# iPERDance/iPERCore

Hardware: AMD Instinct MI355X
Metric: synthesized frames/sec at 512x512 (run_imitator) (higher is better)
Workload: dtype f32; 1 GPU; run_imitator 512x512 single src/ref pair, 300-frame reference clip frame-sharded over 1 GPU(s), AttLWB-SPADE generator fp32 (BASELINE configs[1] at N = 1, configs[2] at N = 8); poses=imitate, image_size=512, frame_batch=300, frame_batch_requested=384, world_size=1, parallelism=frame-shard x1, batches_in_flight=1, weights=random-init (seeded) of the real architecture, 36,276,992 params

## Files before the change

include/lwg_hip.h:

```cpp
#ifndef LWG_HIP_H
#define LWG_HIP_H

#include <stddef.h>
#include <stdint.h>

#ifdef __cplusplus
extern "C" {
#endif

typedef void* lwg_stream_t;

#define LWG_ABI_VERSION 10
int lwg_abi_version(void);

#define LWG_MAX_TAPS 52
enum { LWG_EPI_NONE = 0, LWG_EPI_RESIDUAL = 1, LWG_EPI_SPADE = 2 };
enum { LWG_ACTIVATION_NONE = 0, LWG_ACTIVATION_RELU = 1, LWG_ACTIVATION_TANH = 2, LWG_ACTIVATION_SIGMOID = 3 };
#define LWG_ACTIVATION_RELU_MASK 5
enum { LWG_DT_F32 = 0, LWG_DT_BF16 = 1,
       LWG_DT_F32_Q4 = 2 };

typedef struct LwgConvArgs {
    const float* x0;
    const float* x1;
    int C0, C1;
    int B, H, W;
    int OH, OW;
    int M;
    int stride;
    int ntaps;
    int cshift;
    const float* w;
    int N;
    const float* bias;
    float* y;
    int YH, YW, YC, ycoff;
    int omul, ooy, oox;
    int epi;
    int act;
    const float* res;
    const float* xn;
    const float* mean;
    const float* rstd;
    int xdt;
    int ydt;
    signed char dy[LWG_MAX_TAPS];
    signed char dx[LWG_MAX_TAPS];
} LwgConvArgs;

int lwg_conv2d_nhwc_f32(const LwgConvArgs* args, lwg_stream_t stream);
size_t lwg_conv2d_ws_floats(const LwgConvArgs* args);
int lwg_conv2d_nhwc_f32_ws(const LwgConvArgs* args, float* ws, lwg_stream_t stream);
int lwg_conv_slice_count(const LwgConvArgs* args);

int lwg_conv2d_nhwc_bf16(const LwgConvArgs* args, lwg_stream_t stream);
int lwg_conv2d_winograd_f32(const LwgConvArgs* args, lwg_stream_t stream);
size_t lwg_conv2d_winograd_ws_floats(const LwgConvArgs* args);
int lwg_conv2d_winograd_f32_ws(const LwgConvArgs* args, float* ws, lwg_stream_t stream);
int lwg_conv2d_winograd_plan(const LwgConvArgs* args, int with_ws, long long* blocks, int* slices, int* nbv, int* workgroups);
int lwg_winograd_panel_f32(const float* wpanel, float* upk, int Cin, int N, const int* tap9, lwg_stream_t stream);
typedef struct LwgWinoDesc {
    const float* wpanel;
    float* upk;
    int Cin, N, first_block;
    int tap9[9];
} LwgWinoDesc;
int lwg_winograd_panels_f32(const LwgWinoDesc* descs_dev, int ndesc, int total_blocks, lwg_stream_t stream);
int lwg_conv2d_winograd4_f32(const LwgConvArgs* args, lwg_stream_t stream);
int lwg_winograd4_panel_f32(const float* wpanel, float* upk, int Cin, int N, const int* tap9, lwg_stream_t stream);
int lwg_conv2d_nhwc_bf16_hr(const LwgConvArgs* args, lwg_stream_t stream);
int lwg_conv2d_winograd_bf16(const LwgConvArgs* args, lwg_stream_t stream);
int lwg_conv2d_nhwc_c8_bf16(const LwgConvArgs* args, lwg_stream_t stream);
int lwg_conv_transpose4_nhwc_bf16(const LwgConvArgs* args, lwg_stream_t stream);
int lwg_conv_transpose4_nhwc_f32(const LwgConvArgs* args, lwg_stream_t stream);
int lwg_conv_transpose4_is_one_grid(const LwgConvArgs* args);
int lwg_conv_transpose4_winograd_f32(const LwgConvArgs* args, lwg_stream_t stream);

int lwg_conv_transpose4_winograd24_f32(const LwgConvArgs* args, lwg_stream_t stream);

int lwg_conv2d_nhwc_f32_split(const LwgConvArgs* args, lwg_stream_t stream);

size_t lwg_conv2d_wgrad_ws_floats(int Ktot, int N, int M);
int lwg_conv2d_wgrad_nhwc_f32(const LwgConvArgs* args, const float* dy, float* dw, float* ws, lwg_stream_t stream);
int lwg_conv2d_wgrad_unpacked_f32(const LwgConvArgs* args, const float* dy, float* ws, float* dw, int D0, int D1, int KH, int KW,
                                  int transposed, const int* kidx, int cin, int nout, float* db, lwg_stream_t stream);
int lwg_colsum_nhwc_f32(const float* x, size_t rows, int C, float* out, float* ws, lwg_stream_t stream);
size_t lwg_conv2d_wgrad_winograd_ws_floats(const LwgConvArgs* args);
int lwg_conv2d_wgrad_winograd_f32(const LwgConvArgs* args, const float* dy, float* ws, float* dw, int cin, int nout, lwg_stream_t stream);

int lwg_act_bwd_f32(const float* dy, const float* y, size_t n, int act, float* out, lwg_stream_t stream);
int lwg_norm_fwd_nhwc_f32(const float* x, const float* mean, const float* rstd, const float* gamma, const float* beta, int gstride,
                          int B, int HW, int C, int act, float* y, lwg_stream_t stream);
int lwg_norm_bwd_nhwc_f32(const float* dy, const float* y, const float* x, const float* mean, const float* rstd,
                          const float* gamma, int gstride, int B, int HW, int C, int act, int nsplit, float* dx, float* dgamma,
                          float* dbeta, float* ws, lwg_stream_t stream);
int lwg_adam_step_f32(float* p, const float* g, float* m, float* v, size_t n, float lr, float beta1, float beta2, float eps, int t,
                      lwg_stream_t stream);
int lwg_adam_step_dev_f32(float* p, const float* g, float* m, float* v, size_t n, float lr, float beta1, float beta2, float eps,
                          int* t_dev, lwg_stream_t stream);
int lwg_pack_panel_f32(const float* w, int D0, int D1, int KH, int KW, int transposed, const int* kidx, int ntaps, int cin,
                       int cin_pad, int nout, int n_pad, float* out, lwg_stream_t stream);
int lwg_unpack_wgrad_f32(const float* dwk, int D0, int D1, int KH, int KW, int transposed, const int* kidx, int ntaps, int cin,
                         int cin_pad, int nout, int n_pad, float* dw, lwg_stream_t stream);
typedef struct LwgPackDesc {
    const float* w;
    float* out;
    int D1, KHW, transposed, ntaps, cin, cin_pad, nout, n_pad, Kp, first_block;
    int kidx[LWG_MAX_TAPS];
} LwgPackDesc;
int lwg_pack_panels_f32(const LwgPackDesc* descs_dev, int ndesc, int total_blocks, lwg_stream_t stream);
int lwg_maxpool2_fwd_nhwc_f32(const float* x, float* y, int B, int H, int W, int C, lwg_stream_t stream);
int lwg_maxpool2_bwd_nhwc_f32(const float* x, const float* dy, float* dx, int B, int H, int W, int C, lwg_stream_t stream);
int lwg_crop_resize_bilinear_f32(const float* x, const long long* box, float* y, float* valid, int N, int C, int H, int W, int OH, int OW,
                                 lwg_stream_t stream);
int lwg_crop_resize_bilinear_bwd_f32(const float* dy, const long long* box, float* dx, int N, int C, int H, int W, int OH, int OW, lwg_stream_t stream);
int lwg_prelu_f32(const float* x, const float* slope, const float* res, size_t rows, int C, float* y, lwg_stream_t stream);
int lwg_prelu_bwd_f32(const float* x, const float* slope, const float* dy, size_t rows, int C, float* dx, lwg_stream_t stream);

int lwg_instnorm_stats_nhwc_f32(const float* x, int B, int HW, int C, float eps, float* mean, float* rstd,
                                float* ws, int nsplit, lwg_stream_t stream);
int lwg_instnorm_stats_nhwc_bf16(const void* x, int B, int HW, int C, float eps, float* mean, float* rstd, float* ws, int nsplit,
                                 lwg_stream_t stream);
int lwg_instnorm_apply_nhwc_f32(const float* x, const float* mean, const float* rstd, const float* res,
                                float* y, int B, int HW, int C, int act, lwg_stream_t stream);

int lwg_flow_resize_f32(const float* T, int n, int S, int h, int w, float* out, lwg_stream_t stream);
int lwg_lwb_attention_f32(const float* q, const float* Ks, const float* Vs, const float* bk, const float* bv,
                          const float* T, float* out, int B, int ns, int h, int w, int C, int S,
                          int src_batched, lwg_stream_t stream);
int lwg_lwb_attention_bf16(const void* q, const void* Ks, const void* Vs, const float* bk, const float* bv, const float* T, void* out,
                           int B, int ns, int h, int w, int C, int S, int src_batched, lwg_stream_t stream);
int lwg_lwb_attention_x_records(int h, int w, int C, int element_size);
int lwg_lwb_attention_x_f32(const float* x, const float* Kq, const float* kappa, const float* Vs, const float* bv, const float* T,
                            float* out, float* stats, int B, int ns, int h, int w, int C, int src_batched, lwg_stream_t stream);
int lwg_lwb_attention_x_bf16(const void* x, const void* Kq, const float* kappa, const void* Vs, const float* bv, const float* T,
                             void* out, float* stats, int B, int ns, int h, int w, int C, int src_batched, lwg_stream_t stream);
size_t lwg_instnorm_finalize_ws_floats(int B, int C, int nrec);
int lwg_instnorm_finalize_f32(float* ws, int B, int C, int nrec, float eps, float* mean, float* rstd, lwg_stream_t stream);
int lwg_lwb_attention_bwd_f32(const float* q, const float* Ks, const float* Vs, const float* bk, const float* bv,
                              const float* T, const float* dout, float* dq, float* dKs, float* dVs, int B, int ns,
                              int h, int w, int C, int S, int src_batched, lwg_stream_t stream);
int lwg_lwb_attention_kv_f32(const float* q, const float* kv, const float* bk, const float* bv, const float* T, float* out,
                             int B, int ns, int h, int w, int C, int S, int src_batched, lwg_stream_t stream);
int lwg_lwb_attention_kv_bwd_f32(const float* q, const float* kv, const float* bk, const float* bv, const float* T,
                                 const float* dout, float* dq, float* dkv, int B, int ns, int h, int w, int C, int S,
                                 int src_batched, lwg_stream_t stream);
int lwg_lwb_fuse_f32(const float* tsf_x, const float* src_x, const float* gate, const float* T, float* out, int B, int ns,
                     int h, int w, int C, int S, int src_batched, float scale_w, float scale_o, lwg_stream_t stream);

size_t lwg_rasterize_ws_bytes(int B, int nf, int S);
int lwg_project_faces_f32(const float* verts, const float* cam, const int32_t* faces, int B, int nv, int nf,
                          float eye_dist, float* faces_v, float* f2pts, lwg_stream_t stream);
int lwg_rasterize_fim_wim_f32(const float* faces_v, int B, int nf, int S, float near, float far, int32_t* fim,
                              float* wim, void* ws, lwg_stream_t stream);
int lwg_texture_sample_f32(const int32_t* fim, const float* wim, const float* faces_v, const float* textures, int B, int nf,
                           int S, int T, int tex_batched, float eps, const float* bg_color3_host, float* rgb, lwg_stream_t stream);

int lwg_flow_compose_f32(const int32_t* fim, const float* wim, int B, int S, const float* map_fn, int nf,
                         const float* f_uvs2img, const float* uv_img4, int Hu, int Wu, const float* src_f2pts,
                         int ns, float* tsf_inputs, float* Tst, float* cond_nchw, float* Tuv, lwg_stream_t stream);
int lwg_bc_transform_f32(const float* f2pts, const int32_t* fim, const float* wim, int B, int S, int nf, float* T,
                         lwg_stream_t stream);
int lwg_encode_fim_f32(const int32_t* fim, const float* map_fn, int B, int S, int nf, int D, float* out,
                       lwg_stream_t stream);

size_t lwg_smpl_lbs_ws_floats(int B, int nv, int nj);
int lwg_smpl_lbs_f32(const float* pose, int pose_stride, const float* beta, int beta_stride, int nbeta,
                     const float* cam, int cam_stride, const float* v_template, const float* offsets, int off_batched,
                     const float* shapedirs, const float* posedirs, const float* J_regressor, const int32_t* parents,
                     const float* lbs_weights, const int32_t* links, int nlinks, int B, int nv, int nj, float* verts,
                     float* j3d, float* j2d, float* ws, lwg_stream_t stream);

int lwg_head_compose_f32(const float* x, const float* wpk, const float* bg, size_t bg_bstride, int B, int S, int C,
                         float* pred, float* mask, float* img, lwg_stream_t stream);
int lwg_head_compose_q4_f32(const float* x, const float* wpk, const float* bg, size_t bg_bstride, int B, int S, int C,
                            float* pred, float* mask, float* img, lwg_stream_t stream);
int lwg_thin_conv_f32(const float* x, const float* wpk, int B, int S, int C, int ks, float* y, lwg_stream_t stream);
int lwg_head_compose_bf16(const void* x, const void* wb, const float* bg, size_t bg_bstride, int B, int S, int C, float* pred,
                          float* mask, float* img, lwg_stream_t stream);
int lwg_up4_head_compose_bf16(const LwgConvArgs* args, const void* whead, const float* bg, size_t bg_bstride, float* pred, float* mask, float* img,
                              lwg_stream_t stream);
int lwg_frames_to_u8(const float* pred, int B, int S, int bgr, uint8_t* out, lwg_stream_t stream);
int lwg_nchw_to_nhwc_f32(const float* src, float* dst, int B, int C, int Cp, int P, lwg_stream_t stream);
int lwg_nhwc_to_nchw_f32(const float* src, float* dst, int B, int C, int Cs, int P, lwg_stream_t stream);

int lwg_morph_f32(const float* in, float* out, int n, int H, int W, int ks, int mode, float* ws, lwg_stream_t stream);
int lwg_canny_f32(const float* sil, int n, int H, int W, const float* gauss9, const float* sobelx9, float low, float high,
                  float* edges, float* ws, lwg_stream_t stream);
int lwg_boundary_fill_f32(const float* src, const float* confidant, const float* outpad, const float* edges, int n, int H,
                          int W, float* out, int32_t* top3, int32_t* ws, lwg_stream_t stream);
int lwg_grid_sample_nchw_f32(const float* img, size_t img_bstride, const float* grid, int n, int C, int H, int W, int Ho,
                             int Wo, float* out, lwg_stream_t stream);
int lwg_uv_merge_f32(const float* src_warp, const float* vis, int ns, int H, int W, float* out, lwg_stream_t stream);
int lwg_uv_merge_parts_f32(const float* uv_imgs, const float* vis, int n, int H, int W, float* out, lwg_stream_t stream);
int lwg_pack_inputs_f32(const float* a, int Ca, const float* b, int Cb, const float* mask, int n, int H, int W, int Cp,
                        float* out, lwg_stream_t stream);

int lwg_device_cu_count(void);

#ifdef __cplusplus
}
#endif
#endif
```

ipercore_amd/_lib.py:

```python
import ctypes
import os
import re

_HERE = os.path.dirname(os.path.abspath(__file__))
LIB_PATH = os.path.join(_HERE, "liblwg_hip.so")
HEADER_PATH = os.path.join(os.path.dirname(_HERE), "include", "lwg_hip.h")

LWG_MAX_TAPS = 52
EPI_NONE, EPI_RESIDUAL, EPI_SPADE = 0, 1, 2
ACT_NONE, ACT_RELU, ACT_TANH, ACT_SIGMOID, ACT_LRELU = 0, 1, 2, 3, 4
ACT_RELU_MASK = 5
DT_F32, DT_BF16, DT_F32_Q4 = 0, 1, 2

c_f = ctypes.c_void_p
c_i = ctypes.c_int


class LwgConvArgs(ctypes.Structure):
    _fields_ = [
        ("x0", c_f), ("x1", c_f),
        ("C0", c_i), ("C1", c_i),
        ("B", c_i), ("H", c_i), ("W", c_i),
        ("OH", c_i), ("OW", c_i),
        ("M", c_i), ("stride", c_i), ("ntaps", c_i), ("cshift", c_i),
        ("w", c_f), ("N", c_i), ("bias", c_f),
        ("y", c_f), ("YH", c_i), ("YW", c_i), ("YC", c_i), ("ycoff", c_i),
        ("omul", c_i), ("ooy", c_i), ("oox", c_i),
        ("epi", c_i), ("act", c_i),
        ("res", c_f), ("xn", c_f), ("mean", c_f), ("rstd", c_f),
        ("xdt", c_i), ("ydt", c_i),
        ("dy", ctypes.c_byte * LWG_MAX_TAPS), ("dx", ctypes.c_byte * LWG_MAX_TAPS),
    ]


class LwgWinoDesc(ctypes.Structure):
    _fields_ = [("wpanel", ctypes.c_void_p), ("upk", ctypes.c_void_p), ("Cin", c_i), ("N", c_i), ("first_block", c_i), ("tap9", c_i * 9)]


class LwgPackDesc(ctypes.Structure):
    _fields_ = [("w", c_f), ("out", c_f)] + [(n, c_i) for n in ("D1", "KHW", "transposed", "ntaps", "cin", "cin_pad", "nout", "n_pad", "Kp",
                                                               "first_block")] + [("kidx", c_i * LWG_MAX_TAPS)]


_SIGS = {
    "lwg_abi_version": (c_i, []),
    "lwg_device_cu_count": (c_i, []),
    "lwg_conv2d_nhwc_f32": (c_i, [ctypes.POINTER(LwgConvArgs), c_f]),
    "lwg_conv2d_ws_floats": (ctypes.c_size_t, [ctypes.POINTER(LwgConvArgs)]),
    "lwg_conv2d_nhwc_f32_ws": (c_i, [ctypes.POINTER(LwgConvArgs), c_f, c_f]),
    "lwg_conv2d_nhwc_bf16": (c_i, [ctypes.POINTER(LwgConvArgs), c_f]),
    "lwg_conv2d_winograd_f32": (c_i, [ctypes.POINTER(LwgConvArgs), c_f]),
    "lwg_conv2d_winograd_ws_floats": (ctypes.c_size_t, [ctypes.POINTER(LwgConvArgs)]),
    "lwg_conv2d_winograd_f32_ws": (c_i, [ctypes.POINTER(LwgConvArgs), c_f, c_f]),
    "lwg_conv2d_winograd_plan": (c_i, [ctypes.POINTER(LwgConvArgs), c_i, ctypes.POINTER(ctypes.c_longlong), ctypes.POINTER(c_i), ctypes.POINTER(c_i),
                                       ctypes.POINTER(c_i)]),
    "lwg_winograd_panel_f32": (c_i, [c_f, c_f, c_i, c_i, ctypes.POINTER(c_i), c_f]),
    "lwg_winograd_panels_f32": (c_i, [c_f, c_i, c_i, c_f]),
    "lwg_conv2d_winograd4_f32": (c_i, [ctypes.POINTER(LwgConvArgs), c_f]),
    "lwg_winograd4_panel_f32": (c_i, [c_f, c_f, c_i, c_i, ctypes.POINTER(c_i), c_f]),
    "lwg_conv2d_nhwc_bf16_hr": (c_i, [ctypes.POINTER(LwgConvArgs), c_f]),
    "lwg_conv2d_winograd_bf16": (c_i, [ctypes.POINTER(LwgConvArgs), c_f]),
    "lwg_conv2d_nhwc_c8_bf16": (c_i, [ctypes.POINTER(LwgConvArgs), c_f]),
    "lwg_conv_transpose4_nhwc_bf16": (c_i, [ctypes.POINTER(LwgConvArgs), c_f]),
    "lwg_conv_transpose4_nhwc_f32": (c_i, [ctypes.POINTER(LwgConvArgs), c_f]),
    "lwg_conv_transpose4_winograd_f32": (c_i, [ctypes.POINTER(LwgConvArgs), c_f]),
    "lwg_conv_transpose4_winograd24_f32": (c_i, [ctypes.POINTER(LwgConvArgs), c_f]),
    "lwg_conv_transpose4_is_one_grid": (c_i, [ctypes.POINTER(LwgConvArgs)]),
    "lwg_conv_slice_count": (c_i, [ctypes.POINTER(LwgConvArgs)]),
    "lwg_conv2d_nhwc_f32_split": (c_i, [ctypes.POINTER(LwgConvArgs), c_f]),
    "lwg_conv2d_wgrad_ws_floats": (ctypes.c_size_t, [c_i, c_i, c_i]),
    "lwg_conv2d_wgrad_nhwc_f32": (c_i, [ctypes.POINTER(LwgConvArgs), c_f, c_f, c_f, c_f]),
    "lwg_conv2d_wgrad_unpacked_f32": (c_i, [ctypes.POINTER(LwgConvArgs), c_f, c_f, c_f] + [c_i] * 5 + [ctypes.POINTER(ctypes.c_int), c_i, c_i, c_f, c_f]),
    "lwg_colsum_nhwc_f32": (c_i, [c_f, ctypes.c_size_t, c_i, c_f, c_f, c_f]),
    "lwg_conv2d_wgrad_winograd_ws_floats": (ctypes.c_size_t, [ctypes.POINTER(LwgConvArgs)]),
    "lwg_conv2d_wgrad_winograd_f32": (c_i, [ctypes.POINTER(LwgConvArgs), c_f, c_f, c_f, c_i, c_i, c_f]),
    "lwg_act_bwd_f32": (c_i, [c_f, c_f, ctypes.c_size_t, c_i, c_f, c_f]),
    "lwg_norm_fwd_nhwc_f32": (c_i, [c_f, c_f, c_f, c_f, c_f, c_i, c_i, c_i, c_i, c_i, c_f, c_f]),
    "lwg_norm_bwd_nhwc_f32": (c_i, [c_f, c_f, c_f, c_f, c_f, c_f, c_i, c_i, c_i, c_i, c_i, c_i, c_f, c_f, c_f, c_f, c_f]),
    "lwg_adam_step_f32": (c_i, [c_f, c_f, c_f, c_f, ctypes.c_size_t, ctypes.c_float, ctypes.c_float, ctypes.c_float, ctypes.c_float, c_i, c_f]),
    "lwg_adam_step_dev_f32": (c_i, [c_f, c_f, c_f, c_f, ctypes.c_size_t, ctypes.c_float, ctypes.c_float, ctypes.c_float, ctypes.c_float, c_f, c_f]),
    "lwg_pack_panel_f32": (c_i, [c_f] + [c_i] * 5 + [ctypes.POINTER(ctypes.c_int)] + [c_i] * 5 + [c_f, c_f]),
    "lwg_pack_panels_f32": (c_i, [c_f, c_i, c_i, c_f]),
    "lwg_unpack_wgrad_f32": (c_i, [c_f] + [c_i] * 5 + [ctypes.POINTER(ctypes.c_int)] + [c_i] * 5 + [c_f, c_f]),
    "lwg_maxpool2_fwd_nhwc_f32": (c_i, [c_f, c_f, c_i, c_i, c_i, c_i, c_f]),
    "lwg_maxpool2_bwd_nhwc_f32": (c_i, [c_f, c_f, c_f, c_i, c_i, c_i, c_i, c_f]),
    "lwg_crop_resize_bilinear_f32": (c_i, [c_f, c_f, c_f, c_f, c_i, c_i, c_i, c_i, c_i, c_i, c_f]),
    "lwg_crop_resize_bilinear_bwd_f32": (c_i, [c_f, c_f, c_f, c_i, c_i, c_i, c_i, c_i, c_i, c_f]),
    "lwg_prelu_f32": (c_i, [c_f, c_f, c_f, ctypes.c_size_t, c_i, c_f, c_f]),
    "lwg_prelu_bwd_f32": (c_i, [c_f, c_f, c_f, ctypes.c_size_t, c_i, c_f, c_f]),
    "lwg_instnorm_stats_nhwc_f32": (c_i, [c_f, c_i, c_i, c_i, ctypes.c_float, c_f, c_f, c_f, c_i, c_f]),
    "lwg_instnorm_apply_nhwc_f32": (c_i, [c_f, c_f, c_f, c_f, c_f, c_i, c_i, c_i, c_i, c_f]),
    "lwg_lwb_attention_f32": (c_i, [c_f, c_f, c_f, c_f, c_f, c_f, c_f, c_i, c_i, c_i, c_i, c_i, c_i, c_i, c_f]),
    "lwg_lwb_attention_bf16": (c_i, [c_f, c_f, c_f, c_f, c_f, c_f, c_f, c_i, c_i, c_i, c_i, c_i, c_i, c_i, c_f]),
    "lwg_instnorm_stats_nhwc_bf16": (c_i, [c_f, c_i, c_i, c_i, ctypes.c_float, c_f, c_f, c_f, c_i, c_f]),
    "lwg_head_compose_bf16": (c_i, [c_f, c_f, c_f, ctypes.c_size_t, c_i, c_i, c_i, c_f, c_f, c_f, c_f]),
    "lwg_up4_head_compose_bf16": (c_i, [ctypes.POINTER(LwgConvArgs), c_f, c_f, ctypes.c_size_t, c_f, c_f, c_f, c_f]),
    "lwg_flow_resize_f32": (c_i, [c_f, c_i, c_i, c_i, c_i, c_f, c_f]),
    "lwg_lwb_fuse_f32": (c_i, [c_f] * 5 + [c_i] * 7 + [ctypes.c_float, ctypes.c_float, c_f]),
    "lwg_lwb_attention_x_f32": (c_i, [c_f] * 8 + [c_i] * 6 + [c_f]),
    "lwg_lwb_attention_x_bf16": (c_i, [c_f] * 8 + [c_i] * 6 + [c_f]),
    "lwg_lwb_attention_x_records": (c_i, [c_i, c_i, c_i, c_i]),
    "lwg_instnorm_finalize_ws_floats": (ctypes.c_size_t, [c_i, c_i, c_i]),
    "lwg_instnorm_finalize_f32": (c_i, [c_f, c_i, c_i, c_i, ctypes.c_float, c_f, c_f, c_f]),
    "lwg_lwb_attention_bwd_f32": (c_i, [c_f] * 10 + [c_i] * 7 + [c_f]),
    "lwg_lwb_attention_kv_f32": (c_i, [c_f] * 6 + [c_i] * 7 + [c_f]),
    "lwg_lwb_attention_kv_bwd_f32": (c_i, [c_f] * 8 + [c_i] * 7 + [c_f]),
    "lwg_rasterize_ws_bytes": (ctypes.c_size_t, [c_i, c_i, c_i]),
    "lwg_project_faces_f32": (c_i, [c_f, c_f, c_f, c_i, c_i, c_i, ctypes.c_float, c_f, c_f, c_f]),
    "lwg_rasterize_fim_wim_f32": (c_i, [c_f, c_i, c_i, c_i, ctypes.c_float, ctypes.c_float, c_f, c_f, c_f, c_f]),
    "lwg_texture_sample_f32": (c_i, [c_f, c_f, c_f, c_f, c_i, c_i, c_i, c_i, c_i, ctypes.c_float, ctypes.POINTER(ctypes.c_float), c_f, c_f]),
    "lwg_flow_compose_f32": (c_i, [c_f, c_f, c_i, c_i, c_f, c_i, c_f, c_f, c_i, c_i, c_f, c_i, c_f, c_f, c_f, c_f, c_f]),
    "lwg_bc_transform_f32": (c_i, [c_f, c_f, c_f, c_i, c_i, c_i, c_f, c_f]),
    "lwg_encode_fim_f32": (c_i, [c_f, c_f, c_i, c_i, c_i, c_i, c_f, c_f]),
    "lwg_smpl_lbs_ws_floats": (ctypes.c_size_t, [c_i, c_i, c_i]),
    "lwg_smpl_lbs_f32": (c_i, [c_f, c_i, c_f, c_i, c_i, c_f, c_i, c_f, c_f, c_i, c_f, c_f, c_f, c_f, c_f, c_f, c_i, c_i, c_i,
                               c_i, c_f, c_f, c_f, c_f, c_f]),
    "lwg_head_compose_f32": (c_i, [c_f, c_f, c_f, ctypes.c_size_t, c_i, c_i, c_i, c_f, c_f, c_f, c_f]),
    "lwg_head_compose_q4_f32": (c_i, [c_f, c_f, c_f, ctypes.c_size_t, c_i, c_i, c_i, c_f, c_f, c_f, c_f]),
    "lwg_thin_conv_f32": (c_i, [c_f, c_f, c_i, c_i, c_i, c_i, c_f, c_f]),
    "lwg_nchw_to_nhwc_f32": (c_i, [c_f, c_f, c_i, c_i, c_i, c_i, c_f]),
    "lwg_nhwc_to_nchw_f32": (c_i, [c_f, c_f, c_i, c_i, c_i, c_i, c_f]),
    "lwg_frames_to_u8": (c_i, [c_f, c_i, c_i, c_i, c_f, c_f]),
    "lwg_morph_f32": (c_i, [c_f, c_f, c_i, c_i, c_i, c_i, c_i, c_f, c_f]),
    "lwg_canny_f32": (c_i, [c_f, c_i, c_i, c_i, ctypes.POINTER(ctypes.c_float), ctypes.POINTER(ctypes.c_float),
                            ctypes.c_float, ctypes.c_float, c_f, c_f, c_f]),
    "lwg_boundary_fill_f32": (c_i, [c_f, c_f, c_f, c_f, c_i, c_i, c_i, c_f, c_f, c_f, c_f]),
    "lwg_grid_sample_nchw_f32": (c_i, [c_f, ctypes.c_size_t, c_f, c_i, c_i, c_i, c_i, c_i, c_i, c_f, c_f]),
    "lwg_uv_merge_f32": (c_i, [c_f, c_f, c_i, c_i, c_i, c_f, c_f]),
    "lwg_uv_merge_parts_f32": (c_i, [c_f, c_f, c_i, c_i, c_i, c_f, c_f]),
    "lwg_pack_inputs_f32": (c_i, [c_f, c_i, c_f, c_i, c_f, c_i, c_i, c_i, c_i, c_f, c_f]),
}

_lib = None


def header_symbols():
    with open(HEADER_PATH) as fp:
        src = re.sub(r"/\*.*?\*/", "", fp.read(), flags=re.S)
    return sorted(set(re.findall(r"\b(lwg_[a-z0-9_]+)\s*\(", src)))


def lib():
    global _lib
    if _lib is None:
        if not os.path.exists(LIB_PATH):
            raise RuntimeError(
                f"{LIB_PATH} not found: the HIP kernels are not built (run `python -c 'import __graft_entry__ as g; "
                "g.build()'` or `make -C ipercore_amd/csrc`).  There is no CPU fallback.")
        import torch
        handle = ctypes.CDLL(LIB_PATH)
        for name, (res, args) in _SIGS.items():
            fn = getattr(handle, name)
            fn.restype = res
            fn.argtypes = args
        if handle.lwg_abi_version() != 10:
            raise RuntimeError("liblwg_hip.so ABI version mismatch")
        _lib = handle
    return _lib


def check(err, what):
    if err != 0:
        raise RuntimeError(f"{what} failed with hipError_t {err}")
```

ipercore_amd/csrc/conv_winograd4.hip:

```cpp
#include <hip/hip_runtime.h>
#include "lwg_common.h"
#include "lwg_conv_wino.h"

#define W4_THREADS 512
#define W4_PBX 8
#define W4_PBY 4
#define W4_NB 64
#define W4_KS 8
#define W4_HW 34
#define W4_HH 18
#ifndef W4_RS
#define W4_RS 40
#endif
#define W4_PLANE (18 * W4_RS + 4)
#define W4_RAW (W4_KS * W4_PLANE)
#define W4_VS (36 * W4_KS * 32)
#define W4_NEL (W4_HW * W4_HH * 2)
#define W4_NQ 3
#define W4_DUMP_OFF (2 * W4_RAW + 2 * W4_VS)
#define W4_DUMP (W4_THREADS + 3 * W4_PLANE)
#define W4_LOOP (W4_DUMP_OFF + W4_DUMP)
#define W4_MSR 68
#define W4_NPL 28
#define W4_MS (W4_NPL * 16 * W4_MSR)
#define W4_BIAS_OFF (W4_LOOP > W4_MS ? W4_LOOP : W4_MS)
#ifndef LWG_W4_XCD
#define LWG_W4_XCD 1
#endif
#ifndef LWG_W4_CHUNK
#define LWG_W4_CHUNK 1
#endif
#ifndef LWG_W4_RDMAP
#define LWG_W4_RDMAP 1
#endif
#ifndef LWG_W4_SMALL
#define LWG_W4_SMALL 1
#endif
#define W4SB() __builtin_amdgcn_sched_barrier(0)

#ifdef LWG_W4_TS
#define W4TS(i) do { if (tid == 0 && lab_bi == 1) reinterpret_cast<unsigned long long*>(const_cast<float*>(a.res))[(size_t)blockIdx.x * 16 + (i)] = __builtin_readcyclecounter(); } while (0)
#define W4TSA(i) do { if (tid == 0) reinterpret_cast<unsigned long long*>(const_cast<float*>(a.res))[(size_t)blockIdx.x * 16 + (i)] = __builtin_readcyclecounter(); } while (0)
#else
#define W4TS(i) do { } while (0)
#define W4TSA(i) do { } while (0)
#endif

#ifndef W4_NT
#define W4_NT 0
#endif
#ifndef W4_NT_LD
#define W4_NT_LD W4_NT
#endif
#ifndef W4_NT_RES
#define W4_NT_RES 0
#endif
#ifndef W4_NT_ST
#define W4_NT_ST 2
#endif

__device__ __forceinline__ void w4_bt6(const float (&r)[6], float (&v)[6]) {
    const float a = __builtin_fmaf(-4.f, r[2], r[4]), b = __builtin_fmaf(-4.f, r[1], r[3]);
    const float c = r[4] - r[2], e = r[3] - r[1];
    v[0] = __builtin_fmaf(-5.f, r[2], __builtin_fmaf(4.f, r[0], r[4]));
    v[1] = a + b;
    v[2] = a - b;
    v[3] = __builtin_fmaf(2.f, e, c);
    v[4] = __builtin_fmaf(-2.f, e, c);
    v[5] = __builtin_fmaf(-5.f, r[3], __builtin_fmaf(4.f, r[1], r[5]));
}

template <int EPI, bool TWO, bool SM = false>
__global__ __launch_bounds__(SM ? 256 : W4_THREADS, 1) void lwg_conv_winograd4_kernel(const LwgConvArgs a) {
    constexpr bool SMS = SM && EPI == LWG_EPI_SPADE;
    constexpr int NVP = SM && !SMS ? 2 : 1;
    constexpr int NTH = SM ? 256 : W4_THREADS;
    constexpr int NQ = SM ? 5 : W4_NQ;
    constexpr int NBV = SM ? 32 : W4_NB;
    constexpr int MSR = SM ? 36 : W4_MSR;
    constexpr int NHF = SM ? 2 : 1;
    extern __shared__ __attribute__((aligned(16))) float smem[];
    const int wid = __builtin_amdgcn_readfirstlane(threadIdx.x >> 6);
    const float* __restrict__ bias = a.bias;
    const int H = a.H, W = a.W, Cin = a.C0 + a.C1, N = a.N;
    float* __restrict__ y = a.y;
    float* const raw0 = smem;
    float* const Ms = smem;
    const int tid = threadIdx.x, lane = tid & 63;
    const CwGrid g = cw_grid(a.B, H, W, N, 4 * W4_PBX, 4 * W4_PBY, NBV);
    const CwOrder o = cw_order(cw4_order_kind(LWG_W4_XCD, LWG_W4_CHUNK, SM, gridDim.x, N / NBV, Cin, N, g.tiles, g.total), gridDim.x, blockIdx.x, N / NBV, g);
    int blk = blockIdx.x;
    const int nst = Cin / W4_KS;
    const __amdgpu_buffer_rsrc_t ru = __builtin_amdgcn_make_buffer_rsrc(const_cast<float*>(a.w), 0, (int)(144u * (unsigned)Cin * (unsigned)N), 0x00020000);
    const int q = wid & 3, ct = SM ? 0 : wid >> 2;
    const int half = SM ? 0 : wid >> 2;
    floatx16 acc[9];
    CwBlock<NQ, TWO> bk;
    unsigned uvoff, uvoffc;
    auto setup = [&](int id) {
        int cb, t;
        cw_block(o, id, cb, t);
        bk.locate(a, g, t, 4 * W4_PBX, 4 * W4_PBY, SMS ? cw4_n0_spade_small(cb) : cw_n0(cb, NBV));
        int tids = tid;
        asm volatile("" : "+v"(tids));
        bk.halo(a, tids, NTH, W4_HW, W4_NEL);
        const int col = SMS ? bk.n0 + (((lane & 31) >> 4) << 5) + (lane & 15) : bk.n0 + ct * 32 + (lane & 31);
        uvoff = (unsigned)(((lane >> 5) * 9 * N + 4 * col) * 4);
        uvoffc = (unsigned)(((lane >> 5) * 9 * N + 8 * N + col) * 4);
    };
    setup(blk);
    int wst[NQ];
#pragma unroll
    for (int k = 0; k < NQ; ++k) {
        const int i = tid + NTH * k;
        const int pix = i >> 1, hq = i & 1, hy = pix / W4_HW, hx = pix - hy * W4_HW;
        wst[k] = i < W4_NEL ? 4 * hq * W4_PLANE + hy * W4_RS + hx : W4_DUMP_OFF + tid;
    }
    floatx4 rreg[NQ];
    auto rld1 = [&](int st, int k) -> floatx4 {
#ifdef W4_LAB_HFIX
        const int c = 0 * st;
#else
        const int c = st * W4_KS;
#endif
        return bk.template rld1<W4_NT_LD>(a, c, k);
    };
    auto rst1 = [&](int buf, int k, floatx4 v) { cw_rst1(raw0 + buf * W4_RAW + wst[k], W4_PLANE, v); };
    floatx4 ufa[4], ufb[4];
    float ufc[4];
    const unsigned ukk = (unsigned)N * 72u;
    const unsigned uq = (unsigned)q * (unsigned)nst * 4u * ukk;
    const unsigned ubo = (unsigned)N * 16u;
    auto uldpart = [&](int set, int st, int kk, int part) {
#ifdef W4_LAB_UFIX
        const unsigned so = uq + 0u * (unsigned)(st + kk);
#else
        const unsigned so = uq + (unsigned)(st * 4 + kk) * ukk;
#endif
        if (part == 0) ufa[set] = cw_buf_load(ru, uvoff, so);
        else if (part == 1) ufb[set] = cw_buf_load(ru, uvoff, so + ubo);
        else ufc[set] = __builtin_bit_cast(float, __builtin_amdgcn_raw_buffer_load_b32(ru, (int)uvoffc, (int)so, 0));
    };
    auto uldset = [&](int set, int st, int kk) {
#ifdef W4_LAB_UFIX
        const unsigned so = uq + 0u * (unsigned)(st + kk);
#else
        const unsigned so = uq + (unsigned)(st * 4 + kk) * ukk;
#endif
        ufa[set] = cw_buf_load(ru, uvoff, so);
        ufb[set] = cw_buf_load(ru, uvoff, so + ubo);
        ufc[set] = __builtin_bit_cast(float, __builtin_amdgcn_raw_buffer_load_b32(ru, (int)uvoffc, (int)so, 0));
    };
    const int patch = tid & 31, tc = (tid >> 5) & 7;
    const int pty = patch >> 3, ptx = patch & 7;
    unsigned dbs = (unsigned)(tc * W4_PLANE + (4 * pty) * W4_RS + 4 * ptx) >> 2;
    asm volatile("" : "+v"(dbs));
    dbs <<= 2;
    unsigned dbx[NHF], vbx[NHF], vbt[NHF];
    float alpha[NHF], beta[NHF], nbeta[NHF];
#pragma unroll
    for (int hi = 0; hi < NHF; ++hi) {
        const int hf = SM ? hi : half;
        dbx[hi] = (unsigned)(tc * W4_PLANE + (4 * pty + hf) * W4_RS + 4 * ptx) >> 2;
        asm volatile("" : "+v"(dbx[hi]));
        dbx[hi] <<= 2;
        vbx[hi] = (unsigned)(2 * W4_RAW + (hf ? 30 : 0) * W4_KS * 32 + tc * 32 + patch);
        vbt[hi] = (unsigned)(2 * W4_RAW + (hf ? 18 : 6) * W4_KS * 32 + tc * 32 + patch);
        asm volatile("" : "+v"(vbx[hi]));
        asm volatile("" : "+v"(vbt[hi]));
        alpha[hi] = hf ? -1.f : -4.f;
        beta[hi] = hf ? 2.f : 1.f;
        nbeta[hi] = -beta[hi];
    }
    unsigned fbs[2];
    fbs[0] = (unsigned)(2 * W4_RAW + (6 * q) * W4_KS * 32 + lane);
    fbs[1] = (unsigned)(2 * W4_RAW + (6 * (4 + (q >> 1)) + 3 * (q & 1)) * W4_KS * 32 + lane);
    asm volatile("" : "+v"(fbs[0]));
    asm volatile("" : "+v"(fbs[1]));
    float fb[9];
    auto frag1 = [&](int buf, int kk, int j) -> float {
        return smem[fbs[j < 6 ? 0 : 1] + buf * W4_VS + ((j < 6 ? j : j - 6) * W4_KS + 2 * kk) * 32];
    };
    auto rd6 = [&](unsigned base, int buf, int r, float (&d)[6]) {
        const floatx4 v4 = *reinterpret_cast<const floatx4*>(smem + base + buf * W4_RAW + r * W4_RS);
        const float2 v2 = *reinterpret_cast<const float2*>(smem + base + buf * W4_RAW + r * W4_RS + 4);
        d[0] = v4[0]; d[1] = v4[1]; d[2] = v4[2]; d[3] = v4[3]; d[4] = v2.x; d[5] = v2.y;
    };
    auto vst6 = [&](unsigned base, int buf, int i, const float (&v)[6]) {
        float* dst = smem + base + buf * W4_VS + (6 * i) * W4_KS * 32;
#pragma unroll
        for (int nu = 0; nu < 6; ++nu) dst[nu * W4_KS * 32] = v[nu];
    };
    auto transform_full = [&](int buf) {
#pragma unroll
        for (int hi = 0; hi < NHF; ++hi) {
            float X[6], P[6], Q[6], v[6];
            {
                float dR[3][6];
                rd6(dbx[hi], buf, 0, dR[0]); rd6(dbx[hi], buf, 2, dR[1]); rd6(dbx[hi], buf, 4, dR[2]);
#pragma unroll
                for (int j = 0; j < 6; ++j) X[j] = __builtin_fmaf(-5.f, dR[1][j], __builtin_fmaf(4.f, dR[0][j], dR[2][j]));
            }
            {
                float dR[2][6];
                rd6(dbs, buf, 2, dR[0]); rd6(dbs, buf, 4, dR[1]);
#pragma unroll
                for (int j = 0; j < 6; ++j) P[j] = __builtin_fmaf(alpha[hi], dR[0][j], dR[1][j]);
                rd6(dbs, buf, 1, dR[0]); rd6(dbs, buf, 3, dR[1]);
#pragma unroll
                for (int j = 0; j < 6; ++j) Q[j] = __builtin_fmaf(alpha[hi], dR[0][j], dR[1][j]);
            }
            w4_bt6(X, v); vst6(vbx[hi], buf, 0, v);
            float T[6];
#pragma unroll
            for (int j = 0; j < 6; ++j) T[j] = __builtin_fmaf(beta[hi], Q[j], P[j]);
            w4_bt6(T, v); vst6(vbt[hi], buf, 0, v);
#pragma unroll
            for (int j = 0; j < 6; ++j) T[j] = __builtin_fmaf(nbeta[hi], Q[j], P[j]);
            w4_bt6(T, v); vst6(vbt[hi], buf, 1, v);
        }
    };
    auto iteration = [&](int s, auto SET, auto NXT) {
        constexpr int set = decltype(SET)::value;
        constexpr bool nxt = decltype(NXT)::value != 0;
        const int s3 = s + 3 < nst ? s + 3 : nst - 1;
        float X[6], P[6], Q[6], dR[3][6];
        auto mf = [&](int kk, int j, bool refill) {
            acc[j] = __builtin_amdgcn_mfma_f32_32x32x2f32(j < 4 ? ufa[kk][j & 3] : j < 8 ? ufb[kk][j & 3] : ufc[kk], fb[j], acc[j], 0, 0, 0);
#ifndef W4_KO_FRAG
            if (refill && (j & 1)) {
                fb[j - 1] = kk < 3 ? frag1(set, kk + 1, j - 1) : frag1(set ^ 1, 0, j - 1);
                fb[j] = kk < 3 ? frag1(set, kk + 1, j) : frag1(set ^ 1, 0, j);
            } else if (refill && j == 8) {
                fb[8] = kk < 3 ? frag1(set, kk + 1, 8) : frag1(set ^ 1, 0, 8);
            }
#endif
            W4SB();
        };
        auto ul = [&](int kk, int part) {
#ifndef W4_KO_ULD
            if (kk < 2) uldpart(kk + 2, s, kk + 2, part);
            else if (nxt) uldpart(kk - 2, s + 1, kk - 2, part);
#endif
            W4SB();
        };
        auto halo = [&](int k) {
#ifdef W4_KO_HALO
            return;
#endif
            if (nxt) { rst1(set, k, rreg[k]); rreg[k] = rld1(s3, k); }
            W4SB();
        };
#ifdef W4_KO_TR
        constexpr bool trn = false;
// ... 126 lines not shown
    for (int j = 0; j < 9; ++j) fb[j] = frag1(0, 0, j);
#pragma unroll
    for (int j = 0; j < 9; ++j)
#pragma unroll
        for (int r = 0; r < 16; ++r) acc[j][r] = 0.f;
    if (q == 1) {
#pragma unroll
        for (int g = 0; g < 4; ++g) {
            const floatx4 b4 = *reinterpret_cast<const floatx4*>(smem + W4_BIAS_OFF + ct * 32 + 8 * g + 4 * (lane >> 5));
#pragma unroll
            for (int k = 0; k < 4; ++k) acc[1][4 * g + k] = b4[k];
        }
    }
    W4TS(1);
    {
        int s = 0;
        for (; s + 2 < nst; s += 2) {
            iteration(s, IntC<0>(), IntC<1>());
            iteration(s + 1, IntC<1>(), IntC<1>());
        }
        iteration(s, IntC<0>(), IntC<1>());
        iteration(s + 1, IntC<1>(), IntC<0>());
    }
    W4TS(2);
    const int eb = bk.b, ex0 = bk.x0, ey0 = bk.y0, en0 = bk.n0;
#pragma unroll
    for (int r = 0; r < 16; ++r) {
        const float m0 = acc[0][r], m1 = acc[1][r], m2 = acc[2][r], m3 = acc[3][r], m4 = acc[4][r], m5 = acc[5][r];
        const float s12 = m1 + m2, d12 = m1 - m2, s34 = m3 + m4, d34 = m3 - m4;
        acc[0][r] = (m0 + s12) + s34;
        acc[1][r] = __builtin_fmaf(2.f, d34, d12);
        acc[2][r] = __builtin_fmaf(4.f, s34, s12);
        acc[3][r] = __builtin_fmaf(8.f, d34, d12) + m5;
    }
    if (q & 1) {
#pragma unroll
        for (int r = 0; r < 16; ++r) {
            const float h0 = acc[6][r], h1 = acc[7][r];
            acc[6][r] = h0 + h1;
            acc[7][r] = h0 - h1;
        }
    } else {
#pragma unroll
        for (int r = 0; r < 16; ++r) {
            const float h0 = acc[6][r], h1 = acc[7][r], h2 = acc[8][r];
            acc[6][r] = (h0 + h1) + h2;
            acc[7][r] = h1 - h2;
            acc[8][r] = h1 + h2;
        }
    }
    W4TS(4);
    int tide = tid;
    asm volatile("" : "+v"(tide));
    const int lanee = tide & 63;
    const int rb = wid & 3;
    const unsigned l5 = (unsigned)lanee & 31u, gsel = (0x0FF0F00Fu >> l5) & 1u;
    const int gidx = __builtin_popcount((gsel ? 0x0FF0F00Fu : 0xF00F0FF0u) & ((1u << l5) - 1u));
    const int p16 = LWG_W4_RDMAP && !SM ? (wid >> 2) * 4 + 2 * (lanee >> 5) + (gsel ? 0 : 1) + 8 * (gidx >> 3) : (wid >> 2) * 8 + (lanee >> 3);
    const int n4 = SMS ? (lanee & 3) * 4 : LWG_W4_RDMAP && !SM ? (gidx & 7) * 4 : (lanee & 7) * 4;
    const int cbase = SMS ? (en0 >> 6) * 32 + ((en0 >> 4) & 1) * 16 : en0 >> 1;
    floatx4 mu, rs;
    if (EPI == LWG_EPI_SPADE) {
        mu = *reinterpret_cast<const floatx4*>(a.mean + (size_t)eb * a.YC + cbase + n4);
        rs = *reinterpret_cast<const floatx4*>(a.rstd + (size_t)eb * a.YC + cbase + n4);
    }
    typedef unsigned int w4_u4 __attribute__((ext_vector_type(4)));
    const unsigned img_bytes = (unsigned)(H * W) * (unsigned)a.YC * 4u;
    const __amdgpu_buffer_rsrc_t ry = __builtin_amdgcn_make_buffer_rsrc(y + (size_t)eb * H * W * a.YC, 0, (int)img_bytes, 0x00020000);
    const float* const esrc = EPI == LWG_EPI_SPADE ? a.xn : EPI == LWG_EPI_RESIDUAL ? a.res : a.y;
    const __amdgpu_buffer_rsrc_t re = __builtin_amdgcn_make_buffer_rsrc(const_cast<float*>(esrc) + (size_t)eb * H * W * a.YC, 0, (int)img_bytes, 0x00020000);
    const int chan = EPI == LWG_EPI_SPADE ? cbase + n4 : a.ycoff + en0 + n4;
    bool more = false;
    int nblk = blk;
#pragma unroll
    for (int ph = 0; ph < 2; ++ph) {
        if (ph == 1) __syncthreads();
        if (((lanee >> 4) & 1) == ph) {
            float* dst = Ms + (lanee & 15) * MSR + ct * 32 + 4 * (lanee >> 5);
#pragma unroll
            for (int g = 0; g < 4; ++g) {
#pragma unroll
                for (int bb = 0; bb < 4; ++bb)
                    *reinterpret_cast<floatx4*>(dst + (4 * q + bb) * 16 * MSR + 8 * g) = floatx4{acc[bb][4 * g], acc[bb][4 * g + 1], acc[bb][4 * g + 2], acc[bb][4 * g + 3]};
#pragma unroll
                for (int i = 0; i < 3; ++i)
                    *reinterpret_cast<floatx4*>(dst + (16 + 3 * q + i) * 16 * MSR + 8 * g) = floatx4{acc[6 + i][4 * g], acc[6 + i][4 * g + 1], acc[6 + i][4 * g + 2], acc[6 + i][4 * g + 3]};
            }
        }
        unsigned vo[NVP][4];
#pragma unroll
        for (int hp = 0; hp < NVP; ++hp) {
            const int p = ph * 16 + (SMS ? lanee >> 2 : SM ? 8 * hp + (lanee >> 3) : p16);
            const int ox = ex0 + 4 * (p & 7) + rb, oyb = ey0 + 4 * (p >> 3);
#pragma unroll
            for (int i = 0; i < 4; ++i)
                vo[hp][i] = cw4_out_voff(ox, oyb + i, H, W, a.YC, chan);
        }
        floatx4 ext[2][4];
        if (EPI != LWG_EPI_NONE) {
#pragma unroll
            for (int h = 0; h < (EPI == LWG_EPI_SPADE ? 1 : 2); ++h)
#pragma unroll
                for (int i = 0; i < 4; ++i) ext[h][i] = __builtin_bit_cast(floatx4, __builtin_amdgcn_raw_buffer_load_b128(re, (int)cw4_out_group(vo[NVP == 2 ? h : 0][i], h, !SM), 0, W4_NT_RES));
        }
        if (ph == 1) {
            W4TS(8);
            nblk = blk + (int)gridDim.x;
            more = cw_has_block(o, nblk);
            setup(more ? nblk : blk);
            W4TS(9);
            issue_loads();
            W4TS(10);
        }
        __syncthreads();
        if (ph == 0) W4TS(5); else W4TS(7);
        floatx4 gam[4];
#pragma unroll
        for (int h = 0; h < 2; ++h) {
            const float* base = Ms + (SMS ? lanee >> 2 : SM ? 8 * h + (lanee >> 3) : p16) * MSR + (SMS ? h * 16 : SM ? 0 : h * 32) + n4;
            floatx4 F[6];
#pragma unroll
            for (int xi = 0; xi < 4; ++xi) F[xi] = *reinterpret_cast<const floatx4*>(base + (4 * xi + rb) * 16 * MSR);
            const int ia = rb == 0 ? 0 : rb == 2 ? 2 : 1, ib = (rb & 1) ? 4 : 3;
            const float cb = (float)(1 << rb);
#pragma unroll
            for (int r = 0; r < 2; ++r) {
                const float* hb = base + (16 + 6 * r) * 16 * MSR;
                const floatx4 pa = *reinterpret_cast<const floatx4*>(hb + ia * 16 * MSR);
                const floatx4 pb = *reinterpret_cast<const floatx4*>(hb + ib * 16 * MSR);
                floatx4 f;
#pragma unroll
                for (int c = 0; c < 4; ++c) f[c] = __builtin_fmaf(cb, pb[c], pa[c]);
                if (rb == 3) f += *reinterpret_cast<const floatx4*>(hb + 5 * 16 * MSR);
                F[4 + r] = f;
            }
            floatx4 o[4];
#pragma unroll
            for (int c = 0; c < 4; ++c) {
                const float s12 = F[1][c] + F[2][c], d12 = F[1][c] - F[2][c], s34 = F[3][c] + F[4][c], d34 = F[3][c] - F[4][c];
                o[0][c] = (F[0][c] + s12) + s34;
                o[1][c] = __builtin_fmaf(2.f, d34, d12);
                o[2][c] = __builtin_fmaf(4.f, s34, s12);
                o[3][c] = __builtin_fmaf(8.f, d34, d12) + F[5][c];
            }
            if (EPI == LWG_EPI_SPADE) {
                if (h == 0) {
#pragma unroll
                    for (int i = 0; i < 4; ++i) gam[i] = o[i];
                    continue;
                }
#pragma unroll
                for (int i = 0; i < 4; ++i)
#pragma unroll
                    for (int c = 0; c < 4; ++c) o[i][c] = (ext[0][i][c] - mu[c]) * rs[c] * (1.f + gam[i][c]) + o[i][c];
            } else if (EPI == LWG_EPI_RESIDUAL) {
                if (a.act == LWG_ACT_RELU_MASK) {
#pragma unroll
                    for (int i = 0; i < 4; ++i)
#pragma unroll
                        for (int c = 0; c < 4; ++c) o[i][c] = ext[h][i][c] > 0.f ? o[i][c] : 0.f;
                } else {
#pragma unroll
                    for (int i = 0; i < 4; ++i) o[i] += ext[h][i];
                }
            }
            lwg_act_dispatch(a.act, [&](auto ACTC) {
                constexpr int EA = decltype(ACTC)::value;
#pragma unroll
                for (int i = 0; i < 4; ++i)
#pragma unroll
                    for (int c = 0; c < 4; ++c) o[i][c] = lwg_act_c<EA>(o[i][c], a.act);
            });
#pragma unroll
            for (int i = 0; i < 4; ++i)
                __builtin_amdgcn_raw_buffer_store_b128(__builtin_bit_cast(w4_u4, o[i]), ry, (int)cw4_out_group(vo[NVP == 2 ? h : 0][i], h, EPI != LWG_EPI_SPADE && !SM), 0, W4_NT_ST);
        }
        if (ph == 0) W4TS(6);
    }
    W4TS(3);
#ifdef LWG_W4_TS
    ++lab_bi;
#endif
    if (!more) break;
    blk = nblk;
    __syncthreads();
    }
    W4TSA(12);
#ifdef LWG_W4_TS
    if (tid == 0) reinterpret_cast<unsigned long long*>(const_cast<float*>(a.res))[(size_t)blockIdx.x * 16 + 13] = (unsigned long long)lab_bi;
#endif
}


__global__ __launch_bounds__(256) void lwg_winograd4_panel_kernel(const float* __restrict__ wp, float* __restrict__ U, int Cin, int N, LwgWinoTaps taps) {
    const int n = blockIdx.x * 64 + (threadIdx.x & 63), c = blockIdx.y * 4 + (threadIdx.x >> 6);
    if (n >= N || c >= Cin) return;
    double g[3][3];
#pragma unroll
    for (int r = 0; r < 3; ++r)
#pragma unroll
        for (int s = 0; s < 3; ++s) {
            const int k = ((c >> 5) * 9 + taps.t[3 * r + s]) * 32 + (c & 31);
            g[r][s] = (double)wp[((size_t)(k >> 2) * N + n) * 4 + (k & 3)];
        }
    const double G[6][3] = {{1.0 / 4, 0, 0}, {-1.0 / 6, -1.0 / 6, -1.0 / 6}, {-1.0 / 6, 1.0 / 6, -1.0 / 6}, {1.0 / 24, 1.0 / 12, 1.0 / 6}, {1.0 / 24, -1.0 / 12, 1.0 / 6}, {0, 0, 1}};
    double t[6][3];
#pragma unroll
    for (int i = 0; i < 6; ++i)
#pragma unroll
        for (int s = 0; s < 3; ++s) t[i][s] = G[i][0] * g[0][s] + G[i][1] * g[1][s] + G[i][2] * g[2][s];
    const int s8 = c >> 3, kk = (c & 7) >> 1, kh = c & 1;
#pragma unroll
    for (int qq = 0; qq < 4; ++qq) {
        float* dst = U + ((((size_t)qq * (Cin >> 3) + s8) * 4 + kk) * 2 + kh) * 9 * (size_t)N;
        float o[9];
#pragma unroll
        for (int j = 0; j < 9; ++j) {
            const int xi = j < 6 ? qq : 4 + (qq >> 1), nu = j < 6 ? j : 3 * (qq & 1) + (j - 6);
            o[j] = (float)(t[xi][0] * G[nu][0] + t[xi][1] * G[nu][1] + t[xi][2] * G[nu][2]);
        }
        *reinterpret_cast<floatx4*>(dst + 4 * n) = floatx4{o[0], o[1], o[2], o[3]};
        *reinterpret_cast<floatx4*>(dst + 4 * (size_t)N + 4 * n) = floatx4{o[4], o[5], o[6], o[7]};
        dst[8 * (size_t)N + n] = o[8];
    }
}

extern "C" int lwg_winograd4_panel_f32(const float* wpanel, float* upk, int Cin, int N, const int* tap9, lwg_stream_t stream_) {
    LwgWinoTaps taps;
    if (!cw_panel_args_ok(wpanel, upk, Cin, N, tap9, taps)) return (int)hipErrorInvalidValue;
    hipLaunchKernelGGL(lwg_winograd4_panel_kernel, dim3((unsigned)((N + 63) / 64), (unsigned)((Cin + 3) / 4)), dim3(256), 0,
                       reinterpret_cast<hipStream_t>(stream_), wpanel, upk, Cin, N, taps);
    return (int)hipGetLastError();
}

template <int EPI, bool SM>
static int lwg_wino4_go(const LwgConvArgs& a, dim3 grid, size_t lds, hipStream_t stream) {
    return a.C1 > 0 ? cw_launch<lwg_conv_winograd4_kernel<EPI, true, SM>>(grid, SM ? 256 : W4_THREADS, lds, stream, a)
                    : cw_launch<lwg_conv_winograd4_kernel<EPI, false, SM>>(grid, SM ? 256 : W4_THREADS, lds, stream, a);
}

extern "C" int lwg_conv2d_winograd4_f32(const LwgConvArgs* pa, lwg_stream_t stream_) {
    hipStream_t stream = reinterpret_cast<hipStream_t>(stream_);
    if (!pa || !cw_contract_ok(*pa, 144ull, 256ll)) return (int)hipErrorInvalidValue;
    const LwgConvArgs& a = *pa;
    const size_t lds = (size_t)(W4_BIAS_OFF + 64) * 4;
    const int cus = lwg_device_cus();
    long long total = cw_total_blocks(a.B, a.H, a.W, a.N, 4 * W4_PBX, 4 * W4_PBY, W4_NB);
    const bool sm = LWG_W4_SMALL && 2 * total <= cus;
    if (sm) total *= 2;
    const dim3 grid = cw_persistent_grid(total, cus);
    if (a.epi == LWG_EPI_SPADE) return sm ? lwg_wino4_go<LWG_EPI_SPADE, true>(a, grid, lds, stream) : lwg_wino4_go<LWG_EPI_SPADE, false>(a, grid, lds, stream);
    if (a.epi == LWG_EPI_RESIDUAL) return sm ? lwg_wino4_go<LWG_EPI_RESIDUAL, true>(a, grid, lds, stream) : lwg_wino4_go<LWG_EPI_RESIDUAL, false>(a, grid, lds, stream);
    return sm ? lwg_wino4_go<LWG_EPI_NONE, true>(a, grid, lds, stream) : lwg_wino4_go<LWG_EPI_NONE, false>(a, grid, lds, stream);
}
```

ipercore_amd/csrc/lwb_attn_x.hip:

```cpp
#include "lwg_common.h"
#include "lwg_conv_args.h"

typedef unsigned int uintx4 __attribute__((ext_vector_type(4)));

template <typename ST> struct AttnXTraits;
template <> struct AttnXTraits<float> {
    static constexpr int CPL = 4;
    __device__ static __forceinline__ void unpack(const uintx4 v, float (&f)[4]) {
#pragma unroll
        for (int k = 0; k < 4; ++k) {
            const unsigned u = v[k];
            f[k] = __builtin_bit_cast(float, u);
        }
    }
    __device__ static __forceinline__ uintx4 pack(const float (&f)[4]) {
        uintx4 v;
#pragma unroll
        for (int k = 0; k < 4; ++k) v[k] = __builtin_bit_cast(unsigned, f[k]);
        return v;
    }
};
template <> struct AttnXTraits<__bf16> {
    static constexpr int CPL = 8;
    __device__ static __forceinline__ void unpack(const uintx4 v, float (&f)[8]) {
#pragma unroll
        for (int k = 0; k < 4; ++k) {
            f[2 * k] = __builtin_bit_cast(float, v[k] << 16);
            f[2 * k + 1] = __builtin_bit_cast(float, v[k] & 0xffff0000u);
        }
    }
    __device__ static __forceinline__ uintx4 pack(const float (&f)[8]) {
        typedef __bf16 bf16x2 __attribute__((ext_vector_type(2)));
        uintx4 v;
#pragma unroll
        for (int k = 0; k < 4; ++k) {
            bf16x2 p;
            p[0] = (__bf16)f[2 * k];
            p[1] = (__bf16)f[2 * k + 1];
            v[k] = __builtin_bit_cast(unsigned, p);
        }
        return v;
    }
};

template <typename ST, int LPP, bool STATS, int NSU, int PW, int OCC, bool PIPE = false>
__global__ __launch_bounds__(256 * PW, PW == 1 ? OCC : 1) void lwg_lwb_attnx_kernel(const ST* __restrict__ x, const ST* __restrict__ Kq,
                                                                 const float* __restrict__ kappa, const ST* __restrict__ Vs,
                                                                 const float* __restrict__ bv, const float* __restrict__ T,
                                                                 ST* __restrict__ out, float* __restrict__ stats, int B, int ns, int h, int w,
                                                                 int src_batched) {
    using TR = AttnXTraits<ST>;
    constexpr int CPL = TR::CPL;
    constexpr int C = CPL * LPP;
    constexpr int PPW = 64 / LPP;
    constexpr int PPP = 4 * PPW;
    constexpr int NPASS = 64 / PPP;
    constexpr int NIT = NPASS / PW;
    static_assert(NPASS % PW == 0, "PW must divide the tile's pass count");
    constexpr int NT = NSU > 0 ? NSU : 1;
    constexpr unsigned ROWB = (unsigned)C * sizeof(ST);
    const int lane = threadIdx.x & 63, wid = threadIdx.x >> 6;
    const int wq = wid & 3, pl = wid >> 2;
    const int cl = lane % LPP, pg = lane / LPP;
    const int tiles_x = (w + 7) >> 3;
    int tile, b;
    if (LWG_ATTNX_INTERLEAVE) {
        const int xcd = blockIdx.x & 7;
        const long idx = blockIdx.x >> 3;
        const long grp = idx / B;
        tile = (int)(grp * 8 + xcd);
        b = (int)(idx - grp * B);
        if (tile >= tiles_x * ((h + 7) >> 3)) return;
    } else {
        const long L = lwg_xcd_remap(blockIdx.x, gridDim.x);
        tile = (int)(L / B);
        b = (int)(L - (long)tile * B);
    }
    const int ty = tile / tiles_x, tx = tile - ty * tiles_x;
    const int hw = h * w;
    const unsigned nsrc = (unsigned)(src_batched ? B * ns : ns);
    __amdgpu_buffer_rsrc_t rK = __builtin_amdgcn_make_buffer_rsrc(const_cast<ST*>(Kq), 0, (int)(nsrc * (unsigned)hw * ROWB), 0x00020000);
    __amdgpu_buffer_rsrc_t rV = __builtin_amdgcn_make_buffer_rsrc(const_cast<ST*>(Vs), 0, (int)(nsrc * (unsigned)hw * ROWB), 0x00020000);
    __amdgpu_buffer_rsrc_t rA = __builtin_amdgcn_make_buffer_rsrc(const_cast<float*>(kappa), 0, (int)(nsrc * (unsigned)hw * 4u), 0x00020000);
    const float inv_sqrt_c = 1.0f / sqrtf((float)C);
    constexpr bool BV_REG = CPL == 4 || LWG_ATTNX_BVREG16;
    float bvr[CPL];
    if (BV_REG) {
#pragma unroll
        for (int k = 0; k < CPL; ++k) bvr[k] = bv[CPL * cl + k];
    }
    const float2* Tb = reinterpret_cast<const float2*>(T) + (size_t)b * ns * hw;

    auto pixel_of = [&](int pass, int& yc, int& xc) -> bool {
        const int p = pass * PPP + wq * PPW + pg;
        const int y = ty * 8 + (p >> 3), xx = tx * 8 + (p & 7);
        const bool live = y < h && xx < w;
        yc = live ? y : ty * 8;
        xc = live ? xx : tx * 8;
        return live;
    };
    extern __shared__ __attribute__((aligned(16))) char smem_ax[];
    char* xs = smem_ax;
    float2* Tl = reinterpret_cast<float2*>(smem_ax + NPASS * 4096);
    {
        __amdgpu_buffer_rsrc_t rX = __builtin_amdgcn_make_buffer_rsrc(const_cast<ST*>(x) + (size_t)b * hw * C, 0, (int)((unsigned)hw * ROWB), 0x00020000);
#pragma unroll
        for (int it = 0; it < NIT; ++it) {
            const int pass = it * PW + pl;
            int yc, xc;
            pixel_of(pass, yc, xc);
            const unsigned voff = (unsigned)(yc * w + xc) * ROWB + (unsigned)(CPL * cl) * (unsigned)sizeof(ST);
            __builtin_amdgcn_raw_ptr_buffer_load_lds(rX, (__attribute__((address_space(3))) void*)(xs + (pass * 4 + wq) * 1024), 16, (int)voff, 0, 0, 0);
        }
        for (int i = threadIdx.x; i < ns * 64; i += 256 * PW) {
            const int s = i >> 6, p = i & 63;
            const int y = ty * 8 + (p >> 3), xx = tx * 8 + (p & 7);
            const bool in = y < h && xx < w;
            Tl[i] = Tb[(size_t)s * hw + (size_t)(in ? y : ty * 8) * w + (in ? xx : tx * 8)];
        }
        asm volatile("s_waitcnt vmcnt(0)" ::: "memory");
        __syncthreads();
    }
    auto x_row = [&](int pass) -> uintx4 { return *reinterpret_cast<const uintx4*>(xs + ((pass * 4 + wq) * 64 + lane) * 16); };

    float shift[CPL], s1[CPL], s2[CPL];
    if (STATS) {
        TR::unpack(*reinterpret_cast<const uintx4*>(xs + cl * 16), shift);
#pragma unroll
        for (int k = 0; k < CPL; ++k) s1[k] = s2[k] = 0.f;
    }
    int nlive = 0;
    auto stats_add = [&](const float (&xv)[CPL]) {
        ++nlive;
        if (PW == 1) {
#pragma unroll
            for (int k = 0; k < CPL; ++k) {
                const float d = xv[k] - shift[k];
                s1[k] += d;
                s2[k] = __builtin_fmaf(d, d, s2[k]);
            }
        }
    };
    auto taps_of = [&](const float2 t, float (&wt)[4], int& tx0, int& ty0) {
        const float ix = ((t.x + 1.f) * (float)w - 1.f) * 0.5f, iy = ((t.y + 1.f) * (float)h - 1.f) * 0.5f;
        const float fx0 = floorf(ix), fy0 = floorf(iy);
        const float wx1 = ix - fx0, wy1 = iy - fy0, wx0 = (fx0 + 1.f) - ix, wy0 = (fy0 + 1.f) - iy;
        tx0 = (int)fminf(fmaxf(fx0, -2.f), (float)w + 1.f);
        ty0 = (int)fminf(fmaxf(fy0, -2.f), (float)h + 1.f);
        wt[0] = wy0 * wx0; wt[1] = wy0 * wx1; wt[2] = wy1 * wx0; wt[3] = wy1 * wx1;
    };
    auto fold = [&](const float (&ka)[CPL], const float (&va)[CPL], float kap, const float (&xv)[CPL], float& mrun, float& lrun, float (&o)[CPL]) {
        float dot = 0.f;
#pragma unroll
        for (int k = 0; k < CPL; ++k) dot = __builtin_fmaf(ka[k], xv[k], dot);
#pragma unroll
        for (int off = LPP >> 1; off > 0; off >>= 1) dot += __shfl_xor(dot, off, 64);
        const float logit = (dot + kap) * inv_sqrt_c;
        const float mnew = fmaxf(mrun, logit);
        const float corr = expf(mrun - mnew);
        const float pr = expf(logit - mnew);
        lrun = __builtin_fmaf(lrun, corr, pr);
#pragma unroll
        for (int k = 0; k < CPL; ++k) o[k] = __builtin_fmaf(o[k], corr, pr * va[k]);
        mrun = mnew;
    };
    auto finish = [&](long gp, float lrun, const float (&o)[CPL]) {
        const float invl = 1.f / lrun;
        float r[CPL];
        if (!BV_REG) {
#pragma unroll
            for (int k = 0; k < CPL; k += 4) {
                const floatx4 b4 = *reinterpret_cast<const floatx4*>(bv + CPL * cl + k);
#pragma unroll
                for (int j = 0; j < 4; ++j) bvr[k + j] = b4[j];
            }
        }
#pragma unroll
        for (int k = 0; k < CPL; ++k) r[k] = __builtin_fmaf(o[k], invl, bvr[k]);
        *reinterpret_cast<uintx4*>(out + gp * C + CPL * cl) = TR::pack(r);
    };

    if constexpr (PIPE) {
        static_assert(NSU == 2 && PW == 1 && (NIT % 2) == 0, "the pipelined form is the ns = 2 frame-batch form");
        bool mine = false;
#pragma unroll 1
        for (int it = 0; it < NIT; ++it) {
            int yc, xc;
            const bool live = pixel_of(it, yc, xc);
            const int ptile = it * PPP + wq * PPW + pg;
#pragma unroll
            for (int s = 0; s < 2; ++s) {
                const float2 t = Tl[s * 64 + ptile];
                float wt[4];
                int tx0, ty0;
                taps_of(t, wt, tx0, ty0);
                mine |= live && tx0 >= -1 && tx0 < w && ty0 >= -1 && ty0 < h;
            }
        }
        if (__syncthreads_or(mine ? 1 : 0) == 0) {
#pragma unroll 1
            for (int it = 0; it < NIT; ++it) {
                int yc, xc;
                const bool live = pixel_of(it, yc, xc);
                float xv[CPL];
                TR::unpack(x_row(it), xv);
                if (live) {
                    if (STATS) stats_add(xv);
                    float o[CPL];
#pragma unroll
                    for (int k = 0; k < CPL; ++k) o[k] = 0.f;
                    finish(((long)b * h + yc) * w + xc, 2.f, o);
                }
            }
        } else {
            struct Taps { uintx4 kr[2][4], vr[2][4]; float ar[2][4], wt[2][4]; };
            auto issue = [&](int pass, Taps& g) {
                int yc, xc;
                const bool live = pixel_of(pass, yc, xc);
                const int ptile = pass * PPP + wq * PPW + pg;
#pragma unroll
                for (int s = 0; s < 2; ++s) {
                    int tx0, ty0;
                    taps_of(Tl[s * 64 + ptile], g.wt[s], tx0, ty0);
                    const unsigned pbase = (unsigned)(src_batched ? b * ns + s : s) * (unsigned)hw;
#pragma unroll
                    for (int tp = 0; tp < 4; ++tp) {
                        const int tyy = ty0 + (tp >> 1), txx = tx0 + (tp & 1);
                        const bool ok = live && tyy >= 0 && tyy < h && txx >= 0 && txx < w;
                        const unsigned pix = pbase + (unsigned)(tyy * w + txx);
                        const unsigned voff = ok ? pix * ROWB + (unsigned)(CPL * cl) * (unsigned)sizeof(ST) : 0xC0000000u;
                        g.kr[s][tp] = __builtin_bit_cast(uintx4, __builtin_amdgcn_raw_buffer_load_b128(rK, (int)voff, 0, 0));
                        g.vr[s][tp] = __builtin_bit_cast(uintx4, __builtin_amdgcn_raw_buffer_load_b128(rV, (int)voff, 0, 0));
                        g.ar[s][tp] = __builtin_bit_cast(float, __builtin_amdgcn_raw_buffer_load_b32(rA, ok ? (int)(pix * 4u) : (int)0xC0000000u, 0, 0));
                    }
                }
            };
            auto consume = [&](int pass, const Taps& g) {
                int yc, xc;
                const bool live = pixel_of(pass, yc, xc);
                float xv[CPL];
                TR::unpack(x_row(pass), xv);
                if (STATS && live) stats_add(xv);
                float mrun = -INFINITY, lrun = 0.f;
                float o[CPL];
#pragma unroll
                for (int k = 0; k < CPL; ++k) o[k] = 0.f;
#pragma unroll
                for (int s = 0; s < 2; ++s) {
                    float ka[CPL], va[CPL], kap = 0.f;
#pragma unroll
                    for (int k = 0; k < CPL; ++k) ka[k] = va[k] = 0.f;
#pragma unroll
                    for (int tp = 0; tp < 4; ++tp) {
                        float k8[CPL], v8[CPL];
                        TR::unpack(g.kr[s][tp], k8);
                        TR::unpack(g.vr[s][tp], v8);
#pragma unroll
                        for (int k = 0; k < CPL; ++k) {
                            ka[k] = __builtin_fmaf(k8[k], g.wt[s][tp], ka[k]);
                            va[k] = __builtin_fmaf(v8[k], g.wt[s][tp], va[k]);
                        }
                        kap = __builtin_fmaf(g.ar[s][tp], g.wt[s][tp], kap);
                    }
                    fold(ka, va, kap, xv, mrun, lrun, o);
                }
                if (live) finish(((long)b * h + yc) * w + xc, lrun, o);
            };
            Taps g0, g1;
            issue(0, g0);
#pragma unroll 1
            for (int it = 0; it < NIT; it += 2) {
                issue(it + 1, g1);
                consume(it, g0);
                issue(it + 2 < NIT ? it + 2 : it + 1, g0);
                consume(it + 1, g1);
            }
        }
    } else {
#pragma unroll 1
    for (int it = 0; it < NIT; ++it) {
        const int pass = it * PW + pl;
        int yc, xc;
        const bool live = pixel_of(pass, yc, xc);
        const long gp = ((long)b * h + yc) * w + xc;
        const int ptile = pass * PPP + wq * PPW + pg;
        float xv[CPL];
        TR::unpack(x_row(pass), xv);
        if (STATS && live) stats_add(xv);
        float mrun = -INFINITY, lrun = 0.f;
        float o[CPL];
#pragma unroll
        for (int k = 0; k < CPL; ++k) o[k] = 0.f;

        auto source = [&](int s, const float2 t) {
            float wt[4];
            int tx0, ty0;
            taps_of(t, wt, tx0, ty0);
            const bool any_tap = live && tx0 >= -1 && tx0 < w && ty0 >= -1 && ty0 < h;
            float ka[CPL], va[CPL], kap = 0.f;
#pragma unroll
            for (int k = 0; k < CPL; ++k) ka[k] = va[k] = 0.f;
            if (__builtin_amdgcn_ballot_w64(any_tap) != 0ull) {
                const unsigned sidx = (unsigned)(src_batched ? b * ns + s : s);
                const unsigned pbase = sidx * (unsigned)hw;
                uintx4 kr[4], vr[4];
                float ar[4];
#pragma unroll
                for (int tp = 0; tp < 4; ++tp) {
                    const int tyy = ty0 + (tp >> 1), txx = tx0 + (tp & 1);
                    const bool ok = live && tyy >= 0 && tyy < h && txx >= 0 && txx < w;
                    const unsigned pix = pbase + (unsigned)(tyy * w + txx);
                    const unsigned voff = ok ? pix * ROWB + (unsigned)(CPL * cl) * (unsigned)sizeof(ST) : 0xC0000000u;
                    kr[tp] = __builtin_bit_cast(uintx4, __builtin_amdgcn_raw_buffer_load_b128(rK, (int)voff, 0, 0));
                    vr[tp] = __builtin_bit_cast(uintx4, __builtin_amdgcn_raw_buffer_load_b128(rV, (int)voff, 0, 0));
                    ar[tp] = __builtin_bit_cast(float, __builtin_amdgcn_raw_buffer_load_b32(rA, ok ? (int)(pix * 4u) : (int)0xC0000000u, 0, 0));
                }
#pragma unroll
                for (int tp = 0; tp < 4; ++tp) {
                    float k8[CPL], v8[CPL];
                    TR::unpack(kr[tp], k8);
                    TR::unpack(vr[tp], v8);
#pragma unroll
                    for (int k = 0; k < CPL; ++k) {
                        ka[k] = __builtin_fmaf(k8[k], wt[tp], ka[k]);
                        va[k] = __builtin_fmaf(v8[k], wt[tp], va[k]);
                    }
                    kap = __builtin_fmaf(ar[tp], wt[tp], kap);
                }
            }
            fold(ka, va, kap, xv, mrun, lrun, o);
        };
        if (NSU > 0) {
#pragma unroll
            for (int s = 0; s < NT; ++s) source(s, Tl[s * 64 + ptile]);
        } else {
#pragma unroll 1
            for (int s = 0; s < ns; ++s) source(s, Tl[s * 64 + ptile]);
        }
        if (live) finish(gp, lrun, o);
    }
    }

    if (STATS) {
        if (PW > 1) {
            __shared__ float acc[4][64][2 * CPL];
            if (pl == 0) {
#pragma unroll
                for (int k = 0; k < 2 * CPL; ++k) acc[wq][lane][k] = 0.f;
            }
            __syncthreads();
#pragma unroll 1
            for (int p = 0; p < NPASS; ++p) {
                if (pl == p % PW) {
                    int yc, xc;
                    if (pixel_of(p, yc, xc)) {
                        float xv[CPL];
                        TR::unpack(x_row(p), xv);
#pragma unroll
                        for (int k = 0; k < CPL; ++k) {
                            const float d = xv[k] - shift[k];
                            acc[wq][lane][k] += d;
                            acc[wq][lane][CPL + k] = __builtin_fmaf(d, d, acc[wq][lane][CPL + k]);
                        }
                    }
                }
                __syncthreads();
            }
            if (pl == 0) {
#pragma unroll
                for (int k = 0; k < CPL; ++k) {
                    s1[k] = acc[wq][lane][k];
                    s2[k] = acc[wq][lane][CPL + k];
                }
            }
        }
        __syncthreads();
        float (*sh)[2][C] = reinterpret_cast<float (*)[2][C]>(smem_ax);
        float* shn = reinterpret_cast<float*>(smem_ax + 4 * 2 * C * sizeof(float));
        float fn = (float)nlive;
#pragma unroll
        for (int off = LPP; off < 64; off <<= 1) {
#pragma unroll
            for (int k = 0; k < CPL; ++k) {
                s1[k] += __shfl_xor(s1[k], off, 64);
                s2[k] += __shfl_xor(s2[k], off, 64);
            }
            fn += __shfl_xor(fn, off, 64);
        }
        if (pg == 0) {
            if (pl == 0) {
#pragma unroll
                for (int k = 0; k < CPL; ++k) {
                    sh[wq][0][CPL * cl + k] = s1[k];
                    sh[wq][1][CPL * cl + k] = s2[k];
                }
            }
            if (cl == 0) shn[wid] = fn;
        }
        __syncthreads();
        if (wid == 0 && pg == 0) {
            float tn = 0.f;
#pragma unroll
            for (int k = 0; k < 4 * PW; ++k) tn += shn[k];
            const int nrec = tiles_x * ((h + 7) >> 3);
#pragma unroll
            for (int k = 0; k < CPL; ++k) {
                const int c = CPL * cl + k;
                const float t1 = ((sh[0][0][c] + sh[1][0][c]) + sh[2][0][c]) + sh[3][0][c];
                const float t2 = ((sh[0][1][c] + sh[1][1][c]) + sh[2][1][c]) + sh[3][1][c];
                const float mean = shift[k] + t1 / tn;
                const float m2 = t2 - t1 * t1 / tn;
                float* rec = stats + (((size_t)b * nrec + tile) * C + c) * 3;
                rec[0] = tn;
                rec[1] = mean;
                rec[2] = m2 > 0.f ? m2 : 0.f;
            }
        }
    }
}

extern "C" int lwg_lwb_attention_x_records(int h, int w, int C, int esz) {
    if (h <= 0 || w <= 0 || C <= 0 || (esz != 2 && esz != 4)) return 0;
    const int lpp = C / (16 / esz);
    if (lpp < 8 || lpp > 64 || (lpp & (lpp - 1)) != 0) return 0;
    return ((w + 7) >> 3) * ((h + 7) >> 3);
}

template <typename ST>
static int lwg_attnx_launch(const ST* x, const ST* Kq, const float* kappa, const ST* Vs, const float* bv, const float* T, ST* out, float* stats,
                            int B, int ns, int h, int w, int C, int src_batched, hipStream_t stream) {
    if (!x || !Kq || !kappa || !Vs || !bv || !T || !out || B <= 0 || ns <= 0 || ns > 64 || h <= 0 || w <= 0) return (int)hipErrorInvalidValue;
    const unsigned long long nsrc = (unsigned long long)(src_batched ? B * ns : ns);
    if (nsrc * (unsigned long long)h * w * (unsigned long long)C * sizeof(ST) >= 0xC0000000ull) return (int)hipErrorInvalidValue;
    const long tiles = (long)((w + 7) >> 3) * ((h + 7) >> 3);
    constexpr int CPL = AttnXTraits<ST>::CPL;
    const int npass = (C / CPL) / 4;
    const dim3 grid((unsigned)((LWG_ATTNX_INTERLEAVE ? (tiles + 7) / 8 * 8 : tiles) * B));
    const bool wide = LWG_ATTNX_WIDE && tiles * B < 512 && npass >= 4;
#define LWG_ATTNX_GO(LPP, ST_, NSU, PW)                                                                                              \
    {                                                                                                                                \
             \
        constexpr bool pipe = LWG_ATTNX_PIPE && CPL == 4 && (LPP) == 64 && (NSU) == 2 && (PW) == 1;                                  \
        auto kern = lwg_lwb_attnx_kernel<ST, LPP, ST_, NSU, PW, (pipe ? 2 : CPL == 4 ? LWG_ATTNX_OCC : LWG_ATTNX_OCC16), pipe>;        \
        const size_t lds = (size_t)((LPP) / 4) * 4096 + (size_t)ns * 512;                         \
        static unsigned long long lds_ok = 0;                                                                                        \
        if (lds > 65536) {                                                                                                           \
            const hipError_t e = lwg_allow_dynamic_lds(reinterpret_cast<const void*>(kern), lds, lds_ok);                            \
            if (e != hipSuccess) return (int)e;                                                                                      \
        }                                                                                                                            \
        hipLaunchKernelGGL(kern, grid, dim3(256 * PW), lds, stream, x, Kq, kappa, Vs, bv, T, out, stats, B, ns, h, w, src_batched);   \
    }
#define LWG_ATTNX_PW(LPP, ST_, NSU)                                                                                                  \
    {                                                                                                                                \
        if constexpr ((LPP) / 4 >= 4) {                                                                                              \
            if (wide) LWG_ATTNX_GO(LPP, ST_, NSU, 4) else LWG_ATTNX_GO(LPP, ST_, NSU, 1)                                             \
        } else {                                                                                                                     \
            LWG_ATTNX_GO(LPP, ST_, NSU, 1)                                                                                           \
        }                                                                                                                            \
    }
#define LWG_ATTNX_LAUNCH(LPP)                                                                                                        \
    if (stats) { if (LWG_ATTNX_NSU2 && ns == 2) LWG_ATTNX_PW(LPP, true, 2) else LWG_ATTNX_PW(LPP, true, 0) }                         \
    else { if (LWG_ATTNX_NSU2 && ns == 2) LWG_ATTNX_PW(LPP, false, 2) else LWG_ATTNX_PW(LPP, false, 0) }
    switch (C / CPL) {
        case 8: LWG_ATTNX_LAUNCH(8) break;
        case 16: LWG_ATTNX_LAUNCH(16) break;
        case 32: LWG_ATTNX_LAUNCH(32) break;
        case 64: if constexpr (CPL == 4) { LWG_ATTNX_LAUNCH(64) break; }
                 return (int)hipErrorInvalidValue;
        default: return (int)hipErrorInvalidValue;
    }
#undef LWG_ATTNX_LAUNCH
#undef LWG_ATTNX_PW
#undef LWG_ATTNX_GO
    return (int)hipGetLastError();
}

extern "C" int lwg_lwb_attention_x_f32(const float* x, const float* Kq, const float* kappa, const float* Vs, const float* bv, const float* T,
                                       float* out, float* stats, int B, int ns, int h, int w, int C, int src_batched, lwg_stream_t stream_) {
    if (C != 32 && C != 64 && C != 128 && C != 256) return (int)hipErrorInvalidValue;
    return lwg_attnx_launch<float>(x, Kq, kappa, Vs, bv, T, out, stats, B, ns, h, w, C, src_batched, reinterpret_cast<hipStream_t>(stream_));
}

extern "C" int lwg_lwb_attention_x_bf16(const void* x, const void* Kq, const float* kappa, const void* Vs, const float* bv, const float* T,
                                        void* out, float* stats, int B, int ns, int h, int w, int C, int src_batched, lwg_stream_t stream_) {
    if (C != 64 && C != 128 && C != 256) return (int)hipErrorInvalidValue;
    return lwg_attnx_launch<__bf16>(static_cast<const __bf16*>(x), static_cast<const __bf16*>(Kq), kappa, static_cast<const __bf16*>(Vs), bv, T,
                                    static_cast<__bf16*>(out), stats, B, ns, h, w, C, src_batched, reinterpret_cast<hipStream_t>(stream_));
}

__global__ __launch_bounds__(1024) void lwg_in_stats_merge_seg(const float* __restrict__ ws, int C, int nrec, int nseg, float eps,
                                                              float* __restrict__ part, float* __restrict__ mean, float* __restrict__ rstd) {
    const int lane = threadIdx.x & 63, wid = threadIdx.x >> 6;
    const int c = blockIdx.x * 64 + lane, b = blockIdx.y, seg = blockIdx.z;
    const bool cok = c < C;
    const float* base = ws + ((size_t)b * nrec * C + (cok ? c : 0)) * 3;
    const float r = base[1];
    const int per = (nrec + nseg - 1) / nseg;
    const int r0 = seg * per, r1 = min(nrec, r0 + per);
    float sa = 0.f, ss = 0.f, sq = 0.f;
    if (cok) {
        for (int i = r0 + wid; i < r1; i += 16) {
            const float* o = base + (size_t)i * C * 3;
            const float n = o[0], d = o[1] - r;
            sa += n;
            ss = __builtin_fmaf(n, d, ss);
            sq += __builtin_fmaf(n * d, d, o[2]);
        }
    }
    __shared__ float sh[16][3][64];
    sh[wid][0][lane] = sa;
    sh[wid][1][lane] = ss;
    sh[wid][2][lane] = sq;
    __syncthreads();
    if (wid == 0 && cok) {
        float ta = 0.f, ts = 0.f, tq = 0.f;
#pragma unroll
        for (int k = 0; k < 16; ++k) { ta += sh[k][0][lane]; ts += sh[k][1][lane]; tq += sh[k][2][lane]; }
        if (nseg == 1) {
            const float m2 = tq - ts * ts / ta;
            mean[(size_t)b * C + c] = r + ts / ta;
            rstd[(size_t)b * C + c] = 1.0f / sqrtf((m2 > 0.f ? m2 : 0.f) / ta + eps);
        } else {
            float* o = part + (((size_t)b * nseg + seg) * C + c) * 3;
            o[0] = ta; o[1] = ts; o[2] = tq;
        }
    }
}

__global__ __launch_bounds__(256) void lwg_in_stats_merge_fin(const float* __restrict__ ws, const float* __restrict__ part, int BC, int C, int nrec,
                                                             int nseg, float eps, float* __restrict__ mean, float* __restrict__ rstd) {
    const int i = blockIdx.x * 256 + threadIdx.x;
    if (i >= BC) return;
    const int b = i / C, c = i - b * C;
    const float r = ws[((size_t)b * nrec * C + c) * 3 + 1];
    float ta = 0.f, ts = 0.f, tq = 0.f;
    for (int s = 0; s < nseg; ++s) {
        const float* o = part + (((size_t)b * nseg + s) * C + c) * 3;
        ta += o[0]; ts += o[1]; tq += o[2];
    }
    const float m2 = tq - ts * ts / ta;
    mean[i] = r + ts / ta;
    rstd[i] = 1.0f / sqrtf((m2 > 0.f ? m2 : 0.f) / ta + eps);
}

extern "C" size_t lwg_instnorm_finalize_ws_floats(int B, int C, int nrec) {
    if (B <= 0 || C <= 0 || nrec <= 0) return 0;
    const size_t nseg = nrec > 512 ? (size_t)(nrec + 255) / 256 : 0;
    return (size_t)B * nrec * C * 3 + (size_t)B * nseg * C * 3;
}
extern "C" int lwg_instnorm_finalize_f32(float* ws, int B, int C, int nrec, float eps, float* mean, float* rstd, lwg_stream_t stream_) {
    if (!ws || !mean || !rstd || B <= 0 || C <= 0 || nrec <= 0 || B > 65535) return (int)hipErrorInvalidValue;
    hipStream_t stream = reinterpret_cast<hipStream_t>(stream_);
    const int nseg = nrec > 512 ? (nrec + 255) / 256 : 1;
    if (nseg > 65535) return (int)hipErrorInvalidValue;
    float* part = ws + (size_t)B * nrec * C * 3;
    hipLaunchKernelGGL(lwg_in_stats_merge_seg, dim3((C + 63) / 64, B, nseg), dim3(1024), 0, stream, ws, C, nrec, nseg, eps, part, mean, rstd);
    if (nseg > 1)
        hipLaunchKernelGGL(lwg_in_stats_merge_fin, dim3((B * C + 255) / 256), dim3(256), 0, stream, ws, part, B * C, C, nrec, nseg, eps, mean, rstd);
    return (int)hipGetLastError();
}
```

ipercore_amd/csrc/lwg_conv_epilogue.h:

```cpp
#pragma once
#include "lwg_common.h"
#include "lwg_conv_args.h"

template <int TM, int TN, int EPI, int EA>
__device__ __forceinline__ void lwg_conv_epilogue_a(const LwgConvArgs& a, floatx16 (&acc)[TM][TN], int m_base, int n_base,
                                                    int wm, int wn, int lane, int ooy_add, int oox_add) {
    const int khalf = lane >> 5;
    const int HW = a.OH * a.OW;
    const bool direct = (a.omul == 1) && (a.YH == a.OH) && (a.YW == a.OW);
    const int ncol0 = n_base + wn * TN * 32 + 4 * khalf;
    floatx4 bias4[TN][4];
#pragma unroll
    for (int j = 0; j < TN; ++j)
#pragma unroll
        for (int g = 0; g < 4; ++g) {
            bias4[j][g] = floatx4{0.f, 0.f, 0.f, 0.f};
            if (a.bias) bias4[j][g] = *reinterpret_cast<const floatx4*>(a.bias + ncol0 + 32 * j + 8 * g);
        }
#pragma unroll
    for (int i = 0; i < TM; ++i) {
        const int m = m_base + wm * TM * 32 + i * 32 + (lane & 31);
        if (m >= a.M) continue;
        size_t opix = (size_t)m;
        int bimg = 0;
        if (!direct || EPI == LWG_EPI_SPADE) {
            const int b = m / HW;
            bimg = b;
            if (!direct) {
                const int rem = m - b * HW;
                const int oy = rem / a.OW, ox = rem - oy * a.OW;
                opix = ((size_t)b * a.YH + (oy * a.omul + a.ooy + ooy_add)) * a.YW + (ox * a.omul + a.oox + oox_add);
            }
        }
        if (EPI == LWG_EPI_SPADE) {
            static_assert(EPI != LWG_EPI_SPADE || TN == 2, "SPADE epilogue needs gamma|beta in one wave");
            const int ch0 = ((n_base + wn * TN * 32) >> 1) + 4 * khalf;
            const float* xr = a.xn + opix * a.YC + ch0;
            const float* mr = a.mean + (size_t)bimg * a.YC + ch0;
            const float* rr = a.rstd + (size_t)bimg * a.YC + ch0;
            float* yr = a.y + opix * a.YC + ch0;
#pragma unroll
            for (int g = 0; g < 4; ++g) {
                const floatx4 xv = *reinterpret_cast<const floatx4*>(xr + 8 * g);
                const floatx4 mu = *reinterpret_cast<const floatx4*>(mr + 8 * g);
                const floatx4 rs = *reinterpret_cast<const floatx4*>(rr + 8 * g);
                floatx4 o;
#pragma unroll
                for (int c = 0; c < 4; ++c) {
                    const float gm = acc[i][0][4 * g + c] + bias4[0][g][c];
                    const float bt = acc[i][TN - 1][4 * g + c] + bias4[TN - 1][g][c];
                    o[c] = lwg_act_c<EA>((xv[c] - mu[c]) * rs[c] * (1.f + gm) + bt, a.act);
                }
                *reinterpret_cast<floatx4*>(yr + 8 * g) = o;
            }
        } else if (EPI == LWG_EPI_NONE && a.ydt == LWG_DT_F32_Q4) {
            const int b = m / HW;
            const int rem = m - b * HW;
            const int oy = rem / a.OW, ox = rem - oy * a.OW;
            const size_t plane = (size_t)a.YH * a.YW;
            const size_t pix = (size_t)(oy * a.omul + a.ooy + ooy_add) * a.YW + (ox * a.omul + a.oox + oox_add);
            float* yq = a.y + (((size_t)b * (a.YC >> 2) + ((a.ycoff + ncol0) >> 2)) * plane + pix) * 4;
#pragma unroll
            for (int j = 0; j < TN; ++j)
#pragma unroll
                for (int g = 0; g < 4; ++g) {
                    floatx4 o;
#pragma unroll
                    for (int c = 0; c < 4; ++c) o[c] = lwg_act_c<EA>(acc[i][j][4 * g + c] + bias4[j][g][c], a.act);
                    *reinterpret_cast<floatx4*>(yq + (size_t)(8 * j + 2 * g) * plane * 4) = o;
                }
        } else {
            float* yr = a.y + opix * a.YC + a.ycoff + ncol0;
            const float* rr = EPI == LWG_EPI_RESIDUAL ? a.res + opix * a.YC + a.ycoff + ncol0 : nullptr;
#pragma unroll
            for (int j = 0; j < TN; ++j)
#pragma unroll
                for (int g = 0; g < 4; ++g) {
                    floatx4 o;
                    floatx4 rv = floatx4{0.f, 0.f, 0.f, 0.f};
                    if (EPI == LWG_EPI_RESIDUAL) rv = *reinterpret_cast<const floatx4*>(rr + 32 * j + 8 * g);
#pragma unroll
                    for (int c = 0; c < 4; ++c) {
                        const float v = acc[i][j][4 * g + c] + bias4[j][g][c];
                        o[c] = (EPI == LWG_EPI_RESIDUAL && lwg_act_is_mask<EA>(a.act)) ? (rv[c] > 0.f ? v : 0.f) : lwg_act_c<EA>(v + rv[c], a.act);
                    }
                    if (EPI == LWG_EPI_NONE && a.ydt == LWG_DT_BF16) {
                        typedef __bf16 lwg_bf16x4 __attribute__((ext_vector_type(4)));
                        lwg_bf16x4 ob;
#pragma unroll
                        for (int c = 0; c < 4; ++c) ob[c] = (__bf16)o[c];
                        *reinterpret_cast<lwg_bf16x4*>(reinterpret_cast<__bf16*>(a.y) + opix * a.YC + a.ycoff + ncol0 + 32 * j + 8 * g) = ob;
                    } else {
                        *reinterpret_cast<floatx4*>(yr + 32 * j + 8 * g) = o;
                    }
                }
        }
    }
}

template <int TM, int TN, int EPI>
__device__ __forceinline__ void lwg_conv_epilogue(const LwgConvArgs& a, floatx16 (&acc)[TM][TN], int m_base, int n_base,
                                                  int wm, int wn, int lane, int ooy_add = 0, int oox_add = 0) {
    if (a.act == LWG_ACT_RELU) lwg_conv_epilogue_a<TM, TN, EPI, LWG_ACT_RELU>(a, acc, m_base, n_base, wm, wn, lane, ooy_add, oox_add);
    else if (a.act == LWG_ACT_NONE) lwg_conv_epilogue_a<TM, TN, EPI, LWG_ACT_NONE>(a, acc, m_base, n_base, wm, wn, lane, ooy_add, oox_add);
    else if (EPI == LWG_EPI_RESIDUAL && a.act == LWG_ACT_RELU_MASK)
        lwg_conv_epilogue_a<TM, TN, EPI, LWG_ACT_RELU_MASK>(a, acc, m_base, n_base, wm, wn, lane, ooy_add, oox_add);
    else lwg_conv_epilogue_a<TM, TN, EPI, -1>(a, acc, m_base, n_base, wm, wn, lane, ooy_add, oox_add);
}

template <int TM, int TN>
__device__ __forceinline__ void lwg_conv_epilogue_slab(float* __restrict__ slab, int M, int N, floatx16 (&acc)[TM][TN], int m_base,
                                                       int n_base, int wm, int wn, int lane) {
    const int ncol0 = n_base + wn * TN * 32 + 4 * (lane >> 5);
#pragma unroll
    for (int i = 0; i < TM; ++i) {
        const int m = m_base + wm * TM * 32 + i * 32 + (lane & 31);
        if (m >= M) continue;
        float* yr = slab + (size_t)m * N + ncol0;
#pragma unroll
        for (int j = 0; j < TN; ++j)
#pragma unroll
            for (int g = 0; g < 4; ++g) {
                floatx4 o;
#pragma unroll
                for (int c = 0; c < 4; ++c) o[c] = acc[i][j][4 * g + c];
                *reinterpret_cast<floatx4*>(yr + 32 * j + 8 * g) = o;
            }
    }
}
```

ipercore_amd/csrc/lwg_conv_wino.h:

```cpp
#pragma once
#include <stddef.h>
#include "lwg_conv_args.h"

#ifdef __HIPCC__
#define CW_FN __host__ __device__ __forceinline__
#else
#define CW_FN static inline
#endif
#ifdef __HIP_DEVICE_COMPILE__
#define CW_UNIFORM(v) __builtin_amdgcn_readfirstlane(v)
#else
#define CW_UNIFORM(v) (v)
#endif
#define CW_OOB 0xC0000000u
#define CW_KS 8
#define CW_NB 64
struct CwGrid { int bx, by, tiles, total; };
CW_FN CwGrid cw_grid(int B, int H, int W, int N, int ex, int ey, int nbv) {
    const int bx = (W + ex - 1) / ex, by = (H + ey - 1) / ey, tiles = bx * by * B;
    return CwGrid{bx, by, tiles, tiles * (N / nbv)};
}
CW_FN long long cw_total_blocks(int B, int H, int W, int N, int ex, int ey, int nbv) {
    return (long long)((W + ex - 1) / ex) * ((H + ey - 1) / ey) * B * (N / nbv);
}
// ... 1 lines not shown
enum { CW_COLMAJOR = 0, CW_CHUNK = 1, CW_XCD = 2 };
struct CwOrder { int kind, nwg, wg, ncb, tiles, total, xg, xr; };

CW_FN int cw4_order_kind(int xcd_sw, int chunk_sw, bool sm, unsigned nwg, int ncb, int Cin, int N, int tiles, int total) {
    const bool xcd = xcd_sw && !sm && (nwg & 7u) == 0 && (ncb == 4 || ncb == 8 || (ncb == 2 && (Cin >= 192 || xcd_sw == 2))) && (int)nwg < total && tiles >= (int)nwg / ncb;
    return xcd ? CW_XCD : chunk_sw == 2 || (chunk_sw == 1 && 144u * (unsigned)Cin * (unsigned)N <= (5u << 20)) ? CW_CHUNK : CW_COLMAJOR;
}
CW_FN CwOrder cw_order(int kind, unsigned nwg, unsigned wg, int ncb, const CwGrid& g) {
    return CwOrder{kind, (int)nwg, (int)wg, ncb, g.tiles, g.total, (int)nwg / ncb, (int)(((wg & 7u) / (unsigned)ncb) * (nwg >> 3) + (wg >> 3))};
}
CW_FN bool cw_has_block(const CwOrder& o, int id) {
    return o.kind == CW_XCD ? (id / o.nwg) * o.xg + o.xr < o.tiles : id < o.total;
}
CW_FN void cw_block(const CwOrder& o, int id, int& cb, int& t) {
    if (o.kind == CW_XCD) {
        cb = (int)((unsigned)o.wg & 7u) & (o.ncb - 1);
        t = CW_UNIFORM((id / o.nwg) * o.xg + o.xr);
    } else if (o.kind == CW_CHUNK) {
        const int G = o.nwg, per = G * o.ncb;
        const int ch = CW_UNIFORM(id / per);
        const int r = id - ch * per, base = ch * G;
        const int nt = o.tiles - base < G ? o.tiles - base : G;
        cb = CW_UNIFORM(r / nt);
        t = CW_UNIFORM(base + r - cb * nt);
    } else {
        cb = CW_UNIFORM(id / o.tiles);
        t = CW_UNIFORM(id - cb * o.tiles);
    }
}
CW_FN int cw_image(const CwGrid& g, int t) { return t / (g.bx * g.by); }
CW_FN void cw_corner(const CwGrid& g, int t_in_image, int ex, int ey, int& x0, int& y0) { x0 = (t_in_image % g.bx) * ex, y0 = (t_in_image / g.bx) * ey; }
CW_FN int cw_n0(int cb, int nbv) { return cb * nbv; }
CW_FN int cw4_n0_spade_small(int cb) { return (cb >> 1) * 64 + (cb & 1) * 16; }
CW_FN int cw_halo_pixel(int i, int hw, int nel, int lgp, int x0, int y0, int H, int W) {
    const int pix = i >> lgp, hy = pix / hw, hx = pix - hy * hw;
    const int gy = y0 - 1 + hy, gx = x0 - 1 + hx;
    return i < nel && gy >= 0 && gy < H && gx >= 0 && gx < W ? gy * W + gx : -1;
}
CW_FN unsigned cw_halo_pixel_voff(int lin, int i, int lgp, int C, int ebytes) {
    return lin >= 0 ? (unsigned)(lin * C + (16 / ebytes) * (i & ((1 << lgp) - 1))) * (unsigned)ebytes : CW_OOB;
}
CW_FN unsigned cw_halo_voff(int i, int hw, int nel, int lgp, int x0, int y0, int H, int W, int C, int ebytes) {
    return cw_halo_pixel_voff(cw_halo_pixel(i, hw, nel, lgp, x0, y0, H, W), i, lgp, C, ebytes);
}
CW_FN bool cw_stage_second(int c, int C0, bool two) { return two && c >= C0; }
CW_FN unsigned cw_stage_soff(int c, int C0, bool two, int ebytes) { return (unsigned)(cw_stage_second(c, C0, two) ? c - C0 : c) * (unsigned)ebytes; }
CW_FN unsigned cw4_out_voff(int ox, int oy, int H, int W, int YC, int chan) {
    return ox < W && oy < H ? (unsigned)((oy * W + ox) * YC + chan) * 4u : CW_OOB;
}
CW_FN unsigned cw4_out_group(unsigned vo, int h, bool grouped) { return vo + (grouped ? 128u * (unsigned)h : 0u); }

#define CW_NO_OUT_BUFFER (-1ll)
CW_FN bool cw_contract_ok(const LwgConvArgs& a, unsigned long long pair_bytes, long long out_slack) {
    if (!a.x0 || !a.w || !a.y || a.M <= 0 || a.ntaps != 9 || a.stride != 1 || a.omul != 1 || a.C0 <= 0 || (a.C0 % CW_KS) != 0 || a.C1 < 0 ||
        (a.C1 % CW_KS) != 0 || ((a.C0 + a.C1) % (2 * CW_KS)) != 0 || (a.C1 > 0 && !a.x1) || a.N <= 0 || (a.N % CW_NB) != 0 || a.OH != a.H ||
        a.OW != a.W || a.YH != a.H || a.YW != a.W || a.xdt != LWG_DT_F32 || a.ydt != LWG_DT_F32 || (long long)a.M != (long long)a.B * a.H * a.W ||
        a.ycoff < 0 || (a.ycoff % 4) != 0 || (a.YC % 4) != 0 || (a.act == LWG_ACTIVATION_RELU_MASK && a.epi != LWG_EPI_RESIDUAL))
        return false;
    if (a.epi == LWG_EPI_SPADE) {
        if (!a.xn || !a.mean || !a.rstd || !a.bias || a.YC * 2 != a.N || a.ycoff != 0) return false;
    } else {
        if (a.ycoff + a.N > a.YC) return false;
        if (a.epi != LWG_EPI_NONE && (a.epi != LWG_EPI_RESIDUAL || !a.res)) return false;
    }
    const unsigned long long cmax = (unsigned long long)(a.C0 > a.C1 ? a.C0 : a.C1);
    if ((unsigned long long)a.H * a.W * cmax * 4ull >= (unsigned long long)CW_OOB || pair_bytes * (a.C0 + a.C1) * a.N >= 0xffffffffull) return false;
    if (out_slack >= 0 && (unsigned long long)a.H * a.W * a.YC * 4ull + (unsigned long long)out_slack >= (unsigned long long)CW_OOB) return false;
    return true;
}
CW_FN bool cwb_contract_ok(const LwgConvArgs& a) {
    if (!a.x0 || !a.w || !a.y || a.B <= 0 || a.H <= 0 || a.W <= 0 || a.C0 <= 0 || a.C1 < 0 || a.N <= 0 || a.xdt != LWG_DT_BF16 || a.ydt != LWG_DT_BF16 ||
        a.ntaps != 9 || a.stride != 1 || a.omul != 1 || a.ooy != 0 || a.oox != 0 || a.OH != a.H || a.OW != a.W || a.YH != a.H || a.YW != a.W ||
        (long long)a.M != (long long)a.B * a.H * a.W)
        return false;
    for (int t = 0; t < 9; ++t)
        if (a.dy[t] != t / 3 - 1 || a.dx[t] != t % 3 - 1) return false;
    const int Cin = a.C0 + a.C1;
    if (a.N % 64 != 0 || Cin % 64 != 0 || (a.YC & 7) != 0 || (a.ycoff & 7) != 0 || a.ycoff < 0 || (a.C1 != 0 && (a.C0 % 64 != 0 || !a.x1))) return false;
    if (a.act != LWG_ACTIVATION_NONE && a.act != LWG_ACTIVATION_RELU && a.act != LWG_ACTIVATION_TANH && a.act != LWG_ACTIVATION_SIGMOID) return false;
    if ((unsigned long long)a.H * a.W * (unsigned long long)(a.C0 > a.C1 ? a.C0 : a.C1) * 2ull >= (unsigned long long)CW_OOB ||
        32ull * (unsigned long long)Cin * (unsigned long long)a.N >= (unsigned long long)CW_OOB || cw_total_blocks(a.B, a.H, a.W, a.N, 16, 16, 64) >= 0x7fffffffll)
        return false;
    if (a.epi == LWG_EPI_SPADE) return a.xn && a.mean && a.rstd && a.bias && a.YC * 2 == a.N && a.ycoff == 0;
    return a.ycoff + a.N <= a.YC && (a.epi == LWG_EPI_NONE || (a.epi == LWG_EPI_RESIDUAL && a.res));
}

struct LwgWinoTaps { int t[9]; };
CW_FN bool cw_panel_args_ok(const float* wpanel, const float* upk, int Cin, int N, const int* tap9, LwgWinoTaps& taps) {
    if (!wpanel || !upk || !tap9 || Cin <= 0 || (Cin % 32) != 0 || N <= 0) return false;
    for (int i = 0; i < 9; ++i) {
        if (tap9[i] < 0 || tap9[i] > 8) return false;
        taps.t[i] = tap9[i];
    }
    return true;
}

#ifdef __HIPCC__
#include "lwg_common.h"

template <int V> struct IntC { static constexpr int value = V; };
template <int POLICY = 0>
__device__ __forceinline__ floatx4 cw_buf_load(__amdgpu_buffer_rsrc_t r, unsigned voff, unsigned soff) {
    return __builtin_bit_cast(floatx4, __builtin_amdgcn_raw_buffer_load_b128(r, (int)voff, (int)soff, POLICY));
}
__device__ __forceinline__ __amdgpu_buffer_rsrc_t cw_image_rsrc(const void* x, int b, int H, int W, int C, unsigned ebytes) {
    const unsigned img = (unsigned)(H * W);
    return __builtin_amdgcn_make_buffer_rsrc(const_cast<char*>(static_cast<const char*>(x)) + (size_t)b * img * C * ebytes, 0, (int)(img * (unsigned)C * ebytes), 0x00020000);
}

template <int NQ, bool TWO>
struct CwBlock {
    int b, x0, y0, n0;
    __amdgpu_buffer_rsrc_t rx0, rx1;
    unsigned voff0[NQ], voff1[NQ];

    __device__ __forceinline__ void locate(const LwgConvArgs& a, const CwGrid& g, int t, int ex, int ey, int n) {
        b = __builtin_amdgcn_readfirstlane(cw_image(g, t));
        cw_corner(g, t - b * g.bx * g.by, ex, ey, x0, y0);
        n0 = n;
        rx0 = cw_image_rsrc(a.x0, b, a.H, a.W, a.C0, 4u);
        if constexpr (TWO) rx1 = cw_image_rsrc(a.x1, b, a.H, a.W, a.C1, 4u);
    }
    __device__ __forceinline__ void halo(const LwgConvArgs& a, int tid, int nth, int hw, int nel) {
#pragma unroll
        for (int k = 0; k < NQ; ++k) {
            voff0[k] = cw_halo_voff(tid + nth * k, hw, nel, 1, x0, y0, a.H, a.W, a.C0, 4);
            if constexpr (TWO) voff1[k] = cw_halo_voff(tid + nth * k, hw, nel, 1, x0, y0, a.H, a.W, a.C1, 4);
        }
    }
    template <int POLICY = 0>
    __device__ __forceinline__ floatx4 rld1(const LwgConvArgs& a, int c, int k) const {
        if constexpr (!TWO) {
            return cw_buf_load<POLICY>(rx0, voff0[k], cw_stage_soff(c, a.C0, false, 4));
        } else {
            const bool second = cw_stage_second(c, a.C0, true);
            const __amdgpu_buffer_rsrc_t r = second ? rx1 : rx0;
            const unsigned v = second ? voff1[k] : voff0[k];
            return cw_buf_load<POLICY>(r, v, cw_stage_soff(c, a.C0, true, 4));
        }
    }
};
__device__ __forceinline__ void cw_rst1(float* dst, int plane, floatx4 v) {
#pragma unroll
    for (int k = 0; k < 4; ++k) dst[k * plane] = v[k];
}

template <void (*KERNEL)(const LwgConvArgs)>
static inline int cw_launch(dim3 grid, unsigned threads, size_t lds, hipStream_t stream, const LwgConvArgs& a) {
    static unsigned long long done = 0ull;
    if (hipError_t e = lwg_allow_dynamic_lds(reinterpret_cast<const void*>(KERNEL), lds, done); e != hipSuccess) return (int)e;
    hipLaunchKernelGGL(KERNEL, grid, dim3(threads), lds, stream, a);
    return (int)hipGetLastError();
}
static inline dim3 cw_persistent_grid(long long total, int cus) { return dim3((unsigned)(LWG_WINO_PERSIST && total > cus ? cus : total)); }
#endif
```

ipercore_amd/networks/generator.py:

```python
import math

import torch
import torch.nn as nn

from .. import ops
from . import packing
from .params import generator_param_shapes


class _Node(nn.Module):

    def __init__(self):
        super().__init__()


class ParamTree(nn.Module):
    def __init__(self, shapes):
        super().__init__()
        self._shapes = dict(shapes)
        for name, shape in shapes.items():
            parts = name.split(".")
            node = self
            for p in parts[:-1]:
                if not hasattr(node, p):
# ... 83 lines not shown
    i += 3
    for d in range(1, len(bgf)):
        layers.append(("conv", conv(f"bg_net.main.{i}", stride=2)))
        i += 3
    for _ in range(n_res):
        layers.append(("res", (conv(f"bg_net.main.{i}.main.0"), conv(f"bg_net.main.{i}.main.3"))))
        i += 1
    for d in range(len(bgf) - 1, 0, -1):
        layers.append(("convT", convT(f"bg_net.main.{i}")))
        i += 3
    layers.append(("out", conv(f"bg_net.main.{i}", stride=1, pad=3, n_pad=64)))
    return layers


def run_bg_layers(layers, bg4):
    scratch = _Scratch()
    x = bg4

    def norm(t, act, res=None):
        B, h, w, C = t.shape
        mean, rstd = t.new_empty(B, C), t.new_empty(B, C)
        nsplit = max(1, min(64, (h * w) // 64))
        ops.instnorm_stats(t, mean, rstd, scratch.get(B * C * nsplit * 3, t.device), eps=1e-5, nsplit=nsplit)
        return ops.instnorm_apply(t, mean, rstd, torch.empty_like(t), act=act, res=res)

    for kind, spec in layers:
        B, H, W, _ = x.shape
        if kind == "conv":
            y = ops.conv2d(x, spec, x.new_empty(B, H // spec.stride, W // spec.stride, spec.N))
            x = norm(y, ops.ACT_RELU)
        elif kind == "res":
            h = norm(ops.conv2d(x, spec[0], torch.empty_like(x)), ops.ACT_RELU)
            x = norm(ops.conv2d(h, spec[1], torch.empty_like(x)), ops.ACT_NONE, res=x)
        elif kind == "convT":
            y = x.new_empty(B, 2 * H, 2 * W, spec[0].N)
            x = norm(ops.conv_transpose2d(x, spec, y, act=ops.ACT_NONE), ops.ACT_RELU)
        else:
            y = ops.conv2d(x, spec, x.new_empty(B, H, W, spec.N), act=ops.ACT_TANH)
            return ops.nhwc_to_nchw(y, channels=3)


def _param_version(gen):
    return tuple((p.data_ptr(), p._version) for p in gen.parameters())


class SourceFeatures:

    def __init__(self, enc, res, kv, ns, batched=False):
        self.enc, self.res, self.kv, self.ns, self.batched = enc, res, kv, ns, batched


class AttentionLWBGenerator(nn.Module):
    has_bg = True
    lwb_kind = "att"

    def __init__(self, cfg, temporal=False):
        super().__init__()
        self._name = _get(cfg, "name", "AttLWB-SPADE")
        tsf = _get(cfg, "TSFNet")
        sid = _get(cfg, "SIDNet")
        self.num_filters = [int(c) for c in _get(tsf, "num_filters")]
        self.n_res_block = int(_get(tsf, "n_res_block"))
        if [int(c) for c in _get(sid, "num_filters")] != self.num_filters or int(_get(sid, "n_res_block")) != self.n_res_block:
            raise ValueError("SIDNet and TSFNet must share num_filters / n_res_block (the LWB sites pair them up)")
        for c in self.num_filters:
            if c not in (64, 128, 256):
                raise ValueError(f"num_filters entries must be in {{64,128,256}} for the HIP kernels, got {c}")
        self.cond_nc = int(_get(tsf, "cond_nc"))
        self.temporal = temporal
        self.bg_filters, bg_cond = None, 4
        if self.has_bg:
            bgc = _get(cfg, "BGNet")
            self.bg_filters = [int(c) for c in _get(bgc, "num_filters")]
            bg_cond = int(_get(bgc, "cond_nc"))
        shapes = generator_param_shapes(self.num_filters, self.n_res_block, self.bg_filters or (), cond_nc=self.cond_nc,
                                        bg_cond_nc=bg_cond, with_bg=self.has_bg,
                                        lwb={"att": "att", "add": "plain", "avg": "plain"}.get(self.lwb_kind, "softgate"))
        tree = ParamTree(shapes)
        for name, child in tree.named_children():
            self.add_module(name, child)
        self._packed = None
        self.conv_precision = "winograd"

    def packed(self):
        if self._packed is None or self._packed.version != _param_version(self):
            self._packed = _Packed(self)
        return self._packed

    def _check(self, *tensors):
        if torch.is_grad_enabled() and any(p.requires_grad for p in self.parameters()) and self.training:
            raise NotImplementedError("these methods are the no_grad inference engine: call under torch.no_grad() / .eval(), or train "
                                      "through ipercore_amd.networks.training.TrainableGenerator (trainers.LWGTrainer)")
        for t in tensors:
            if t is not None and not t.is_cuda:
                raise RuntimeError("ipercore_amd generator runs on the MI355X only: got a CPU tensor (no fallback)")

    @staticmethod
    def _check_square(t):
        if t.shape[-1] != t.shape[-2]:
            raise ValueError(f"square images only (got {t.shape[-2]} x {t.shape[-1]}): the reference's image_size is one number and the "
                             "attention blocks' flow fields are resized to square feature maps")

    @torch.no_grad()
    def _encode_sources_impl(self, src8, batched=False, ns=None):
        pk = self.packed()
        x = src8
        adt = self._act_dtype()
        enc, res = [], []
        for i, spec in enumerate(pk.src_enc):
            n, H, W, _ = x.shape
            y = x.new_empty(n, H // 2, W // 2, spec.N, dtype=adt)
            x = ops.conv2d(x, spec, y, act=ops.ACT_RELU)
            enc.append(x)
        for c0, c1 in pk.src_res:
            h = ops.conv2d(x, c0, torch.empty_like(x), act=ops.ACT_RELU)
            x = ops.conv2d(h, c1, torch.empty_like(x), epi=ops.EPI_RESIDUAL, res=x)
            res.append(x)
        return SourceFeatures(enc, res, self._project_sources(pk, enc, res), ns if ns is not None else src8.shape[0], batched)

    def _project_sources(self, pk, enc, res):
        kv = []
        for feats, sites in ((enc, pk.enc_sites), (res, pk.res_sites)):
            for f, st in zip(feats, sites):
                if self.lwb_kind == "att":
                    n, h, w, _ = f.shape
                    with ops.conv_precision("fp32" if self.conv_precision in ("bf16", "bf16_winograd") else self.conv_precision):
                        kap = ops.conv2d(f.float(), st["fkap"], f.new_empty(n, h, w, 64, dtype=torch.float32))[..., 0].contiguous()
                    kv.append((ops.conv2d(f, st["fkq"], torch.empty_like(f)), ops.conv2d(f, st["fv"], torch.empty_like(f)), kap))
                else:
                    kv.append((f, None, None))
        return kv

    def _attlwb(self, st, tsf_x, kv, Tst, batched, scratch):
        B, h, w, C = tsf_x.shape
        if self.lwb_kind != "att":
            ns = Tst.shape[1]
            Tst = scratch.flow(Tst, h, w)
            if self.lwb_kind == "add":
                return ops.lwb_fuse(tsf_x, kv[0], Tst, torch.empty_like(tsf_x), src_batched=batched)
            if self.lwb_kind == "avg":
                return ops.lwb_fuse(tsf_x, kv[0], Tst, torch.empty_like(tsf_x), scale_o=1.0 / (ns + 1), src_batched=batched)
            g = ops.conv2d(tsf_x, st["g0"], torch.empty_like(tsf_x), act=ops.ACT_RELU)
            g = ops.conv2d(g, st["g2"], torch.empty_like(tsf_x), act=ops.ACT_SIGMOID)
            return ops.lwb_fuse(tsf_x, kv[0], Tst, torch.empty_like(tsf_x), gate=g,
                                scale_w=1.0 if self.lwb_kind == "sg_add" else 1.0 / ns, src_batched=batched)
        mean = tsf_x.new_empty(B, C, dtype=torch.float32)
        rstd = tsf_x.new_empty(B, C, dtype=torch.float32)
        nrec = ops.attn_records(h, w, C, tsf_x.dtype)
        ws = scratch.get(ops.instnorm_finalize_ws(B, C, nrec), tsf_x.device)
        flow = scratch.flow(Tst, h, w)
        if tuple(flow.shape[2:4]) != (h, w):
            raise NotImplementedError("the attention block takes flows resized to its feature size: non-square feature maps are not built "
                                      "(image_size is one number throughout the reference)")
        att = ops.lwb_attention_x(tsf_x, kv[0], kv[2], kv[1], st["bv"], flow, torch.empty_like(tsf_x), stats=ws,
                                  src_batched=batched)
        ops.instnorm_finalize(ws, B, C, nrec, mean, rstd, eps=1e-5)
        actv = ops.conv2d(att, st["shared"], tsf_x.new_empty(B, h, w, st["shared"].N), act=ops.ACT_RELU)
        return ops.conv2d(actv, st["gb"], torch.empty_like(tsf_x), epi=ops.EPI_SPADE, xn=tsf_x, mean=mean, rstd=rstd)

    @staticmethod
    def _upconv(x, specs, act, q4=False):
        B, H, W, _ = x.shape
        if q4:
            return ops.conv_transpose2d(x, specs, x.new_empty(B, specs[0].N // 4, 2 * H, 2 * W, 4), act=act, q4=True)
        y = x.new_empty(B, 2 * H, 2 * W, specs[0].N)
        return ops.conv_transpose2d(x, specs, y, act=act)

    @torch.no_grad()
    def _run_tsf_impl(self, tsf8, feats, Tst, bg=None, want_pred=True, want_mask=True, want_img=False):
        pk = self.packed()
        scratch = _Scratch()
        n_down = len(pk.tsf_enc)
        x = tsf8
        adt = self._act_dtype()
        if adt != torch.float32 and self.lwb_kind != "att":
            raise NotImplementedError("bf16 activation storage is built for the attention LWB (AttLWB-SPADE) generators")
        if feats.kv[0][0].dtype != adt:
            raise RuntimeError(f"source features are {feats.kv[0][0].dtype} but the generator runs in {self.conv_precision} mode: "
                               "rebuild them (Imitator.set_source / forward_src) after changing conv_precision")
        enc = []
        site = 0
        for i, spec in enumerate(pk.tsf_enc):
            B, H, W, _ = x.shape
            x = ops.conv2d(x, spec, x.new_empty(B, H // 2, W // 2, spec.N, dtype=adt), act=ops.ACT_RELU)
            x = self._attlwb(pk.enc_sites[i], x, feats.kv[site], Tst, feats.batched, scratch)
            site += 1
            enc.append(x)
        for i, (c0, c1) in enumerate(pk.res):
            h = ops.conv2d(x, c0, torch.empty_like(x), act=ops.ACT_RELU)
            x = ops.conv2d(h, c1, torch.empty_like(x), epi=ops.EPI_RESIDUAL, res=x)
            x = self._attlwb(pk.res_sites[i], x, feats.kv[site], Tst, feats.batched, scratch)
            site += 1
        q4 = adt == torch.float32 and self.conv_precision in ("fp32", "winograd", "winograd2x2")
        for i in range(n_down):
            if i == n_down - 1 and pk.head16 is not None and ops.up4_head_eligible(x, pk.upconvs[i], ops.ACT_RELU):
                return ops.up4_head_compose_bf16(x, pk.upconvs[i], pk.head16, bg, want_pred=want_pred and bg is not None, want_mask=want_mask,
                                                 want_img=want_img)
            x = self._upconv(x, pk.upconvs[i], ops.ACT_RELU, q4=q4 and i == n_down - 1)
            if i != n_down - 1:
                skip = enc[n_down - 2 - i]
                sp = pk.skippers[i]
                x = ops.conv2d(skip, sp, x.new_empty(x.shape[0], x.shape[1], x.shape[2], sp.N), x1=x, act=ops.ACT_RELU)
        head = pk.head
        if x.dtype == torch.bfloat16:
            if pk.head16 is not None:
                head = pk.head16
            else:
                x = x.float()
        return ops.head_compose(x, head, bg, want_pred=want_pred and bg is not None, want_mask=want_mask, want_img=want_img, q4=q4)

    def _act_dtype(self):
        return torch.bfloat16 if self.conv_precision in ("bf16", "bf16_winograd") else torch.float32

    @torch.no_grad()
    def _run_bg_impl(self, bg4):
        return run_bg_layers(self.packed().bg, bg4)

    @torch.no_grad()
    def _run_src_decode_impl(self, x):
        pk = self.packed()
        for specs in pk.src_dec:
            x = self._upconv(x, specs, ops.ACT_RELU)
        _, mask, img = ops.head_compose(x.float(), pk.src_head, None, want_pred=False, want_mask=True, want_img=True)
        return img, mask

    def encode_sources(self, *a, **k):
        with ops.conv_precision(self.conv_precision):
            return self._encode_sources_impl(*a, **k)

    def run_tsf(self, *a, **k):
        with ops.conv_precision(self.conv_precision):
            return self._run_tsf_impl(*a, **k)

    def run_bg(self, *a, **k):
        with ops.conv_precision("fp32" if self.conv_precision in ("bf16", "bf16_winograd") else self.conv_precision):
            return self._run_bg_impl(*a, **k)

    def run_src_decode(self, *a, **k):
        with ops.conv_precision(self.conv_precision):
            return self._run_src_decode_impl(*a, **k)

    @torch.no_grad()
    def forward_bg(self, bg_inputs):
        if not self.has_bg:
            raise AttributeError("this generator has no background network")
        self._check(bg_inputs)
        bs, ns, c, h, w = bg_inputs.shape
        x = ops.nchw_to_nhwc(bg_inputs.reshape(bs * ns, c, h, w).contiguous().float(), c_pad=4)
        return self.run_bg(x).view(bs, ns, 3, h, w)

    @torch.no_grad()
    def forward_src(self, src_inputs, only_enc=True):
        self._check(src_inputs)
        self._check_square(src_inputs)
        bs, ns, c, h, w = src_inputs.shape
        src8 = ops.nchw_to_nhwc(src_inputs.reshape(bs * ns, c, h, w).contiguous().float(), c_pad=8)
        feats = self.encode_sources(src8, batched=bs > 1, ns=ns)
        enc = _FeatList(ops.nhwc_to_nchw(t.float()) for t in feats.enc)
        res = _FeatList(ops.nhwc_to_nchw(t.float()) for t in feats.res)
        enc.lwg_cache = res.lwg_cache = feats
        if only_enc:
            return enc, res
        img, mask = self.run_src_decode(feats.res[-1])
        return enc, res, img.view(bs, ns, 3, h, w), mask.view(bs, ns, 1, h, w)

    def _features_from_api(self, src_enc_outs, src_res_outs, bs):
        cache = getattr(src_enc_outs, "lwg_cache", None)
        if cache is not None and getattr(src_res_outs, "lwg_cache", None) is cache:
            return cache
        pk = self.packed()
        adt = self._act_dtype()
        enc = [ops.nchw_to_nhwc(t.contiguous().float()).to(adt) for t in src_enc_outs]
        res = [ops.nchw_to_nhwc(t.contiguous().float()).to(adt) for t in src_res_outs]
        n = enc[0].shape[0]
        return SourceFeatures(enc, res, self._project_sources(pk, enc, res), n // bs, batched=bs > 1)

    @torch.no_grad()
    def forward_tsf(self, tsf_inputs, src_enc_outs, src_res_outs, Tst, temp_enc_outs=None, temp_res_outs=None, Ttt=None):
        self._check(tsf_inputs, Tst)
        self._check_square(tsf_inputs)
        bs = tsf_inputs.shape[0]
        feats = self._features_from_api(src_enc_outs, src_res_outs, bs)
        T = Tst.contiguous().float()
        if temp_enc_outs is not None and Ttt is not None and self.lwb_kind == "att":
            if bs != 1:
                raise NotImplementedError("temporal attention runs one clip per process (bs = 1), as Imitator.inference does")
            tfe = self._features_from_api(temp_enc_outs, temp_res_outs, bs)
            feats = SourceFeatures(feats.enc, feats.res, [tuple(torch.cat([a, ta], dim=0) for a, ta in zip(site, tsite))
                                                          for site, tsite in zip(feats.kv, tfe.kv)],
                                   feats.ns + Ttt.shape[1], batched=False)
            T = torch.cat([T, Ttt.contiguous().float()], dim=1).contiguous()
        tsf8 = ops.nchw_to_nhwc(tsf_inputs.contiguous().float(), c_pad=8)
        _, mask, img = self.run_tsf(tsf8, feats, T, bg=None, want_pred=False, want_mask=True, want_img=True)
        return img, mask

    @torch.no_grad()
    def _forward_streams(self, src_inputs, tsf_inputs, Tst, only_tsf):
        bs, nt = Tst.shape[0], Tst.shape[1]
        if only_tsf:
            enc, res = self.forward_src(src_inputs, only_enc=True)
            src_imgs = src_masks = None
        else:
            enc, res, src_imgs, src_masks = self.forward_src(src_inputs, only_enc=False)
        imgs, masks = [], []
        for t in range(nt):
            if t != 0 and self.temporal:
                raise NotImplementedError("multi-step temporal training forward (Ttt inside forward()) is not built; "
                                          "temporal INFERENCE goes through Imitator(temporal=True) / forward_tsf(temp_*)")
            img, mask = self.forward_tsf(tsf_inputs[:, t], enc, res, Tst[:, t].contiguous())
# ... 204 lines not shown
```

ipercore_amd/ops.py:

```python
import ctypes

import torch

from . import _lib
from ._lib import ACT_LRELU, ACT_NONE, ACT_RELU, ACT_RELU_MASK, ACT_SIGMOID, ACT_TANH, EPI_NONE, EPI_RESIDUAL, EPI_SPADE

EYE_DIST = 2.7320508075688776


def _ptr(t, dtype=torch.float32):
    if t is None:
        return None
    if not t.is_cuda:
        raise RuntimeError("ipercore_amd ops need CUDA (HIP) tensors: the MI355X path has no CPU fallback")
    if t.dtype != dtype:
        raise TypeError(f"expected {dtype}, got {t.dtype}")
    if not t.is_contiguous():
        raise ValueError("tensor must be contiguous")
    return t.data_ptr()


CONV_PRECISION = "fp32"


# ... 223 lines not shown
    units32 = blocks.value * (nbv.value // 32)
    return slices.value * a.M * spec.N if units32 >= WINO_MIN_GRID else None


def _wwino(spec):
    if spec._wwino is None or spec._wwino.device != spec.w.device:
        K4, N, _ = spec.w.shape
        cin, nt = spec.Cin, spec.ntaps
        assert nt == 9 and cin % 32 == 0 and K4 * 4 == nt * cin, (cin, nt, K4)
        if not spec.w.is_cuda:
            raise RuntimeError("ipercore_amd ops need CUDA (HIP) tensors: the MI355X path has no CPU fallback")
        tap9 = (ctypes.c_int * 9)()
        for t in range(nt):
            tap9[3 * (spec.dy[t] + 1) + spec.dx[t] + 1] = t
        if PANEL_CACHE is not None:
            U = PANEL_CACHE.winograd(spec, list(tap9))
            if U is not None:
                spec._wwino = U
                return U
        U = torch.empty(16, cin // 8, 2, N, 4, device=spec.w.device, dtype=torch.float32)
        _lib.check(_lib.lib().lwg_winograd_panel_f32(_ptr(spec.w), _ptr(U), cin, N, tap9, _stream()), "lwg_winograd_panel_f32")
        spec._wwino = U
    return spec._wwino


WINO4 = True
WINO4_MIN_CIN = 64


def _wino4_use(spec, splitk):
    return WINO4 and not splitk and spec.Cin >= WINO4_MIN_CIN


def _wwino4(spec):
    if spec._wwino4 is None or spec._wwino4.device != spec.w.device:
        K4, N, _ = spec.w.shape
        cin, nt = spec.Cin, spec.ntaps
        assert nt == 9 and cin % 32 == 0 and K4 * 4 == nt * cin, (cin, nt, K4)
        if not spec.w.is_cuda:
            raise RuntimeError("ipercore_amd ops need CUDA (HIP) tensors: the MI355X path has no CPU fallback")
        tap9 = (ctypes.c_int * 9)()
        for t in range(nt):
            tap9[3 * (spec.dy[t] + 1) + spec.dx[t] + 1] = t
        U = torch.empty(4, cin // 8, 4, 2, 9 * N, device=spec.w.device, dtype=torch.float32)
        _lib.check(_lib.lib().lwg_winograd4_panel_f32(_ptr(spec.w), _ptr(U), cin, N, tap9, _stream()), "lwg_winograd4_panel_f32")
        spec._wwino4 = U
    return spec._wwino4


def conv_args(x0, spec, y, x1=None, epi=EPI_NONE, act=ACT_NONE, res=None, xn=None, mean=None, rstd=None,
              out_hw=None, ycoff=0, q4=False):
    B, H, W, C0 = x0.shape
    C1 = 0 if x1 is None else x1.shape[3]
    assert C0 + C1 == spec.Cin, (C0, C1, spec.Cin)
    if q4:
        YB, YCq, YH, YW, four = y.shape
        assert four == 4 and y.dtype == torch.float32 and x0.dtype == torch.float32 and epi == EPI_NONE and y.is_contiguous()
        YC = 4 * YCq
    else:
        YB, YH, YW, YC = y.shape
    if out_hw is None:
        OH, OW = (YH, YW) if spec.omul == 1 else (YH // spec.omul, YW // spec.omul)
    else:
        OH, OW = out_hw
    a = _lib.LwgConvArgs()
    xdt, ydt = x0.dtype, y.dtype
    a.xdt = _lib.DT_BF16 if xdt == torch.bfloat16 else _lib.DT_F32
    a.ydt = _lib.DT_F32_Q4 if q4 else (_lib.DT_BF16 if ydt == torch.bfloat16 else _lib.DT_F32)
    a.x0, a.x1 = _ptr(x0, xdt), _ptr(x1, xdt)
    a.C0, a.C1 = C0, C1
    a.B, a.H, a.W = B, H, W
    a.OH, a.OW, a.M = OH, OW, B * OH * OW
    a.stride, a.ntaps, a.cshift = spec.stride, spec.ntaps, spec.cshift
    a.w, a.N, a.bias = _ptr(spec.w), spec.N, _ptr(spec.bias)
    a.y, a.YH, a.YW, a.YC, a.ycoff = _ptr(y, ydt), YH, YW, YC, ycoff
    a.omul, a.ooy, a.oox = spec.omul, spec.ooy, spec.oox
    a.epi, a.act = epi, act
    a.res, a.xn, a.mean, a.rstd = _ptr(res, ydt), _ptr(xn, ydt), _ptr(mean), _ptr(rstd)
    for i in range(spec.ntaps):
        a.dy[i] = spec.dy[i]
        a.dx[i] = spec.dx[i]
    return a


def _hook_end(a, spec, epi, kind, slices=True, extra=0):
    n = (max(1, int(_lib.lib().lwg_conv_slice_count(a))) if slices else 1) + extra
    CONV_HOOK(False, a.M, spec, epi, {"kernels": n, "kind": kind})


def conv2d(x0, spec, y, x1=None, epi=EPI_NONE, act=ACT_NONE, res=None, xn=None, mean=None, rstd=None,
           out_hw=None, ycoff=0, splitk=False, q4=False):
    a = conv_args(x0, spec, y, x1, epi, act, res, xn, mean, rstd, out_hw, ycoff, q4)
    if q4 and (splitk or CONV_PRECISION not in ("fp32", "winograd") or x0.dtype != torch.float32):
        raise ValueError("channel-quad-plane outputs: fp32 activations on the fp32 MFMA path, no split-K")
    if CONV_HOOK is not None:
        CONV_HOOK(True, a.M, spec, epi, None)
    kind, sliced, extra = "direct", True, 0
    if x0.dtype == torch.bfloat16:
        kind = "bf16"
        if y.dtype != torch.bfloat16 or spec.Cin % 64 != 0:
            raise ValueError("bf16 convolutions need bf16 outputs and Cin % 64 == 0")
        if CONV_PRECISION == "bf16_winograd" and _bf16_wino_eligible(spec, x0, y, x1, epi, act, out_hw, ycoff):
            kind, sliced = "bf16_winograd", False
            panel, bias = _wwino16(spec, epi == EPI_SPADE)
            a.w, a.bias = _ptr(panel, torch.bfloat16), _ptr(bias)
            for i, (dy, dx) in enumerate(_WINO_TAPS):
                a.dy[i], a.dx[i] = dy, dx
            _lib.check(_lib.lib().lwg_conv2d_winograd_bf16(a, _stream()), "lwg_conv2d_winograd_bf16")
        elif _hr_eligible(spec, x0, y, out_hw) or _pw_eligible(spec, x0, y, x1, epi, out_hw):
            panel, bias = _w16hr(spec, epi == EPI_SPADE)
            a.w, a.bias = _ptr(panel, torch.bfloat16), _ptr(bias)
            for i, t in enumerate(_hr_tap_order(spec)):
                a.dy[i], a.dx[i] = spec.dy[t], spec.dx[t]
            _lib.check(_lib.lib().lwg_conv2d_nhwc_bf16_hr(a, _stream()), "lwg_conv2d_nhwc_bf16_hr")
        else:
            a.w = _ptr(_w16v2(spec), torch.bfloat16)
            _lib.check(_lib.lib().lwg_conv2d_nhwc_bf16(a, _stream()), "lwg_conv2d_nhwc_bf16")
    elif y.dtype == torch.bfloat16:
        if BF16_C8 and spec.Cin == 8 and spec.N == 64 and spec.ntaps <= 10 and x1 is None and epi == EPI_NONE and spec.omul == 1:
            a.w = _ptr(_w16c8(spec), torch.bfloat16)
            _lib.check(_lib.lib().lwg_conv2d_nhwc_c8_bf16(a, _stream()), "lwg_conv2d_nhwc_c8_bf16")
        else:
            _lib.check(_lib.lib().lwg_conv2d_nhwc_f32(a, _stream()), "lwg_conv2d_nhwc_f32")
    elif CONV_PRECISION == "winograd" and _wino_eligible(spec, x0, y, x1, epi, act, out_hw, q4, ycoff) and \
            (nws := _wino_plan(a, spec, y, splitk)) is not None:
        kind, sliced = "winograd", False
        if _wino4_use(spec, splitk):
            a.w = _ptr(_wwino4(spec))
            kind = "winograd4"
            _lib.check(_lib.lib().lwg_conv2d_winograd4_f32(a, _stream()), "lwg_conv2d_winograd4_f32")
        elif nws:
            a.w = _ptr(_wwino(spec))
            ws, extra = torch.empty(nws, device=x0.device, dtype=torch.float32), 1
            _lib.check(_lib.lib().lwg_conv2d_winograd_f32_ws(a, _ptr(ws), _stream()), "lwg_conv2d_winograd_f32_ws")
        else:
            a.w = _ptr(_wwino(spec))
            _lib.check(_lib.lib().lwg_conv2d_winograd_f32(a, _stream()), "lwg_conv2d_winograd_f32")
    elif CONV_PRECISION == "split" and spec.Cin % 32 == 0:
        a.w = _ptr(_w16x3(spec), torch.bfloat16)
        kind = "split"
        _lib.check(_lib.lib().lwg_conv2d_nhwc_f32_split(a, _stream()), "lwg_conv2d_nhwc_f32_split")
    else:
        nws = _lib.lib().lwg_conv2d_ws_floats(a) if splitk else 0
        if nws:
            ws = torch.empty(nws, device=x0.device, dtype=torch.float32)
            _lib.check(_lib.lib().lwg_conv2d_nhwc_f32_ws(a, _ptr(ws), _stream()), "lwg_conv2d_nhwc_f32_ws")
        else:
            _lib.check(_lib.lib().lwg_conv2d_nhwc_f32(a, _stream()), "lwg_conv2d_nhwc_f32")
    if CONV_HOOK is not None:
        _hook_end(a, spec, epi, kind, sliced, extra)
    return y


WINO_UP4 = True
F32_UP4 = True
BF16_UP4 = True


def _parity_specs_ok(specs):
    s0 = specs[0]
    return (len(specs) == 4 and all(s.ntaps == 4 and s.omul == 2 and s.stride == 1 and (s.ooy, s.oox) == (i >> 1, i & 1) and s.N == s0.N and s.Cin == s0.Cin
                                    and [(dy - (i >> 1), dx - (i & 1)) for dy, dx in zip(s.dy, s.dx)] == list(zip(s0.dy, s0.dx)) for i, s in enumerate(specs)))


def _wwino_t(specs):
    s0 = specs[0]
    U = s0._wwino_t
    if U is not None and U.device == s0.w.device:
        return U
    Cin, N = s0.Cin, s0.N
    G = torch.tensor([[1.0, 0.0], [1.0, 1.0], [0.0, 1.0]], dtype=torch.float64, device=s0.w.device)
    parts = []
    for par, sp in enumerate(specs):
        py, px = par >> 1, par & 1
        W = sp.w.double().permute(0, 2, 1).reshape(4 * Cin, N)
        W = W.view(Cin // 32, 4, 32, N).permute(1, 0, 2, 3).reshape(4, Cin, N)
        g = torch.zeros(2, 2, Cin, N, dtype=torch.float64, device=W.device)
        for t, (dy, dx) in enumerate(zip(sp.dy, sp.dx)):
            g[dy - (py - 1), dx - (px - 1)] = W[t]
        u = torch.einsum("ar,rqcn,bq->abcn", G, g, G)
        if py:
            u[0] = -u[0]
        if px:
            u[:, 0] = -u[:, 0]
        parts.append(u.reshape(9, Cin, N))
    U9 = torch.stack(parts).float()
    U = torch.cat([U9[:, 0:4].permute(0, 2, 3, 1).reshape(4, Cin, 4 * N), U9[:, 4:8].permute(0, 2, 3, 1).reshape(4, Cin, 4 * N), U9[:, 8]], dim=2)
    U = U.view(4, Cin // 8, 4, 2, 9 * N).contiguous()
    s0._wwino_t = U
    return U


_G_X24 = ((1.0, 0.0), (0.5, 0.5), (-1.0 / 6.0, 1.0 / 6.0), (-8.0 / 3.0, -4.0 / 3.0), (0.0, 0.5))


def _wwino_t24(specs):
    s0 = specs[0]
    U = s0._wwino_t24
    if U is not None and U.device == s0.w.device:
        return U
    Cin, N = s0.Cin, s0.N
    Gy = torch.tensor([[1.0, 0.0], [1.0, 1.0], [0.0, 1.0]], dtype=torch.float64, device=s0.w.device)
    Gx = torch.tensor(_G_X24, dtype=torch.float64, device=s0.w.device)
    parts = []
    for par, sp in enumerate(specs):
        py, px = par >> 1, par & 1
        W = sp.w.double().permute(0, 2, 1).reshape(4 * Cin, N)
        W = W.view(Cin // 32, 4, 32, N).permute(1, 0, 2, 3).reshape(4, Cin, N)
        g = torch.zeros(2, 2, Cin, N, dtype=torch.float64, device=W.device)
        for t, (dy, dx) in enumerate(zip(sp.dy, sp.dx)):
            g[dy - (py - 1), dx - (px - 1)] = W[t]
        u = torch.einsum("ar,rqcn,bq->abcn", Gy, g, Gx)
        if py:
            u[0] = -u[0]
        parts.append(torch.cat([u[:, :3].reshape(9, Cin, N), u[:, 3:].reshape(6, Cin, N)]))
    U15 = torch.stack(parts).float()
    quad = lambda lo, hi: U15[:, lo:hi].permute(0, 2, 3, 1).reshape(4, Cin, (hi - lo) * N)
    U = torch.cat([quad(0, 4), quad(4, 8), U15[:, 8], quad(9, 13), U15[:, 13], U15[:, 14]], dim=2)
    U = U.view(4, Cin // 8, 4, 2, 15 * N).contiguous()
    s0._wwino_t24 = U
    return U


WINO_UP4_24 = True
WINO_UP4_24_MIN_HW = 64 * 64


def _up4_24(x):
    return WINO_UP4_24 and x.shape[1] * x.shape[2] >= WINO_UP4_24_MIN_HW


class _FusedTransposeSpec(object):

    def __init__(self, s0, panel):
        self.N, self.Cin, self.ntaps, self.stride, self.omul = 4 * s0.N, s0.Cin, 16, 1, 2
        self.algo_kn, self.w = 4 * s0.algo_kn, panel


def conv_transpose2d(x, specs, y, act=ACT_NONE, splitk=False, out_hw=None, q4=False):
    s0 = specs[0]
    if (BF16_UP4 and BF16_HR and x.dtype == torch.bfloat16 and y.dtype == torch.bfloat16 and len(specs) == 4 and s0.Cin in (64, 128)
            and s0.N % 64 == 0 and all(s.ntaps == 4 and s.omul == 2 and (s.ooy, s.oox) == (i >> 1, i & 1) for i, s in enumerate(specs))):
        a = conv_args(x, s0, y, act=act)
        panel = getattr(s0, "_w16up", None)
        if panel is None or panel.device != s0.w.device:
            panel = torch.stack([_w16hr(s, False)[0] for s in specs]).contiguous()
            s0._w16up = panel
        a.w = _ptr(panel, torch.bfloat16)
        if CONV_HOOK is not None:
            whole = _FusedTransposeSpec(s0, panel)
            CONV_HOOK(True, a.M, whole, EPI_NONE, None)
        _lib.check(_lib.lib().lwg_conv_transpose4_nhwc_bf16(a, _stream()), "lwg_conv_transpose4_nhwc_bf16")
        if CONV_HOOK is not None:
            _hook_end(a, whole, EPI_NONE, "up4")
        return y
    if (WINO_UP4 and CONV_PRECISION == "winograd" and not splitk and out_hw is None and x.is_cuda and x.dtype == torch.float32 and y.dtype == torch.float32
            and s0.Cin % 32 == 0 and s0.N % 32 == 0 and _parity_specs_ok(specs)):
        a = conv_args(x, s0, y, act=act, q4=q4)
        f24 = _up4_24(x)
        panel = _wwino_t24(specs) if f24 else _wwino_t(specs)
        a.w = _ptr(panel)
        if CONV_HOOK is not None:
            whole = _FusedTransposeSpec(s0, panel)
            CONV_HOOK(True, a.M, whole, EPI_NONE, None)
        if f24:
            _lib.check(_lib.lib().lwg_conv_transpose4_winograd24_f32(a, _stream()), "lwg_conv_transpose4_winograd24_f32")
        else:
            _lib.check(_lib.lib().lwg_conv_transpose4_winograd_f32(a, _stream()), "lwg_conv_transpose4_winograd_f32")
        if CONV_HOOK is not None:
            _hook_end(a, whole, EPI_NONE, "winograd_up4", False)
        return y
    if (F32_UP4 and x.is_cuda and x.dtype == torch.float32 and y.dtype == torch.float32 and CONV_PRECISION in ("fp32", "winograd") and s0.Cin % 32 == 0
            and _parity_specs_ok(specs)):
        a = conv_args(x, s0, y, act=act, q4=q4)
        if _lib.lib().lwg_conv_transpose4_is_one_grid(a):
            panel = getattr(s0, "_w32up", None)
            if panel is None or panel.device != s0.w.device:
                panel = torch.stack([s.w.reshape(-1) for s in specs]).contiguous()
                s0._w32up = panel
            a.w = _ptr(panel)
            if CONV_HOOK is not None:
                whole = _FusedTransposeSpec(s0, panel)
                CONV_HOOK(True, a.M, whole, EPI_NONE, None)
            _lib.check(_lib.lib().lwg_conv_transpose4_nhwc_f32(a, _stream()), "lwg_conv_transpose4_nhwc_f32")
            if CONV_HOOK is not None:
                _hook_end(a, whole, EPI_NONE, "up4")
            return y
    for s in specs:
        conv2d(x, s, y, act=act, splitk=splitk, out_hw=None if out_hw is None else out_hw(s), q4=q4)
    return y


def instnorm_stats(x, mean, rstd, ws, eps=1e-5, nsplit=None):
    B, H, W, C = x.shape
    HW = H * W
    if nsplit is None:
        nsplit = max(1, min(64, HW // 64))
    assert ws.numel() >= B * C * nsplit * 3
    if x.dtype == torch.bfloat16:
        _lib.check(_lib.lib().lwg_instnorm_stats_nhwc_bf16(_ptr(x, torch.bfloat16), B, HW, C, eps, _ptr(mean), _ptr(rstd), _ptr(ws), nsplit,
                                                            _stream()), "lwg_instnorm_stats_nhwc_bf16")
        return
    _lib.check(_lib.lib().lwg_instnorm_stats_nhwc_f32(_ptr(x), B, HW, C, eps, _ptr(mean), _ptr(rstd), _ptr(ws), nsplit,
                                                       _stream()), "lwg_instnorm_stats_nhwc_f32")


def instnorm_apply(x, mean, rstd, y, act=ACT_NONE, res=None):
    B, H, W, C = x.shape
    _lib.check(_lib.lib().lwg_instnorm_apply_nhwc_f32(_ptr(x), _ptr(mean), _ptr(rstd), _ptr(res), _ptr(y), B, H * W, C, act,
                                                       _stream()), "lwg_instnorm_apply_nhwc_f32")
    return y


def flow_resize(T, h, w):
    B, ns, S = T.shape[0], T.shape[1], T.shape[2]
    T = T.contiguous()
    out = torch.empty(B, ns, h, w, 2, device=T.device, dtype=torch.float32)
    _lib.check(_lib.lib().lwg_flow_resize_f32(_ptr(T), B * ns, S, h, w, _ptr(out), _stream()), "lwg_flow_resize_f32")
    return out


def lwb_attention(q, Ks, Vs, bk, bv, T, out, src_batched=False):
    B, h, w, C = q.shape
    ns = T.shape[1]
    S = T.shape[2]
    assert T.shape[0] == B and Ks.shape[0] == (B * ns if src_batched else ns) and tuple(Ks.shape[1:]) == (h, w, C)
    if q.dtype == torch.bfloat16:
        bf = torch.bfloat16
        _lib.check(_lib.lib().lwg_lwb_attention_bf16(_ptr(q, bf), _ptr(Ks, bf), _ptr(Vs, bf), _ptr(bk), _ptr(bv), _ptr(T), _ptr(out, bf), B, ns, h,
                                                      w, C, S, 1 if src_batched else 0, _stream()), "lwg_lwb_attention_bf16")
        return out
    _lib.check(_lib.lib().lwg_lwb_attention_f32(_ptr(q), _ptr(Ks), _ptr(Vs), _ptr(bk), _ptr(bv), _ptr(T), _ptr(out), B, ns, h,
                                                 w, C, S, 1 if src_batched else 0, _stream()), "lwg_lwb_attention_f32")
    return out


def attn_records(h, w, C, dtype=torch.float32):
    n = _lib.lib().lwg_lwb_attention_x_records(int(h), int(w), int(C), 2 if dtype == torch.bfloat16 else 4)
    if n <= 0:
        raise ValueError(f"lwb_attention_x: unsupported (h, w, C, dtype) = {(h, w, C, dtype)}")
    return n


def lwb_attention_x(x, Kq, kappa, Vs, bv, T, out, stats=None, src_batched=False):
    B, h, w, C = x.shape
    ns = T.shape[1]
    nsrc = B * ns if src_batched else ns
    assert tuple(T.shape) == (B, ns, h, w, 2), (tuple(T.shape), (B, ns, h, w, 2))
    assert tuple(Kq.shape) == (nsrc, h, w, C) and tuple(Vs.shape) == (nsrc, h, w, C) and tuple(kappa.shape) == (nsrc, h, w)
    assert Kq.dtype == x.dtype and Vs.dtype == x.dtype and out.dtype == x.dtype and kappa.dtype == torch.float32
    assert stats is None or stats.numel() >= B * attn_records(h, w, C, x.dtype) * C * 3
    if x.dtype == torch.bfloat16:
        bf = torch.bfloat16
        _lib.check(_lib.lib().lwg_lwb_attention_x_bf16(_ptr(x, bf), _ptr(Kq, bf), _ptr(kappa), _ptr(Vs, bf), _ptr(bv), _ptr(T), _ptr(out, bf),
                                                        _ptr(stats), B, ns, h, w, C, 1 if src_batched else 0, _stream()), "lwg_lwb_attention_x_bf16")
        return out
    _lib.check(_lib.lib().lwg_lwb_attention_x_f32(_ptr(x), _ptr(Kq), _ptr(kappa), _ptr(Vs), _ptr(bv), _ptr(T), _ptr(out), _ptr(stats), B, ns, h, w,
                                                   C, 1 if src_batched else 0, _stream()), "lwg_lwb_attention_x_f32")
    return out


def instnorm_finalize_ws(B, C, nrec):
    return int(_lib.lib().lwg_instnorm_finalize_ws_floats(int(B), int(C), int(nrec)))


def instnorm_finalize(ws, B, C, nrec, mean, rstd, eps=1e-5):
    assert ws.numel() >= instnorm_finalize_ws(B, C, nrec)
    _lib.check(_lib.lib().lwg_instnorm_finalize_f32(_ptr(ws), B, C, nrec, float(eps), _ptr(mean), _ptr(rstd), _stream()), "lwg_instnorm_finalize_f32")


def lwb_fuse(tsf_x, src_x, T, out, gate=None, scale_w=1.0, scale_o=1.0, src_batched=False):
    B, h, w, C = tsf_x.shape
    ns, S = T.shape[1], T.shape[2]
    assert T.shape[0] == B and src_x.shape[0] == (B * ns if src_batched else ns) and tuple(src_x.shape[1:]) == (h, w, C)
    _lib.check(_lib.lib().lwg_lwb_fuse_f32(_ptr(tsf_x), _ptr(src_x), _ptr(gate), _ptr(T), _ptr(out), B, ns, h, w, C, S,
                                           1 if src_batched else 0, float(scale_w), float(scale_o), _stream()), "lwg_lwb_fuse_f32")
    return out


def lwb_attention_bwd(q, Ks, Vs, bk, bv, T, dout, src_batched=False):
    B, h, w, C = q.shape
    ns, S = T.shape[1], T.shape[2]
    dout = dout.contiguous()
    dq = torch.empty_like(q)
    dKs = torch.zeros_like(Ks)
    dVs = torch.zeros_like(Vs)
    _lib.check(_lib.lib().lwg_lwb_attention_bwd_f32(_ptr(q), _ptr(Ks), _ptr(Vs), _ptr(bk), _ptr(bv), _ptr(T), _ptr(dout), _ptr(dq),
                                                     _ptr(dKs), _ptr(dVs), B, ns, h, w, C, S, 1 if src_batched else 0, _stream()),
               "lwg_lwb_attention_bwd_f32")
    return dq, dKs, dVs


def lwb_attention_kv(q, kv, bk, bv, T, out, src_batched=False):
    B, h, w, C = q.shape
    ns, S = T.shape[1], T.shape[2]
    assert T.shape[0] == B and kv.shape[0] == (B * ns if src_batched else ns) and tuple(kv.shape[1:]) == (h, w, 2 * C)
    _lib.check(_lib.lib().lwg_lwb_attention_kv_f32(_ptr(q), _ptr(kv), _ptr(bk), _ptr(bv), _ptr(T), _ptr(out), B, ns, h, w, C, S,
                                                    1 if src_batched else 0, _stream()), "lwg_lwb_attention_kv_f32")
    return out


def lwb_attention_kv_bwd(q, kv, bk, bv, T, dout, src_batched=False):
    B, h, w, C = q.shape
    ns, S = T.shape[1], T.shape[2]
    dout = dout.contiguous()
    dq = torch.empty_like(q)
    dkv = torch.zeros_like(kv)
    _lib.check(_lib.lib().lwg_lwb_attention_kv_bwd_f32(_ptr(q), _ptr(kv), _ptr(bk), _ptr(bv), _ptr(T), _ptr(dout), _ptr(dq), _ptr(dkv),
                                                        B, ns, h, w, C, S, 1 if src_batched else 0, _stream()), "lwg_lwb_attention_kv_bwd_f32")
    return dq, dkv


def project_faces(verts, cam, faces, want_faces_v=True, want_f2pts=True):
    B, nv, _ = verts.shape
    nf = faces.shape[0]
    fv = torch.empty(B, nf, 3, 3, device=verts.device, dtype=torch.float32) if want_faces_v else None
    f2 = torch.empty(B, nf, 3, 2, device=verts.device, dtype=torch.float32) if want_f2pts else None
    cam = cam.contiguous()
    _lib.check(_lib.lib().lwg_project_faces_f32(_ptr(verts), _ptr(cam), _ptr(faces, torch.int32), B, nv, nf, EYE_DIST, _ptr(fv),
                                                 _ptr(f2), _stream()), "lwg_project_faces_f32")
    return fv, f2


def rasterize_fim_wim(faces_v, image_size, near=0.1, far=100.0):
    B, nf = faces_v.shape[0], faces_v.shape[1]
    S = int(image_size)
    dev = faces_v.device
    fim = torch.empty(B, S, S, device=dev, dtype=torch.int32)
    wim = torch.empty(B, S, S, 3, device=dev, dtype=torch.float32)
    ws = torch.empty(_lib.lib().lwg_rasterize_ws_bytes(B, nf, S), device=dev, dtype=torch.uint8)
    _lib.check(_lib.lib().lwg_rasterize_fim_wim_f32(_ptr(faces_v), B, nf, S, near, far, _ptr(fim, torch.int32), _ptr(wim),
                                                     ws.data_ptr(), _stream()), "lwg_rasterize_fim_wim_f32")
    return fim, wim


def texture_sample(fim, wim, faces_v, textures, eps=1e-3, background_color=(0.0, 0.0, 0.0)):
    B, S = fim.shape[0], fim.shape[1]
    nf, T = faces_v.shape[1], textures.shape[2]
    assert textures.shape[0] in (1, B) and textures.shape[1] == nf
    rgb = torch.empty(B, S, S, 3, device=fim.device, dtype=torch.float32)
    bg = (ctypes.c_float * 3)(*[float(c) for c in background_color])
    _lib.check(_lib.lib().lwg_texture_sample_f32(_ptr(fim, torch.int32), _ptr(wim), _ptr(faces_v.contiguous()), _ptr(textures.contiguous()), B, nf,
                                                 S, T, 1 if textures.shape[0] == B and B > 1 else (1 if textures.shape[0] == B else 0),
                                                 float(eps), bg, _ptr(rgb), _stream()), "lwg_texture_sample_f32")
    return rgb


def flow_compose(fim, wim, map_fn, f_uvs2img, uv_img4, src_f2pts, want_cond=False, want_tuv=False):
    B, S, _ = fim.shape
    nf = f_uvs2img.shape[0]
    ns = src_f2pts.shape[0]
    dev = fim.device
    tsf = torch.empty(B, S, S, 8, device=dev, dtype=torch.float32)
    Tst = torch.empty(B, ns, S, S, 2, device=dev, dtype=torch.float32)
    cond = torch.empty(B, 3, S, S, device=dev, dtype=torch.float32) if want_cond else None
    tuv = torch.empty(B, S, S, 2, device=dev, dtype=torch.float32) if want_tuv else None
    Hu, Wu = uv_img4.shape[0], uv_img4.shape[1]
    _lib.check(_lib.lib().lwg_flow_compose_f32(_ptr(fim, torch.int32), _ptr(wim), B, S, _ptr(map_fn), nf, _ptr(f_uvs2img),
                                                _ptr(uv_img4), Hu, Wu, _ptr(src_f2pts), ns, _ptr(tsf), _ptr(Tst), _ptr(cond),
                                                _ptr(tuv), _stream()), "lwg_flow_compose_f32")
    return tsf, Tst, cond, tuv


def bc_transform(f2pts, fim, wim):
    B, S, _ = fim.shape
    nf = f2pts.shape[1]
    T = torch.empty(B, S, S, 2, device=fim.device, dtype=torch.float32)
    _lib.check(_lib.lib().lwg_bc_transform_f32(_ptr(f2pts), _ptr(fim, torch.int32), _ptr(wim), B, S, nf, _ptr(T), _stream()),
               "lwg_bc_transform_f32")
    return T


def encode_fim(fim, map_fn):
    B, S, _ = fim.shape
    D = map_fn.shape[1]
    out = torch.empty(B, D, S, S, device=fim.device, dtype=torch.float32)
    _lib.check(_lib.lib().lwg_encode_fim_f32(_ptr(fim, torch.int32), _ptr(map_fn), B, S, map_fn.shape[0] - 1, D, _ptr(out),
                                              _stream()), "lwg_encode_fim_f32")
    return out


def head_compose(x, wpk, bg, want_pred=True, want_mask=True, want_img=False, q4=False):
    if q4:
        B, Cq, S, _, four = x.shape
        C = 4 * Cq
        assert four == 4 and x.dtype == torch.float32 and x.is_contiguous()
    else:
        B, S, _, C = x.shape
    dev = x.device
    pred = torch.empty(B, 3, S, S, device=dev, dtype=torch.float32) if want_pred else None
    mask = torch.empty(B, 1, S, S, device=dev, dtype=torch.float32) if want_mask else None
    img = torch.empty(B, 3, S, S, device=dev, dtype=torch.float32) if want_img else None
    bstride = 0
    if bg is not None and bg.shape[0] != 1:
        assert bg.shape[0] == B
        bstride = 3 * S * S
    if x.dtype == torch.bfloat16:
        _lib.check(_lib.lib().lwg_head_compose_bf16(_ptr(x, torch.bfloat16), _ptr(wpk, torch.bfloat16), _ptr(bg), bstride, B, S, C, _ptr(pred),
                                                     _ptr(mask), _ptr(img), _stream()), "lwg_head_compose_bf16")
        return pred, mask, img
    if q4:
        _lib.check(_lib.lib().lwg_head_compose_q4_f32(_ptr(x), _ptr(wpk), _ptr(bg), bstride, B, S, C, _ptr(pred), _ptr(mask), _ptr(img),
                                                       _stream()), "lwg_head_compose_q4_f32")
        return pred, mask, img
    _lib.check(_lib.lib().lwg_head_compose_f32(_ptr(x), _ptr(wpk), _ptr(bg), bstride, B, S, C, _ptr(pred), _ptr(mask), _ptr(img),
                                                _stream()), "lwg_head_compose_f32")
    return pred, mask, img

# ... 521 lines not shown
```

Before: 1217 frames/s.

## Skip SPADE convs on tiles where LWB attention has no source taps

The attention kernel now writes per-8x8-tile activity flags. These are compacted into active and inactive tile lists at the SPADE tile size. Both SPADE Winograd convs then run only over active tiles through a new tile-list kernel variant. Inactive tiles, whose attention output is just the bias, are filled from a precomputed canonical conv result of a constant-bias frame. This removes conv work on empty regions, at the cost of extra list-building, fill kernels, a canonical conv computed every call, and reliance on the inactive-tile output being exactly constant, including the halo of tiles that border active ones.

```diff
diff --git a/include/lwg_hip.h b/include/lwg_hip.h
--- a/include/lwg_hip.h
+++ b/include/lwg_hip.h
@@ -67,6 +67,7 @@
 } LwgWinoDesc;
 int lwg_winograd_panels_f32(const LwgWinoDesc* descs_dev, int ndesc, int total_blocks, lwg_stream_t stream);
 int lwg_conv2d_winograd4_f32(const LwgConvArgs* args, lwg_stream_t stream);
+int lwg_conv2d_winograd4_tiles_f32(const LwgConvArgs* args, const int* tile_ids, const int* tile_off, lwg_stream_t stream);
 int lwg_winograd4_panel_f32(const float* wpanel, float* upk, int Cin, int N, const int* tap9, lwg_stream_t stream);
 int lwg_conv2d_nhwc_bf16_hr(const LwgConvArgs* args, lwg_stream_t stream);
 int lwg_conv2d_winograd_bf16(const LwgConvArgs* args, lwg_stream_t stream);
@@ -135,6 +136,14 @@
                             float* out, float* stats, int B, int ns, int h, int w, int C, int src_batched, lwg_stream_t stream);
 int lwg_lwb_attention_x_bf16(const void* x, const void* Kq, const float* kappa, const void* Vs, const float* bv, const float* T,
                              void* out, float* stats, int B, int ns, int h, int w, int C, int src_batched, lwg_stream_t stream);
+int lwg_lwb_attention_x_flags_f32(const float* x, const float* Kq, const float* kappa, const float* Vs, const float* bv, const float* T,
+                                  float* out, float* stats, unsigned char* flags, int B, int ns, int h, int w, int C, int src_batched,
+                                  lwg_stream_t stream);
+int lwg_spade_tile_lists(const unsigned char* flags, int B, int fh, int fw, int ty, int tx, int* work, int* ids_active, int* ids_inactive,
+                         int* off_active, int* off_inactive, lwg_stream_t stream);
+int lwg_spade_fill_tiles_f32(const float* canon, float* y, int B, int H, int W, int C, const int* tile_ids, const int* tile_off, lwg_stream_t stream);
+int lwg_spade_const_tiles_f32(const float* gb_canon, const float* xn, const float* mean, const float* rstd, float* y, int B, int H, int W, int C,
+                              const int* tile_ids, const int* tile_off, lwg_stream_t stream);
 size_t lwg_instnorm_finalize_ws_floats(int B, int C, int nrec);
 int lwg_instnorm_finalize_f32(float* ws, int B, int C, int nrec, float eps, float* mean, float* rstd, lwg_stream_t stream);
 int lwg_lwb_attention_bwd_f32(const float* q, const float* Ks, const float* Vs, const float* bk, const float* bv,
diff --git a/ipercore_amd/_lib.py b/ipercore_amd/_lib.py
--- a/ipercore_amd/_lib.py
+++ b/ipercore_amd/_lib.py
@@ -57,6 +57,7 @@
     "lwg_winograd_panel_f32": (c_i, [c_f, c_f, c_i, c_i, ctypes.POINTER(c_i), c_f]),
     "lwg_winograd_panels_f32": (c_i, [c_f, c_i, c_i, c_f]),
     "lwg_conv2d_winograd4_f32": (c_i, [ctypes.POINTER(LwgConvArgs), c_f]),
+    "lwg_conv2d_winograd4_tiles_f32": (c_i, [ctypes.POINTER(LwgConvArgs), c_f, c_f, c_f]),
     "lwg_winograd4_panel_f32": (c_i, [c_f, c_f, c_i, c_i, ctypes.POINTER(c_i), c_f]),
     "lwg_conv2d_nhwc_bf16_hr": (c_i, [ctypes.POINTER(LwgConvArgs), c_f]),
     "lwg_conv2d_winograd_bf16": (c_i, [ctypes.POINTER(LwgConvArgs), c_f]),
@@ -98,6 +99,10 @@
     "lwg_flow_resize_f32": (c_i, [c_f, c_i, c_i, c_i, c_i, c_f, c_f]),
     "lwg_lwb_fuse_f32": (c_i, [c_f] * 5 + [c_i] * 7 + [ctypes.c_float, ctypes.c_float, c_f]),
     "lwg_lwb_attention_x_f32": (c_i, [c_f] * 8 + [c_i] * 6 + [c_f]),
+    "lwg_lwb_attention_x_flags_f32": (c_i, [c_f] * 9 + [c_i] * 6 + [c_f]),
+    "lwg_spade_tile_lists": (c_i, [c_f] + [c_i] * 5 + [c_f] * 6),
+    "lwg_spade_fill_tiles_f32": (c_i, [c_f] * 2 + [c_i] * 4 + [c_f] * 3),
+    "lwg_spade_const_tiles_f32": (c_i, [c_f] * 5 + [c_i] * 4 + [c_f] * 3),
     "lwg_lwb_attention_x_bf16": (c_i, [c_f] * 8 + [c_i] * 6 + [c_f]),
     "lwg_lwb_attention_x_records": (c_i, [c_i, c_i, c_i, c_i]),
     "lwg_instnorm_finalize_ws_floats": (ctypes.c_size_t, [c_i, c_i, c_i]),
diff --git a/ipercore_amd/csrc/conv_winograd4.hip b/ipercore_amd/csrc/conv_winograd4.hip
--- a/ipercore_amd/csrc/conv_winograd4.hip
+++ b/ipercore_amd/csrc/conv_winograd4.hip
@@ -1,6 +1,8 @@
+#ifndef W4_PASS2
 #include <hip/hip_runtime.h>
 #include "lwg_common.h"
 #include "lwg_conv_wino.h"
+#include "lwg_conv_epilogue.h"
 
 #define W4_THREADS 512
 #define W4_PBX 8
@@ -70,8 +72,16 @@
     v[5] = __builtin_fmaf(-5.f, r[3], __builtin_fmaf(4.f, r[1], r[5]));
 }
 
+#define W4_LIST 0
+#endif
+
 template <int EPI, bool TWO, bool SM = false>
+#if W4_LIST
+__global__ __launch_bounds__(SM ? 256 : W4_THREADS, 1) void lwg_conv_winograd4_tiles_kernel(const LwgConvArgs a, const int* __restrict__ tile_ids,
+                                                                                            const int* __restrict__ tile_cnt) {
+#else
 __global__ __launch_bounds__(SM ? 256 : W4_THREADS, 1) void lwg_conv_winograd4_kernel(const LwgConvArgs a) {
+#endif
     constexpr bool SMS = SM && EPI == LWG_EPI_SPADE;
     constexpr int NVP = SM && !SMS ? 2 : 1;
     constexpr int NTH = SM ? 256 : W4_THREADS;
@@ -87,9 +97,19 @@
     float* const raw0 = smem;
     float* const Ms = smem;
     const int tid = threadIdx.x, lane = tid & 63;
+#if W4_LIST
+    const CwGrid gd = cw_grid(a.B, H, W, N, 4 * W4_PBX, 4 * W4_PBY, NBV);
+    const int ntl = __builtin_amdgcn_readfirstlane(*tile_cnt);
+    const int ntc = ntl < 0 ? 0 : ntl > gd.tiles ? gd.tiles : ntl;
+    const CwGrid g = CwGrid{gd.bx, gd.by, ntc, ntc * (N / NBV)};
+#else
     const CwGrid g = cw_grid(a.B, H, W, N, 4 * W4_PBX, 4 * W4_PBY, NBV);
+#endif
     const CwOrder o = cw_order(cw4_order_kind(LWG_W4_XCD, LWG_W4_CHUNK, SM, gridDim.x, N / NBV, Cin, N, g.tiles, g.total), gridDim.x, blockIdx.x, N / NBV, g);
     int blk = blockIdx.x;
+#if W4_LIST
+    if (!cw_has_block(o, blk)) return;
+#endif
     const int nst = Cin / W4_KS;
     const __amdgpu_buffer_rsrc_t ru = __builtin_amdgcn_make_buffer_rsrc(const_cast<float*>(a.w), 0, (int)(144u * (unsigned)Cin * (unsigned)N), 0x00020000);
     const int q = wid & 3, ct = SM ? 0 : wid >> 2;
@@ -100,6 +120,12 @@
     auto setup = [&](int id) {
         int cb, t;
         cw_block(o, id, cb, t);
+#if W4_LIST
+        {
+            const int lt = __builtin_amdgcn_readfirstlane(tile_ids[t]);
+            t = lt < 0 ? 0 : lt >= gd.tiles ? gd.tiles - 1 : lt;
+        }
+#endif
         bk.locate(a, g, t, 4 * W4_PBX, 4 * W4_PBY, SMS ? cw4_n0_spade_small(cb) : cw_n0(cb, NBV));
         int tids = tid;
         asm volatile("" : "+v"(tids));
@@ -532,7 +558,7 @@
 #pragma unroll
                 for (int i = 0; i < 4; ++i)
 #pragma unroll
-                    for (int c = 0; c < 4; ++c) o[i][c] = (ext[0][i][c] - mu[c]) * rs[c] * (1.f + gam[i][c]) + o[i][c];
+                    for (int c = 0; c < 4; ++c) o[i][c] = lwg_spade_modulate(ext[0][i][c], mu[c], rs[c], gam[i][c], o[i][c]);
             } else if (EPI == LWG_EPI_RESIDUAL) {
                 if (a.act == LWG_ACT_RELU_MASK) {
 #pragma unroll
@@ -570,6 +596,13 @@
     if (tid == 0) reinterpret_cast<unsigned long long*>(const_cast<float*>(a.res))[(size_t)blockIdx.x * 16 + 13] = (unsigned long long)lab_bi;
 #endif
 }
+
+#ifndef W4_PASS2
+#define W4_PASS2
+#undef W4_LIST
+#define W4_LIST 1
+#include "conv_winograd4.hip"
+#undef W4_LIST
 
 
 __global__ __launch_bounds__(256) void lwg_winograd4_panel_kernel(const float* __restrict__ wp, float* __restrict__ U, int Cin, int N, LwgWinoTaps taps) {
@@ -633,3 +666,27 @@
     if (a.epi == LWG_EPI_RESIDUAL) return sm ? lwg_wino4_go<LWG_EPI_RESIDUAL, true>(a, grid, lds, stream) : lwg_wino4_go<LWG_EPI_RESIDUAL, false>(a, grid, lds, stream);
     return sm ? lwg_wino4_go<LWG_EPI_NONE, true>(a, grid, lds, stream) : lwg_wino4_go<LWG_EPI_NONE, false>(a, grid, lds, stream);
 }
+
+template <int EPI, bool SM>
+static int lwg_wino4_tiles_go(const LwgConvArgs& a, const int* ids, const int* cnt, dim3 grid, size_t lds, hipStream_t stream) {
+    return a.C1 > 0 ? cw_launch_tiles<lwg_conv_winograd4_tiles_kernel<EPI, true, SM>>(grid, SM ? 256 : W4_THREADS, lds, stream, a, ids, cnt)
+                    : cw_launch_tiles<lwg_conv_winograd4_tiles_kernel<EPI, false, SM>>(grid, SM ? 256 : W4_THREADS, lds, stream, a, ids, cnt);
+}
+
+extern "C" int lwg_conv2d_winograd4_tiles_f32(const LwgConvArgs* pa, const int* tile_ids, const int* tile_off, lwg_stream_t stream_) {
+    hipStream_t stream = reinterpret_cast<hipStream_t>(stream_);
+    if (!pa || !tile_ids || !tile_off || !cw_contract_ok(*pa, 144ull, 256ll)) return (int)hipErrorInvalidValue;
+    const LwgConvArgs& a = *pa;
+    const size_t lds = (size_t)(W4_BIAS_OFF + 64) * 4;
+    const int cus = lwg_device_cus();
+    long long total = cw_total_blocks(a.B, a.H, a.W, a.N, 4 * W4_PBX, 4 * W4_PBY, W4_NB);
+    if (total >= 0x3fffffffll) return (int)hipErrorInvalidValue;
+    const bool sm = LWG_W4_SMALL && 2 * total <= cus;
+    if (sm) total *= 2;
+    const dim3 grid = cw_persistent_grid(total, cus);
+    const int* cnt = tile_off + a.B;
+    if (a.epi == LWG_EPI_SPADE) return sm ? lwg_wino4_tiles_go<LWG_EPI_SPADE, true>(a, tile_ids, cnt, grid, lds, stream) : lwg_wino4_tiles_go<LWG_EPI_SPADE, false>(a, tile_ids, cnt, grid, lds, stream);
+    if (a.epi == LWG_EPI_RESIDUAL) return sm ? lwg_wino4_tiles_go<LWG_EPI_RESIDUAL, true>(a, tile_ids, cnt, grid, lds, stream) : lwg_wino4_tiles_go<LWG_EPI_RESIDUAL, false>(a, tile_ids, cnt, grid, lds, stream);
+    return sm ? lwg_wino4_tiles_go<LWG_EPI_NONE, true>(a, tile_ids, cnt, grid, lds, stream) : lwg_wino4_tiles_go<LWG_EPI_NONE, false>(a, tile_ids, cnt, grid, lds, stream);
+}
+#endif
diff --git a/ipercore_amd/csrc/lwb_attn_x.hip b/ipercore_amd/csrc/lwb_attn_x.hip
--- a/ipercore_amd/csrc/lwb_attn_x.hip
+++ b/ipercore_amd/csrc/lwb_attn_x.hip
@@ -43,12 +43,16 @@
     }
 };
 
-template <typename ST, int LPP, bool STATS, int NSU, int PW, int OCC, bool PIPE = false>
+__device__ __forceinline__ unsigned char* lwg_attnx_flags() { return nullptr; }
+__device__ __forceinline__ unsigned char* lwg_attnx_flags(unsigned char* f) { return f; }
+template <typename ST, int LPP, bool STATS, int NSU, int PW, int OCC, bool PIPE = false, typename... FL>
 __global__ __launch_bounds__(256 * PW, PW == 1 ? OCC : 1) void lwg_lwb_attnx_kernel(const ST* __restrict__ x, const ST* __restrict__ Kq,
                                                                  const float* __restrict__ kappa, const ST* __restrict__ Vs,
                                                                  const float* __restrict__ bv, const float* __restrict__ T,
                                                                  ST* __restrict__ out, float* __restrict__ stats, int B, int ns, int h, int w,
-                                                                 int src_batched) {
+                                                                 int src_batched, FL... flags_arg) {
+    constexpr bool FLAGS = sizeof...(FL) > 0;
+    unsigned char* const flags = lwg_attnx_flags(flags_arg...);
     using TR = AttnXTraits<ST>;
     constexpr int CPL = TR::CPL;
     constexpr int C = CPL * LPP;
@@ -197,7 +201,11 @@
                 mine |= live && tx0 >= -1 && tx0 < w && ty0 >= -1 && ty0 < h;
             }
         }
-        if (__syncthreads_or(mine ? 1 : 0) == 0) {
+        const int tile_any = __syncthreads_or(mine ? 1 : 0);
+        if constexpr (FLAGS) {
+            if (threadIdx.x == 0) flags[(size_t)b * (tiles_x * ((h + 7) >> 3)) + tile] = tile_any ? 1 : 0;
+        }
+        if (tile_any == 0) {
 #pragma unroll 1
             for (int it = 0; it < NIT; ++it) {
                 int yc, xc;
@@ -277,6 +285,7 @@
             }
         }
     } else {
+    bool mine = false;
 #pragma unroll 1
     for (int it = 0; it < NIT; ++it) {
         const int pass = it * PW + pl;
@@ -297,6 +306,7 @@
             int tx0, ty0;
             taps_of(t, wt, tx0, ty0);
             const bool any_tap = live && tx0 >= -1 && tx0 < w && ty0 >= -1 && ty0 < h;
+            if constexpr (FLAGS) mine |= any_tap;
             float ka[CPL], va[CPL], kap = 0.f;
 #pragma unroll
             for (int k = 0; k < CPL; ++k) ka[k] = va[k] = 0.f;
@@ -338,6 +348,10 @@
             for (int s = 0; s < ns; ++s) source(s, Tl[s * 64 + ptile]);
         }
         if (live) finish(gp, lrun, o);
+    }
+    if constexpr (FLAGS) {
+        const int tile_any = __syncthreads_or(mine ? 1 : 0);
+        if (threadIdx.x == 0) flags[(size_t)b * (tiles_x * ((h + 7) >> 3)) + tile] = tile_any ? 1 : 0;
     }
     }
 
@@ -428,7 +442,7 @@
 
 template <typename ST>
 static int lwg_attnx_launch(const ST* x, const ST* Kq, const float* kappa, const ST* Vs, const float* bv, const float* T, ST* out, float* stats,
-                            int B, int ns, int h, int w, int C, int src_batched, hipStream_t stream) {
+                            int B, int ns, int h, int w, int C, int src_batched, hipStream_t stream, unsigned char* flags = nullptr) {
     if (!x || !Kq || !kappa || !Vs || !bv || !T || !out || B <= 0 || ns <= 0 || ns > 64 || h <= 0 || w <= 0) return (int)hipErrorInvalidValue;
     const unsigned long long nsrc = (unsigned long long)(src_batched ? B * ns : ns);
     if (nsrc * (unsigned long long)h * w * (unsigned long long)C * sizeof(ST) >= 0xC0000000ull) return (int)hipErrorInvalidValue;
@@ -441,14 +455,30 @@
     {                                                                                                                                \
              \
         constexpr bool pipe = LWG_ATTNX_PIPE && CPL == 4 && (LPP) == 64 && (NSU) == 2 && (PW) == 1;                                  \
-        auto kern = lwg_lwb_attnx_kernel<ST, LPP, ST_, NSU, PW, (pipe ? 2 : CPL == 4 ? LWG_ATTNX_OCC : LWG_ATTNX_OCC16), pipe>;        \
+        constexpr int occ = pipe ? 2 : CPL == 4 ? LWG_ATTNX_OCC : LWG_ATTNX_OCC16;                                                   \
         const size_t lds = (size_t)((LPP) / 4) * 4096 + (size_t)ns * 512;                         \
-        static unsigned long long lds_ok = 0;                                                                                        \
-        if (lds > 65536) {                                                                                                           \
-            const hipError_t e = lwg_allow_dynamic_lds(reinterpret_cast<const void*>(kern), lds, lds_ok);                            \
-            if (e != hipSuccess) return (int)e;                                                                                      \
+        bool launched = false;                                                                                                       \
+        if constexpr (CPL == 4) {                                                                                                    \
+            if (flags) {                                                  \
+                auto kernf = lwg_lwb_attnx_kernel<ST, LPP, ST_, NSU, PW, occ, pipe, unsigned char*>;                                 \
+                static unsigned long long lds_okf = 0;                                                                               \
+                if (lds > 65536) {                                                                                                   \
+                    const hipError_t e = lwg_allow_dynamic_lds(reinterpret_cast<const void*>(kernf), lds, lds_okf);                  \
+                    if (e != hipSuccess) return (int)e;                                                                              \
+                }                                                                                                                    \
+                hipLaunchKernelGGL(kernf, grid, dim3(256 * PW), lds, stream, x, Kq, kappa, Vs, bv, T, out, stats, B, ns, h, w, src_batched, flags); \
+                launched = true;                                                                                                     \
+            }                                                                                                                        \
         }                                                                                                                            \
-        hipLaunchKernelGGL(kern, grid, dim3(256 * PW), lds, stream, x, Kq, kappa, Vs, bv, T, out, stats, B, ns, h, w, src_batched);   \
+        if (!launched) {                                                                                                             \
+            auto kern = lwg_lwb_attnx_kernel<ST, LPP, ST_, NSU, PW, occ, pipe>;                                                      \
+            static unsigned long long lds_ok = 0;                                                                                    \
+            if (lds > 65536) {                                                                                                       \
+                const hipError_t e = lwg_allow_dynamic_lds(reinterpret_cast<const void*>(kern), lds, lds_ok);                        \
+                if (e != hipSuccess) return (int)e;                                                                                  \
+            }                                                                                                                        \
+            hipLaunchKernelGGL(kern, grid, dim3(256 * PW), lds, stream, x, Kq, kappa, Vs, bv, T, out, stats, B, ns, h, w, src_batched); \
+        }                                                                                                                            \
     }
 #define LWG_ATTNX_PW(LPP, ST_, NSU)                                                                                                  \
     {                                                                                                                                \
@@ -475,10 +505,15 @@
     return (int)hipGetLastError();
 }
 
+extern "C" int lwg_lwb_attention_x_flags_f32(const float* x, const float* Kq, const float* kappa, const float* Vs, const float* bv, const float* T,
+                                             float* out, float* stats, unsigned char* flags, int B, int ns, int h, int w, int C, int src_batched,
+                                             lwg_stream_t stream_) {
+    if (C != 32 && C != 64 && C != 128 && C != 256) return (int)hipErrorInvalidValue;
+    return lwg_attnx_launch<float>(x, Kq, kappa, Vs, bv, T, out, stats, B, ns, h, w, C, src_batched, reinterpret_cast<hipStream_t>(stream_), flags);
+}
 extern "C" int lwg_lwb_attention_x_f32(const float* x, const float* Kq, const float* kappa, const float* Vs, const float* bv, const float* T,
                                        float* out, float* stats, int B, int ns, int h, int w, int C, int src_batched, lwg_stream_t stream_) {
-    if (C != 32 && C != 64 && C != 128 && C != 256) return (int)hipErrorInvalidValue;
-    return lwg_attnx_launch<float>(x, Kq, kappa, Vs, bv, T, out, stats, B, ns, h, w, C, src_batched, reinterpret_cast<hipStream_t>(stream_));
+    return lwg_lwb_attention_x_flags_f32(x, Kq, kappa, Vs, bv, T, out, stats, nullptr, B, ns, h, w, C, src_batched, stream_);
 }
 
 extern "C" int lwg_lwb_attention_x_bf16(const void* x, const void* Kq, const float* kappa, const void* Vs, const float* bv, const float* T,
diff --git a/ipercore_amd/csrc/lwg_conv_epilogue.h b/ipercore_amd/csrc/lwg_conv_epilogue.h
--- a/ipercore_amd/csrc/lwg_conv_epilogue.h
+++ b/ipercore_amd/csrc/lwg_conv_epilogue.h
@@ -1,6 +1,10 @@
 #pragma once
 #include "lwg_common.h"
 #include "lwg_conv_args.h"
+
+__device__ __forceinline__ float lwg_spade_modulate(float x, float mu, float rs, float gamma, float beta) {
+    return __builtin_fmaf((x - mu) * rs, 1.f + gamma, beta);
+}
 
 template <int TM, int TN, int EPI, int EA>
 __device__ __forceinline__ void lwg_conv_epilogue_a(const LwgConvArgs& a, floatx16 (&acc)[TM][TN], int m_base, int n_base,
diff --git a/ipercore_amd/csrc/lwg_conv_wino.h b/ipercore_amd/csrc/lwg_conv_wino.h
--- a/ipercore_amd/csrc/lwg_conv_wino.h
+++ b/ipercore_amd/csrc/lwg_conv_wino.h
@@ -177,5 +177,12 @@
     hipLaunchKernelGGL(KERNEL, grid, dim3(threads), lds, stream, a);
     return (int)hipGetLastError();
 }
+template <void (*KERNEL)(const LwgConvArgs, const int*, const int*)>
+static inline int cw_launch_tiles(dim3 grid, unsigned threads, size_t lds, hipStream_t stream, const LwgConvArgs& a, const int* ids, const int* cnt) {
+    static unsigned long long done = 0ull;
+    if (hipError_t e = lwg_allow_dynamic_lds(reinterpret_cast<const void*>(KERNEL), lds, done); e != hipSuccess) return (int)e;
+    hipLaunchKernelGGL(KERNEL, grid, dim3(threads), lds, stream, a, ids, cnt);
+    return (int)hipGetLastError();
+}
 static inline dim3 cw_persistent_grid(long long total, int cus) { return dim3((unsigned)(LWG_WINO_PERSIST && total > cus ? cus : total)); }
 #endif
diff --git a/ipercore_amd/csrc/spade_tiles.hip b/ipercore_amd/csrc/spade_tiles.hip
--- /dev/null
+++ b/ipercore_amd/csrc/spade_tiles.hip
@@ -0,0 +1,160 @@
+#include <hip/hip_runtime.h>
+#include "lwg_common.h"
+#include "lwg_conv_args.h"
+#include "lwg_conv_epilogue.h"
+
+#define ST_TW 32
+#define ST_TH 16
+#define ST_CW (3 * ST_TW)
+#define ST_CH (3 * ST_TH)
+
+__device__ __forceinline__ bool st_active(const unsigned char* __restrict__ fb, int fh, int fw, int tyi, int txi) {
+    const int r0 = max(2 * tyi - 1, 0), r1 = min(2 * tyi + 2, fh - 1), c0 = max(4 * txi - 1, 0), c1 = min(4 * txi + 4, fw - 1);
+    bool any = false;
+    for (int r = r0; r <= r1; ++r)
+        for (int c = c0; c <= c1; ++c) any |= fb[r * fw + c] != 0;
+    return any;
+}
+
+__device__ __forceinline__ int st_block_sum(int n, int* wsum) {
+#pragma unroll
+    for (int off = 32; off > 0; off >>= 1) n += __shfl_xor(n, off, 64);
+    __syncthreads();
+    if ((threadIdx.x & 63) == 0) wsum[threadIdx.x >> 6] = n;
+    __syncthreads();
+    return wsum[0] + wsum[1] + wsum[2] + wsum[3];
+}
+
+__global__ __launch_bounds__(256) void lwg_spade_tile_count_kernel(const unsigned char* __restrict__ flags, int fh, int fw, int ty, int tx, int* __restrict__ cnt) {
+    const int b = blockIdx.x, tpf = ty * tx;
+    const unsigned char* fb = flags + (size_t)b * fh * fw;
+    int n = 0;
+    for (int t = threadIdx.x; t < tpf; t += 256) n += st_active(fb, fh, fw, t / tx, t % tx) ? 1 : 0;
+    __shared__ int wsum[4];
+    const int s = st_block_sum(n, wsum);
+    if (threadIdx.x == 0) cnt[b] = s;
+}
+
+__global__ __launch_bounds__(256) void lwg_spade_tile_write_kernel(const unsigned char* __restrict__ flags, int B, int fh, int fw, int ty, int tx,
+                                                                  const int* __restrict__ cnt, int* __restrict__ ids_a, int* __restrict__ ids_i,
+                                                                  int* __restrict__ off_a, int* __restrict__ off_i) {
+    const int b = blockIdx.x, tpf = ty * tx, lane = threadIdx.x & 63, wid = threadIdx.x >> 6;
+    const unsigned char* fb = flags + (size_t)b * fh * fw;
+    __shared__ int wsum[4];
+    int n = 0;
+    for (int k = threadIdx.x; k < b; k += 256) n += cnt[k];
+    const int base_a = st_block_sum(n, wsum);
+    const int base_i = b * tpf - base_a;
+    int run = 0;
+    for (int t0 = 0; t0 < tpf; t0 += 256) {
+        const int t = t0 + (int)threadIdx.x;
+        const bool in = t < tpf;
+        const bool act = in && st_active(fb, fh, fw, t / tx, t % tx);
+        const unsigned long long m = __builtin_amdgcn_ballot_w64(act);
+        __syncthreads();
+        if (lane == 0) wsum[wid] = __builtin_popcountll(m);
+        __syncthreads();
+        int before = run;
+        for (int k = 0; k < wid; ++k) before += wsum[k];
+        before += __builtin_popcountll(m & ((1ull << lane) - 1ull));
+        if (in) {
+            if (act) ids_a[base_a + before] = b * tpf + t;
+            else ids_i[base_i + (t - before)] = b * tpf + t;
+        }
+        run += wsum[0] + wsum[1] + wsum[2] + wsum[3];
+    }
+    if (threadIdx.x == 0) {
+        off_a[b] = base_a;
+        off_i[b] = base_i;
+        if (b == B - 1) {
+            off_a[B] = base_a + run;
+            off_i[B] = B * tpf - (base_a + run);
+        }
+    }
+}
+
+extern "C" int lwg_spade_tile_lists(const unsigned char* flags, int B, int fh, int fw, int ty, int tx, int* work, int* ids_active, int* ids_inactive,
+                                    int* off_active, int* off_inactive, lwg_stream_t stream_) {
+    if (!flags || !work || !ids_active || !ids_inactive || !off_active || !off_inactive || B <= 0 || B > 65535 || fh <= 0 || fw <= 0 || ty <= 0 || tx <= 0 ||
+        fh != 2 * ty || fw != 4 * tx || (long long)B * ty * tx >= 0x3fffffffll)
+        return (int)hipErrorInvalidValue;
+    hipStream_t stream = reinterpret_cast<hipStream_t>(stream_);
+    hipLaunchKernelGGL(lwg_spade_tile_count_kernel, dim3((unsigned)B), dim3(256), 0, stream, flags, fh, fw, ty, tx, work);
+    hipLaunchKernelGGL(lwg_spade_tile_write_kernel, dim3((unsigned)B), dim3(256), 0, stream, flags, B, fh, fw, ty, tx, work, ids_active, ids_inactive,
+                       off_active, off_inactive);
+    return (int)hipGetLastError();
+}
+
+#define ST_MAX_GRID 2048
+__device__ __forceinline__ bool st_locate(const int* __restrict__ ids, int i, int B, int ty, int tx, int& b, int& y0, int& x0, int& cy0, int& cx0) {
+    const int tpf = ty * tx;
+    const int id = ids[i];
+    if (id < 0 || id >= B * tpf) return false;
+    b = id / tpf;
+    const int t = id - b * tpf, tyi = t / tx, txi = t - tyi * tx;
+    y0 = tyi * ST_TH, x0 = txi * ST_TW;
+    cy0 = (tyi == 0 ? 0 : tyi == ty - 1 ? 2 : 1) * ST_TH;
+    cx0 = (txi == 0 ? 0 : txi == tx - 1 ? 2 : 1) * ST_TW;
+    return true;
+}
+
+__global__ __launch_bounds__(256) void lwg_spade_fill_tiles_kernel(const float* __restrict__ canon, float* __restrict__ y, int B, int H, int W, int C,
+                                                                  const int* __restrict__ ids, const int* __restrict__ cnt) {
+    const int c4 = C >> 2, tiles = B * (H / ST_TH) * (W / ST_TW), n = min(*cnt, tiles);
+    for (int i = blockIdx.x; i < n; i += gridDim.x) {
+    int b, y0, x0, cy0, cx0;
+    if (!st_locate(ids, i, B, H / ST_TH, W / ST_TW, b, y0, x0, cy0, cx0)) continue;
+    for (int e = threadIdx.x; e < ST_TH * ST_TW * c4; e += 256) {
+        const int q = e % c4, p = e / c4, py = p / ST_TW, px = p - py * ST_TW;
+        const floatx4 v = *reinterpret_cast<const floatx4*>(canon + ((size_t)(cy0 + py) * ST_CW + cx0 + px) * C + 4 * q);
+        *reinterpret_cast<floatx4*>(y + (((size_t)b * H + y0 + py) * W + x0 + px) * C + 4 * q) = v;
+    }
+    }
+}
+
+__global__ __launch_bounds__(256) void lwg_spade_const_tiles_kernel(const float* __restrict__ gbc, const float* __restrict__ xn, const float* __restrict__ mean,
+                                                                   const float* __restrict__ rstd, float* __restrict__ y, int B, int H, int W, int C,
+                                                                   const int* __restrict__ ids, const int* __restrict__ cnt) {
+    const int c4 = C >> 2, tiles = B * (H / ST_TH) * (W / ST_TW), n = min(*cnt, tiles);
+    for (int i = blockIdx.x; i < n; i += gridDim.x) {
+    int b, y0, x0, cy0, cx0;
+    if (!st_locate(ids, i, B, H / ST_TH, W / ST_TW, b, y0, x0, cy0, cx0)) continue;
+    for (int e = threadIdx.x; e < ST_TH * ST_TW * c4; e += 256) {
+        const int q = e % c4, p = e / c4, py = p / ST_TW, px = p - py * ST_TW;
+        const int ch = 4 * q, col = (ch >> 5) * 64 + (ch & 31);
+        const float* g = gbc + ((size_t)(cy0 + py) * ST_CW + cx0 + px) * (2 * C) + col;
+        const floatx4 gm = *reinterpret_cast<const floatx4*>(g), bt = *reinterpret_cast<const floatx4*>(g + 32);
+        const floatx4 mu = *reinterpret_cast<const floatx4*>(mean + (size_t)b * C + ch), rs = *reinterpret_cast<const floatx4*>(rstd + (size_t)b * C + ch);
+        const size_t o = (((size_t)b * H + y0 + py) * W + x0 + px) * C + ch;
+        const floatx4 xv = *reinterpret_cast<const floatx4*>(xn + o);
+        floatx4 r;
+#pragma unroll
+        for (int k = 0; k < 4; ++k) r[k] = lwg_spade_modulate(xv[k], mu[k], rs[k], gm[k], bt[k]);
+        *reinterpret_cast<floatx4*>(y + o) = r;
+    }
+    }
+}
+
+static int st_grid(int B, int H, int W) {
+    const long long t = (long long)B * (H / ST_TH) * (W / ST_TW);
+    return (int)(t < ST_MAX_GRID ? t : ST_MAX_GRID);
+}
+static bool st_shape_ok(int B, int H, int W, int C) {
+    return B > 0 && H >= 2 * ST_TH && W >= 2 * ST_TW && (H % ST_TH) == 0 && (W % ST_TW) == 0 && C > 0 && (C % 32) == 0 &&
+           (long long)B * (H / ST_TH) * (W / ST_TW) < 0x3fffffffll;
+}
+
+extern "C" int lwg_spade_fill_tiles_f32(const float* canon, float* y, int B, int H, int W, int C, const int* tile_ids, const int* tile_off, lwg_stream_t stream_) {
+    if (!canon || !y || !tile_ids || !tile_off || !st_shape_ok(B, H, W, C)) return (int)hipErrorInvalidValue;
+    hipLaunchKernelGGL(lwg_spade_fill_tiles_kernel, dim3((unsigned)st_grid(B, H, W)), dim3(256), 0, reinterpret_cast<hipStream_t>(stream_), canon, y,
+                       B, H, W, C, tile_ids, tile_off + B);
+    return (int)hipGetLastError();
+}
+
+extern "C" int lwg_spade_const_tiles_f32(const float* gb_canon, const float* xn, const float* mean, const float* rstd, float* y, int B, int H, int W, int C,
+                                         const int* tile_ids, const int* tile_off, lwg_stream_t stream_) {
+    if (!gb_canon || !xn || !mean || !rstd || !y || !tile_ids || !tile_off || !st_shape_ok(B, H, W, C)) return (int)hipErrorInvalidValue;
+    hipLaunchKernelGGL(lwg_spade_const_tiles_kernel, dim3((unsigned)st_grid(B, H, W)), dim3(256), 0, reinterpret_cast<hipStream_t>(stream_), gb_canon,
+                       xn, mean, rstd, y, B, H, W, C, tile_ids, tile_off + B);
+    return (int)hipGetLastError();
+}
diff --git a/ipercore_amd/networks/generator.py b/ipercore_amd/networks/generator.py
--- a/ipercore_amd/networks/generator.py
+++ b/ipercore_amd/networks/generator.py
@@ -259,9 +259,13 @@
         if tuple(flow.shape[2:4]) != (h, w):
             raise NotImplementedError("the attention block takes flows resized to its feature size: non-square feature maps are not built "
                                       "(image_size is one number throughout the reference)")
+        sparse = ops.spade_sparse_eligible(tsf_x, st["shared"], st["gb"])
+        flags = torch.empty(B, (h + 7) // 8, (w + 7) // 8, device=tsf_x.device, dtype=torch.uint8) if sparse else None
         att = ops.lwb_attention_x(tsf_x, kv[0], kv[2], kv[1], st["bv"], flow, torch.empty_like(tsf_x), stats=ws,
-                                  src_batched=batched)
+                                  src_batched=batched, **({"flags": flags} if sparse else {}))
         ops.instnorm_finalize(ws, B, C, nrec, mean, rstd, eps=1e-5)
+        if sparse:
+            return ops.spade_sparse(att, flags, st["bv"], st["shared"], st["gb"], tsf_x, mean, rstd, torch.empty_like(tsf_x))
         actv = ops.conv2d(att, st["shared"], tsf_x.new_empty(B, h, w, st["shared"].N), act=ops.ACT_RELU)
         return ops.conv2d(actv, st["gb"], torch.empty_like(tsf_x), epi=ops.EPI_SPADE, xn=tsf_x, mean=mean, rstd=rstd)
 
diff --git a/ipercore_amd/ops.py b/ipercore_amd/ops.py
--- a/ipercore_amd/ops.py
+++ b/ipercore_amd/ops.py
@@ -399,6 +399,100 @@
     return y
 
 
+SPARSE_SPADE = True
+SPARSE_SPADE_MIN_TILES = 32
+SPARSE_SPADE_MIN_BATCH_TILES = 1024
+SPADE_TILE_H, SPADE_TILE_W = 16, 32
+
+
+def spade_sparse_eligible(x, shared, gb, splitk=False):
+    if not SPARSE_SPADE or splitk or CONV_PRECISION != "winograd" or not x.is_cuda or x.dtype != torch.float32:
+        return False
+    B, h, w, C = x.shape
+    if h % SPADE_TILE_H or w % SPADE_TILE_W or h < 2 * SPADE_TILE_H or w < 2 * SPADE_TILE_W or gb.N != 2 * C or shared.Cin != C or gb.Cin != shared.N:
+        return False
+    tiles = (h // SPADE_TILE_H) * (w // SPADE_TILE_W)
+    if tiles < SPARSE_SPADE_MIN_TILES or B * tiles < SPARSE_SPADE_MIN_BATCH_TILES:
+        return False
+    actv = x.new_empty((B, h, w, shared.N), device="meta")
+    return (_wino_eligible(shared, x, actv, None, EPI_NONE, ACT_RELU, None, False) and _wino4_use(shared, False) and
+            _wino_eligible(gb, actv, x, None, EPI_SPADE, ACT_NONE, None, False) and _wino4_use(gb, False))
+
+
+def spade_tile_lists(flags, ty, tx):
+    B, fh, fw = flags.shape
+    assert flags.dtype == torch.uint8 and (fh, fw) == (2 * ty, 4 * tx), (tuple(flags.shape), ty, tx)
+    i32 = torch.int32
+    buf = torch.empty(2 * B * ty * tx + 3 * B + 2, device=flags.device, dtype=i32)
+    n = B * ty * tx
+    ids_a, ids_i, off_a, off_i, work = buf[:n], buf[n:2 * n], buf[2 * n:2 * n + B + 1], buf[2 * n + B + 1:2 * n + 2 * B + 2], buf[2 * n + 2 * B + 2:]
+    _lib.check(_lib.lib().lwg_spade_tile_lists(_ptr(flags, torch.uint8), B, fh, fw, ty, tx, _ptr(work, i32), _ptr(ids_a, i32), _ptr(ids_i, i32),
+                                              _ptr(off_a, i32), _ptr(off_i, i32), _stream()), "lwg_spade_tile_lists")
+    return ids_a, off_a, ids_i, off_i
+
+
+def conv2d_winograd4_tiles(x0, spec, y, tile_ids, tile_off, epi=EPI_NONE, act=ACT_NONE, res=None, xn=None, mean=None, rstd=None):
+    a = conv_args(x0, spec, y, None, epi, act, res, xn, mean, rstd)
+    if CONV_PRECISION != "winograd" or not _wino_eligible(spec, x0, y, None, epi, act, None, False) or not _wino4_use(spec, False):
+        raise ValueError("conv2d_winograd4_tiles: not a launch of the F(4x4, 3x3) kernel")
+    assert tile_off.numel() == x0.shape[0] + 1 and tile_ids.dtype == torch.int32 and tile_off.dtype == torch.int32
+    a.w = _ptr(_wwino4(spec))
+    _lib.check(_lib.lib().lwg_conv2d_winograd4_tiles_f32(a, _ptr(tile_ids, torch.int32), _ptr(tile_off, torch.int32), _stream()),
+               "lwg_conv2d_winograd4_tiles_f32")
+    return y
+
+
+def spade_fill_tiles(canon, y, tile_ids, tile_off):
+    B, H, W, C = y.shape
+    assert tuple(canon.shape) == (1, 3 * SPADE_TILE_H, 3 * SPADE_TILE_W, C) and tile_off.numel() == B + 1
+    _lib.check(_lib.lib().lwg_spade_fill_tiles_f32(_ptr(canon), _ptr(y), B, H, W, C, _ptr(tile_ids, torch.int32), _ptr(tile_off, torch.int32), _stream()),
+               "lwg_spade_fill_tiles_f32")
+    return y
+
+
+def spade_const_tiles(gb_canon, xn, mean, rstd, y, tile_ids, tile_off):
+    B, H, W, C = y.shape
+    assert tuple(gb_canon.shape) == (1, 3 * SPADE_TILE_H, 3 * SPADE_TILE_W, 2 * C) and tuple(xn.shape) == (B, H, W, C) and tile_off.numel() == B + 1
+    assert tuple(mean.shape) == (B, C) and tuple(rstd.shape) == (B, C)
+    _lib.check(_lib.lib().lwg_spade_const_tiles_f32(_ptr(gb_canon), _ptr(xn), _ptr(mean), _ptr(rstd), _ptr(y), B, H, W, C, _ptr(tile_ids, torch.int32),
+                                                   _ptr(tile_off, torch.int32), _stream()), "lwg_spade_const_tiles_f32")
+    return y
+
+
+def spade_canonical(bv, shared, gb):
+    global CONV_HOOK
+    C = bv.numel()
+    frame = (bv.reshape(1, 1, 1, C) + 0.0).expand(1, 3 * SPADE_TILE_H, 3 * SPADE_TILE_W, C).contiguous()
+    hook, CONV_HOOK = CONV_HOOK, None
+    try:
+        actv_c = conv2d(frame, shared, frame.new_empty(1, 3 * SPADE_TILE_H, 3 * SPADE_TILE_W, shared.N), act=ACT_RELU)
+        gb_c = conv2d(actv_c, gb, frame.new_empty(1, 3 * SPADE_TILE_H, 3 * SPADE_TILE_W, gb.N))
+    finally:
+        CONV_HOOK = hook
+    return actv_c, gb_c
+
+
+def spade_sparse(att, flags, bv, shared, gb, xn, mean, rstd, out):
+    B, h, w, C = att.shape
+    ty, tx = h // SPADE_TILE_H, w // SPADE_TILE_W
+    ids_a, off_a, ids_i, off_i = spade_tile_lists(flags, ty, tx)
+    actv_c, gb_c = spade_canonical(bv, shared, gb)
+    actv = att.new_empty(B, h, w, shared.N)
+    a = conv_args(att, shared, actv, None, EPI_NONE, ACT_RELU)
+    if CONV_HOOK is not None:
+        CONV_HOOK(True, a.M, shared, EPI_NONE, None)
+    conv2d_winograd4_tiles(att, shared, actv, ids_a, off_a, act=ACT_RELU)
+    spade_fill_tiles(actv_c, actv, ids_i, off_i)
+    if CONV_HOOK is not None:
+        CONV_HOOK(False, a.M, shared, EPI_NONE, {"kernels": 2, "kind": "winograd4"})
+        CONV_HOOK(True, a.M, gb, EPI_SPADE, None)
+    conv2d_winograd4_tiles(actv, gb, out, ids_a, off_a, epi=EPI_SPADE, xn=xn, mean=mean, rstd=rstd)
+    spade_const_tiles(gb_c, xn, mean, rstd, out, ids_i, off_i)
+    if CONV_HOOK is not None:
+        CONV_HOOK(False, a.M, gb, EPI_SPADE, {"kernels": 2, "kind": "winograd4"})
+    return out
+
+
 WINO_UP4 = True
 F32_UP4 = True
 BF16_UP4 = True
@@ -589,7 +683,7 @@
     return n
 
 
-def lwb_attention_x(x, Kq, kappa, Vs, bv, T, out, stats=None, src_batched=False):
+def lwb_attention_x(x, Kq, kappa, Vs, bv, T, out, stats=None, src_batched=False, flags=None):
     B, h, w, C = x.shape
     ns = T.shape[1]
     nsrc = B * ns if src_batched else ns
@@ -599,8 +693,16 @@
     assert stats is None or stats.numel() >= B * attn_records(h, w, C, x.dtype) * C * 3
     if x.dtype == torch.bfloat16:
         bf = torch.bfloat16
+        if flags is not None:
+            raise ValueError("lwb_attention_x: activity flags are written by the fp32 form only")
         _lib.check(_lib.lib().lwg_lwb_attention_x_bf16(_ptr(x, bf), _ptr(Kq, bf), _ptr(kappa), _ptr(Vs, bf), _ptr(bv), _ptr(T), _ptr(out, bf),
                                                         _ptr(stats), B, ns, h, w, C, 1 if src_batched else 0, _stream()), "lwg_lwb_attention_x_bf16")
+        return out
+    if flags is not None:
+        assert tuple(flags.shape) == (B, (h + 7) // 8, (w + 7) // 8) and flags.dtype == torch.uint8
+        _lib.check(_lib.lib().lwg_lwb_attention_x_flags_f32(_ptr(x), _ptr(Kq), _ptr(kappa), _ptr(Vs), _ptr(bv), _ptr(T), _ptr(out), _ptr(stats),
+                                                             _ptr(flags, torch.uint8), B, ns, h, w, C, 1 if src_batched else 0, _stream()),
+                   "lwg_lwb_attention_x_flags_f32")
         return out
     _lib.check(_lib.lib().lwg_lwb_attention_x_f32(_ptr(x), _ptr(Kq), _ptr(kappa), _ptr(Vs), _ptr(bv), _ptr(T), _ptr(out), _ptr(stats), B, ns, h, w,
                                                    C, 1 if src_batched else 0, _stream()), "lwg_lwb_attention_x_f32")
```

Result: faster. 1284 frames/s (median of 6 runs) (+5.5%).
